# frank-xwang/InstanceDiffusion

Hardware: AMD Instinct MI355X
Metric: images/sec at 512x512, 50 PLMS steps, N=8 instances (Multi-instance Sampler) (higher is better)
Workload: dtype bf16; 1 GPU; C3: SD-1.5 InstanceDiffusion UNet (1.228B params, seeded random weights), 64x64 latent (512x512), 50 PLMS steps, CFG 7.5, N=8 boxes, MIS 0.36, alpha [0.8,0,0.2]; images_per_gpu=32, unet_forwards_per_image=406

## Files before the change

include/idf.h:

```cpp
#ifndef IDF_H_
#define IDF_H_

#include <stdint.h>

#ifdef __cplusplus
extern "C" {
#endif

#define IDF_ABI_VERSION 5

enum { IDF_BF16 = 0, IDF_F16 = 1 };
enum { IDF_E_ARG = -1, IDF_E_ALIGN = -2, IDF_E_UNSUPPORTED = -3 };

enum {
  IDF_EPI_BIAS     = 1,
  IDF_EPI_ROWBIAS  = 2,
  IDF_EPI_RES      = 4,
  IDF_EPI_GATE     = 8,
  IDF_EPI_SILU     = 16,
  IDF_EPI_GELU     = 32,
  IDF_EPI_GEGLU    = 64,
  IDF_EPI_OUT_F32  = 128,
  IDF_EPI_OUT_NCHW = 256,
  IDF_EPI_LN_ROW   = 512,
  IDF_EPI_LN_COL   = 1024,
  IDF_EPI_GEGLU_P32 = 2048
};

int idf_abi_version(void);
const char* idf_build_info(void);

enum { IDF_TUNE_GEMM_BIG = 0, IDF_TUNE_ATTN2 = 1, IDF_TUNE_GEMM_RING = 2, IDF_TUNE_BIG_MIN_EFF = 3, IDF_TUNE_ATTN8 = 4, IDF_TUNE_MLP = 5,
       IDF_TUNE_QKV_ROW = 6, IDF_TUNE_GEGLU_ROW = 7 };
int idf_set_tuning(int knob, int value);
enum { IDF_STAT_GEMM_BIG_LAUNCHES = 0, IDF_STAT_ATTN2_LAUNCHES = 1, IDF_STAT_GEMM_RING_LAUNCHES = 2, IDF_STAT_ATTN8_LAUNCHES = 3,
       IDF_STAT_GN_EPI_LAUNCHES = 4 ,
       IDF_STAT_QKV_ROW_LAUNCHES = 6 ,
       IDF_STAT_GEGLU_ROW_LAUNCHES = 7  };
long long idf_get_stat(int stat);

typedef struct {
  const void* A; const void* W; void* out;
  const float* bias; const void* rowbias; const void* res; const float* gate;
  int M, N, K;
  int lda, ldw, ldo, ldr, ld_rowbias;
  int rows_per_batch;
  int batch; long long strideA, strideW, strideO, strideR;
  int epi; int dtype;
  void* ws; long long ws_bytes;
  const float* ln_stats; long long stride_ln_stats;
  const float* ln_c;
  const float* ln_d;
  float* out_stats; float out_stats_eps;
  float ln_eps; float* ln_stats_out;
  void* vt_out; int ld_vt; int vt_col0;
} idf_gemm_args;
int idf_gemm(const idf_gemm_args* a, void* stream);

typedef struct {
  const void* x; int ldx;
  const float* ln_stats;
  const void* w1; int ldw1;
  const float* cd;
  const void* w2p; int ldw2;
  const float* b2;
  const float* gate;
  void* out; int ldo;
  int M, C;
  int dtype;
} idf_mlp_args;
int idf_mlp_geglu(const idf_mlp_args* a, void* stream);

int idf_row_stats(const void* x, int ldx, float* stats, int M, int C, float eps, int dtype, void* stream);

typedef struct {
  const void* x; const void* W; void* out;
  const float* bias; const void* rowbias; const void* res;
  int B, Hin, Win, Cin, Cout;
  int stride;
  int upsample;
  int ldx, ldo, ldr, ld_rowbias;
  int n_valid;
  int epi; int dtype;
  void* ws; long long ws_bytes;
  float* gn_partial;
} idf_conv3x3_args;
int idf_conv3x3(const idf_conv3x3_args* a, void* stream);

int idf_conv_in(const float* x_nchw, const float* w , const float* bias, void* out,
                int B, int Cin, int H, int W, int Cout, int dtype, void* stream);

typedef struct {
  const void* q; int ldq; long long strideQ; int nq;
  const void* k0; int ldk0; long long strideK0; const void* vt0; int ldv0; long long strideV0; int n0;
  const void* k1; int ldk1; long long strideK1; const void* vt1; int ldv1; long long strideV1; int n1;
  void* out; int ldo; long long strideO;
  int B, H, d;
  float scale;
  int dtype;
  const void* qbits; long long strideQb;
  const void* kbits0; long long strideKb0;
  const void* kbits1; long long strideKb1;
} idf_attn_args;
int idf_attention(const idf_attn_args* a, void* stream);

long long idf_groupnorm_ws_floats(int B, int HW);
int idf_groupnorm(const void* x, void* out, const float* gamma, const float* beta, float* ws,
                  int B, int HW, int C, float eps, int silu, int dtype, void* stream);
int idf_groupnorm_stats(const void* x, float* partial, int B, int HW, int C, int nchunks, int dtype, void* stream);
int idf_groupnorm_apply(const void* x, void* out, const float* gamma, const float* beta, const float* partial,
                        int B, int HW, int C, int nchunks, float eps, int silu, int dtype, void* stream);

int idf_layernorm(const void* x, int ldx, void* out, int ldo, const float* gamma, const float* beta,
                  int M, int C, float eps, int dtype, void* stream);

int idf_layernorm_patch2(const void* x, void* out, int ldo, const float* gamma, const float* beta,
                         int B, int H, int W, int C, float eps, int dtype, void* stream);

int idf_seg_in_conv(const float* segs, const float* w , const float* bias, void* out,
                    int B, int Cin, int S, int ldo, int dtype, void* stream);
int idf_dwconv7x7(const void* x, const float* w_tap_major, const float* bias, void* out, int B, int H, int W, int C,
                  int dtype, void* stream);

int idf_scaleu_concat(const void* h, const void* skip, void* out, const float* hscale, const float* sm1,
                      float* ws, int B, int H, int W, int Ch, int Cs, int dtype, void* stream);

int idf_timestep_embedding(const float* t, void* out, int B, int dim, int dtype, void* stream);

int idf_unifusion_embed(const float* text, const float* loc, const float* tmask, const float* lmask,
                        const float* null_text, const float* null_loc, const float* freqs , void* out,
                        int rows, int text_dim, int D, int dtype, void* stream);

int idf_cfg_combine(const float* eps_cond, const float* eps_uncond, float guidance, float* e_t,
                    long long n, void* stream);
int idf_plms_update(const float* x, const float* e_t, const float* e1, const float* e2, const float* e3,
                    const float* e_next, int mode, float a_t, float a_prev, float sqrt_1m_at,
                    float* x_out, long long n, void* stream);

int idf_mis_merge(const float* lat, const int* boxes, float* out, int n_inst, int B, int C, int H, int W,
                  int mode, void* stream);

int idf_softmax_rows(const float* s, void* p, long long rows, int n, long long lds, long long ldp, float scale,
                     int dtype, void* stream);
int idf_pointwise_nchw(const float* x, const float* w , const float* bias, float* out, int B, int Cin,
                       int Cout, long long HW, float in_scale, void* stream);

int idf_cast_f32_to_16(const float* x, void* out, long long n, int dtype, void* stream);

#ifdef __cplusplus
}
#endif
#endif
```

instancediffusion_amd/_lib.py:

```python
from __future__ import annotations

import ctypes as C
import os

_HERE = os.path.dirname(os.path.abspath(__file__))
LIB_PATH = os.environ.get("IDF_LIB_PATH", os.path.join(_HERE, "libidf_gfx950.so"))

IDF_BF16, IDF_F16 = 0, 1
IDF_STAT_GEMM_BIG_LAUNCHES, IDF_STAT_ATTN2_LAUNCHES, IDF_STAT_GEMM_RING_LAUNCHES, IDF_STAT_ATTN8_LAUNCHES, IDF_STAT_GN_EPI_LAUNCHES = 0, 1, 2, 3, 4
IDF_STAT_QKV_ROW_LAUNCHES, IDF_STAT_GEGLU_ROW_LAUNCHES = 6, 7
IDF_TUNE_GEMM_BIG, IDF_TUNE_ATTN2, IDF_TUNE_GEMM_RING, IDF_TUNE_BIG_MIN_EFF, IDF_TUNE_ATTN8, IDF_TUNE_MLP, IDF_TUNE_QKV_ROW, IDF_TUNE_GEGLU_ROW = 0, 1, 2, 3, 4, 5, 6, 7
EPI_LN_ROW, EPI_LN_COL, EPI_GEGLU_P32 = 512, 1024, 2048
EPI_BIAS, EPI_ROWBIAS, EPI_RES, EPI_GATE, EPI_SILU, EPI_GELU, EPI_GEGLU, EPI_OUT_F32, EPI_OUT_NCHW = \
    1, 2, 4, 8, 16, 32, 64, 128, 256

vp, ll, ci, cf = C.c_void_p, C.c_longlong, C.c_int, C.c_float


class GemmArgs(C.Structure):
    _fields_ = [("A", vp), ("W", vp), ("out", vp), ("bias", vp), ("rowbias", vp), ("res", vp), ("gate", vp),
                ("M", ci), ("N", ci), ("K", ci),
                ("lda", ci), ("ldw", ci), ("ldo", ci), ("ldr", ci), ("ld_rowbias", ci),
                ("rows_per_batch", ci),
                ("batch", ci), ("strideA", ll), ("strideW", ll), ("strideO", ll), ("strideR", ll),
                ("epi", ci), ("dtype", ci), ("ws", vp), ("ws_bytes", ll),
                ("ln_stats", vp), ("stride_ln_stats", ll), ("ln_c", vp), ("ln_d", vp),
                ("out_stats", vp), ("out_stats_eps", cf),
                ("ln_eps", cf), ("ln_stats_out", vp),
                ("vt_out", vp), ("ld_vt", ci), ("vt_col0", ci)]


class ConvArgs(C.Structure):
    _fields_ = [("x", vp), ("W", vp), ("out", vp), ("bias", vp), ("rowbias", vp), ("res", vp),
                ("B", ci), ("Hin", ci), ("Win", ci), ("Cin", ci), ("Cout", ci),
                ("stride", ci), ("upsample", ci),
                ("ldx", ci), ("ldo", ci), ("ldr", ci), ("ld_rowbias", ci),
                ("n_valid", ci), ("epi", ci), ("dtype", ci), ("ws", vp), ("ws_bytes", ll), ("gn_partial", vp)]


class AttnArgs(C.Structure):
    _fields_ = [("q", vp), ("ldq", ci), ("strideQ", ll), ("nq", ci),
                ("k0", vp), ("ldk0", ci), ("strideK0", ll), ("vt0", vp), ("ldv0", ci), ("strideV0", ll), ("n0", ci),
                ("k1", vp), ("ldk1", ci), ("strideK1", ll), ("vt1", vp), ("ldv1", ci), ("strideV1", ll), ("n1", ci),
                ("out", vp), ("ldo", ci), ("strideO", ll),
                ("B", ci), ("H", ci), ("d", ci), ("scale", cf), ("dtype", ci),
                ("qbits", vp), ("strideQb", ll), ("kbits0", vp), ("strideKb0", ll), ("kbits1", vp), ("strideKb1", ll)]


class MlpArgs(C.Structure):
    _fields_ = [("x", vp), ("ldx", ci), ("ln_stats", vp), ("w1", vp), ("ldw1", ci), ("cd", vp), ("w2p", vp), ("ldw2", ci),
                ("b2", vp), ("gate", vp), ("out", vp), ("ldo", ci), ("M", ci), ("C", ci), ("dtype", ci)]


SYMBOLS = {
    "idf_abi_version": (ci, []),
    "idf_build_info": (C.c_char_p, []),
    "idf_set_tuning": (ci, [ci, ci]),
    "idf_get_stat": (ll, [ci]),
    "idf_gemm": (ci, [C.POINTER(GemmArgs), vp]),
    "idf_conv3x3": (ci, [C.POINTER(ConvArgs), vp]),
    "idf_mlp_geglu": (ci, [C.POINTER(MlpArgs), vp]),
    "idf_conv_in": (ci, [vp, vp, vp, vp, ci, ci, ci, ci, ci, ci, vp]),
    "idf_attention": (ci, [C.POINTER(AttnArgs), vp]),
    "idf_groupnorm_ws_floats": (ll, [ci, ci]),
    "idf_groupnorm": (ci, [vp, vp, vp, vp, vp, ci, ci, ci, cf, ci, ci, vp]),
    "idf_groupnorm_stats": (ci, [vp, vp, ci, ci, ci, ci, ci, vp]),
    "idf_groupnorm_apply": (ci, [vp, vp, vp, vp, vp, ci, ci, ci, ci, cf, ci, ci, vp]),
    "idf_layernorm": (ci, [vp, ci, vp, ci, vp, vp, ci, ci, cf, ci, vp]),
    "idf_row_stats": (ci, [vp, ci, vp, ci, ci, cf, ci, vp]),
    "idf_layernorm_patch2": (ci, [vp, vp, ci, vp, vp, ci, ci, ci, ci, cf, ci, vp]),
    "idf_seg_in_conv": (ci, [vp, vp, vp, vp, ci, ci, ci, ci, ci, vp]),
    "idf_dwconv7x7": (ci, [vp, vp, vp, vp, ci, ci, ci, ci, ci, vp]),
    "idf_scaleu_concat": (ci, [vp, vp, vp, vp, vp, vp, ci, ci, ci, ci, ci, ci, vp]),
    "idf_timestep_embedding": (ci, [vp, vp, ci, ci, ci, vp]),
    "idf_unifusion_embed": (ci, [vp, vp, vp, vp, vp, vp, vp, vp, ci, ci, ci, ci, vp]),
    "idf_cfg_combine": (ci, [vp, vp, cf, vp, ll, vp]),
    "idf_plms_update": (ci, [vp, vp, vp, vp, vp, vp, ci, cf, cf, cf, vp, ll, vp]),
    "idf_mis_merge": (ci, [vp, vp, vp, ci, ci, ci, ci, ci, ci, vp]),
    "idf_cast_f32_to_16": (ci, [vp, vp, ll, ci, vp]),
    "idf_softmax_rows": (ci, [vp, vp, ll, ci, ll, ll, cf, ci, vp]),
    "idf_pointwise_nchw": (ci, [vp, vp, vp, vp, ci, ci, ci, ll, cf, vp]),
}

_lib = None


def load() -> C.CDLL:
    global _lib
    if _lib is not None:
        return _lib
    if not os.path.exists(LIB_PATH):
        raise RuntimeError(
            f"{LIB_PATH} is missing: the MI355X HIP extension has not been built "
            f"(run instancediffusion_amd/csrc/build.sh or __graft_entry__.build()). "
            f"There is no CPU fallback for the InstanceDiffusion sampling path.")
    import torch
    lib = C.CDLL(LIB_PATH)
    for name, (res, args) in SYMBOLS.items():
        fn = getattr(lib, name)
        fn.restype = res
        fn.argtypes = args
    if lib.idf_abi_version() != 5:
        raise RuntimeError("libidf_gfx950.so ABI version mismatch")
    _lib = lib
    return lib


class IdfError(RuntimeError):
    pass


def check(status: int, what: str):
    if status != 0:
        kind = {-1: "invalid argument", -2: "misaligned pointer/leading dimension", -3: "unsupported"}.get(
            status, f"hipError_t {status}")
        raise IdfError(f"{what} failed: {kind}")
```

instancediffusion_amd/csrc/gemm_conv.hip:

```cpp
#include "gemm_core.h"
#include "attn_core.h"
#include <cstdlib>

using namespace idfcore;

namespace {

#ifndef IDF_GEMM_BIG_DEFAULT
#define IDF_GEMM_BIG_DEFAULT 1
#endif
constexpr int LSTR = 72;

template <int DT, int BM, int BN, int WM, int WN, int KLOOP_LDS_BYTES>
__device__ __forceinline__ void tile_epilogue(const CoreParams& p, f32x16 (&acc)[WN / 32][WM / 32], unsigned short* smem,
                                              int m0, int n0, int bz, int wm, int wn, int lane, int wave) {
  constexpr int TM = WM / 32, TN = WN / 32;
  const int l31 = lane & 31, hi = lane >> 5;
  constexpr int CSTR = WN + 4;
  static_assert(4 * WM * CSTR * 4 <= KLOOP_LDS_BYTES, "C staging must fit in the allocated LDS");
  __syncthreads();
  float* Cl = reinterpret_cast<float*>(smem) + wave * (WM * CSTR);
#pragma unroll
  for (int a = 0; a < TN; ++a)
#pragma unroll
    for (int b = 0; b < TM; ++b)
#pragma unroll
      for (int q = 0; q < 4; ++q)
        *reinterpret_cast<f32x4*>(Cl + (b * 32 + l31) * CSTR + a * 32 + 8 * q + 4 * hi) =
            f32x4{acc[a][b][4 * q], acc[a][b][4 * q + 1], acc[a][b][4 * q + 2], acc[a][b][4 * q + 3]};
  __builtin_amdgcn_fence(__ATOMIC_RELEASE, "wavefront");
  __builtin_amdgcn_wave_barrier();
  __builtin_amdgcn_fence(__ATOMIC_ACQUIRE, "wavefront");

  const int epi = p.epi;
  const float gate = (epi & IDF_EPI_GATE) ? p.gate[0] : 0.0f;
  const int mw = m0 + wm * WM, nw = n0 + wn * WN;
  if (epi & IDF_EPI_GEGLU) {
    if constexpr (WN >= 64) {
      constexpr int CHV = WN / 16;
      constexpr int RPP = 64 / CHV;
      const int P = (epi & IDF_EPI_GEGLU_P32) ? 32 : 64, half = P >> 1, cpg = P >> 4;
#pragma unroll
      for (int pass = 0; pass < WM / RPP; ++pass) {
        const int row = pass * RPP + lane / CHV, c = lane % CHV;
        const int grp = c / cpg, cc = c - grp * cpg;
        const int m = mw + row;
        const int npk = nw + grp * P + cc * 8;
        if (m < p.M && npk + half < p.N) {
          const float* src = Cl + row * CSTR + grp * P + cc * 8;
          float v[8], g[8];
          *reinterpret_cast<f32x4*>(v) = *reinterpret_cast<const f32x4*>(src);
          *reinterpret_cast<f32x4*>(v + 4) = *reinterpret_cast<const f32x4*>(src + 4);
          *reinterpret_cast<f32x4*>(g) = *reinterpret_cast<const f32x4*>(src + half);
          *reinterpret_cast<f32x4*>(g + 4) = *reinterpret_cast<const f32x4*>(src + half + 4);
          const f32x4 bv0 = *reinterpret_cast<const f32x4*>(p.bias + npk), bv1 = *reinterpret_cast<const f32x4*>(p.bias + npk + 4);
          const f32x4 bg0 = *reinterpret_cast<const f32x4*>(p.bias + npk + half), bg1 = *reinterpret_cast<const f32x4*>(p.bias + npk + half + 4);
          if (epi & IDF_EPI_LN_ROW) {
            const f32x2 st = *reinterpret_cast<const f32x2*>(p.ln_stats + (size_t)bz * p.stride_ln_stats + 2 * (size_t)m);
#pragma unroll
            for (int e = 0; e < 8; ++e) {
              v[e] = st[1] * fmaf(-st[0], p.ln_c[npk + e], v[e]);
              g[e] = st[1] * fmaf(-st[0], p.ln_c[npk + half + e], g[e]);
            }
          }
#pragma unroll
          for (int e = 0; e < 4; ++e) {
            v[e] = (v[e] + bv0[e]) * gelu_erf_f(g[e] + bg0[e]);
            v[e + 4] = (v[e + 4] + bv1[e]) * gelu_erf_f(g[e + 4] + bg1[e]);
          }
          const int j = (nw + grp * P) / 2 + cc * 8;
          unsigned short* o = reinterpret_cast<unsigned short*>(p.out) + (size_t)bz * p.strideO + (size_t)m * p.ldo + j;
          if ((p.ldo & 7) == 0) {
            *reinterpret_cast<u32x4*>(o) = pack8<DT>(v);
          } else {
            const u32x4 pk = pack8<DT>(v);
            *reinterpret_cast<u32x2*>(o) = u32x2{pk[0], pk[1]};
            *reinterpret_cast<u32x2*>(o + 4) = u32x2{pk[2], pk[3]};
          }
        }
      }
    }
    return;
  }
  constexpr int CH = WN / 8;
  constexpr int RPP = 64 / CH;
#pragma unroll
  for (int pass = 0; pass < WM / RPP; ++pass) {
    const int row = pass * RPP + lane / CH, c = lane % CH;
    const int m = mw + row, n = nw + c * 8;
    if (m >= p.M || n >= p.N) continue;
    const float* src = Cl + row * CSTR + c * 8;
    float v[8];
    *reinterpret_cast<f32x4*>(v) = *reinterpret_cast<const f32x4*>(src);
    *reinterpret_cast<f32x4*>(v + 4) = *reinterpret_cast<const f32x4*>(src + 4);
    if (p.splitk > 1) {
      float* o = p.ws + ((size_t)blockIdx.z * p.M + m) * p.N + n;
      if (n + 7 < p.N && ((p.N & 3) == 0)) {
        *reinterpret_cast<f32x4*>(o) = f32x4{v[0], v[1], v[2], v[3]};
        *reinterpret_cast<f32x4*>(o + 4) = f32x4{v[4], v[5], v[6], v[7]};
      } else {
#pragma unroll
        for (int e = 0; e < 8; ++e) if (n + e < p.N) o[e] = v[e];
      }
    } else {
      epilogue8<DT>(p, bz, m, n, v, gate);
    }
  }
}

template <int DT, int BM, int BN, int WM, int WN, bool CONV>
__global__ __launch_bounds__(256, 2) void gemm_kernel(const CoreParams p) {
  constexpr int TM = WM / 32, TN = WN / 32;
  constexpr int WAVES_N = BN / WN;
  constexpr int AR = BM / 32, WR = BN / 32;
  static_assert((BM / WM) * (BN / WN) == 4, "4 waves per workgroup");
  extern __shared__ __attribute__((aligned(16))) unsigned short smem[];
  constexpr int BUF = (BM + BN) * LSTR;

  const int tid = threadIdx.x;
  const int lane = tid & 63, wave = tid >> 6;
  const int l31 = lane & 31, hi = lane >> 5;
  const int wn = wave % WAVES_N, wm = wave / WAVES_N;
  int tile;
  {
    const int T = gridDim.x, L = blockIdx.x;
    const int q = T >> 3, r = T & 7, xcd = L & 7, i = L >> 3;
    tile = (xcd < r ? xcd * (q + 1) : r * (q + 1) + (xcd - r) * q) + i;
  }
  const int tiles_n = (p.N + BN - 1) / BN;
  const int m_tile = tile / tiles_n;
  const int n0 = (tile - m_tile * tiles_n) * BN, m0 = m_tile * BM;
  const int bz = (p.splitk > 1) ? 0 : blockIdx.z;

  const unsigned short* Wb = p.W + (size_t)bz * p.strideW;
  const unsigned short* Ab = p.A + (size_t)bz * p.strideA;

  const int c = tid & 7, r0 = tid >> 3;
  const unsigned short* wrow[WR];
#pragma unroll
  for (int i = 0; i < WR; ++i) {
    int n = min(n0 + r0 + 32 * i, p.N - 1);
    wrow[i] = Wb + (size_t)n * p.ldw + c * 8;
  }
  const unsigned short* arow[AR];
  int ay[AR], ax[AR];
#pragma unroll
  for (int i = 0; i < AR; ++i) {
    int m = min(m0 + r0 + 32 * i, p.M - 1);
    if (CONV) {
      int hw = p.Ho * p.Wo;
      int b = m / hw, rem = m - b * hw;
      int yo = rem / p.Wo, xo = rem - yo * p.Wo;
      ay[i] = yo * p.stride - 1;
      ax[i] = xo * p.stride - 1;
      arow[i] = Ab + (size_t)b * p.Hin * p.Win * p.lda + c * 8;
    } else {
      ay[i] = ax[i] = 0;
      arow[i] = Ab + (size_t)m * p.lda + c * 8;
    }
  }
  const int nk_all = p.K / BK;
  const int kt_begin = (p.splitk > 1) ? blockIdx.z * p.kt_per_slice : 0;
  const int nk = (p.splitk > 1) ? min(p.kt_per_slice, nk_all - kt_begin) : nk_all;
  int tap = 0, ci0 = 0;
  if (CONV) { tap = (kt_begin * BK) / p.Cin; ci0 = kt_begin * BK - tap * p.Cin; }

  u32x4 raA[AR], rwA[WR], raB[AR], rwB[WR];
  unsigned okA = 0, okB = 0;
  auto load_tile = [&](int kt, u32x4* ra, u32x4* rw, unsigned& okbits) {
#pragma unroll
    for (int i = 0; i < WR; ++i) rw[i] = *reinterpret_cast<const u32x4*>(wrow[i] + (size_t)(kt_begin + kt) * BK);
    if (CONV) {
      const int ky = tap / 3, kx = tap - ky * 3;
      const int Hup = p.Hin << p.up, Wup = p.Win << p.up;
      unsigned bits = 0;
#pragma unroll
      for (int i = 0; i < AR; ++i) {
        const int yi = ay[i] + ky, xi = ax[i] + kx;
        const bool ok = (yi >= 0) & (yi < Hup) & (xi >= 0) & (xi < Wup);
        const int ys = min(max(yi, 0), Hup - 1) >> p.up, xs = min(max(xi, 0), Wup - 1) >> p.up;
        ra[i] = *reinterpret_cast<const u32x4*>(arow[i] + ((size_t)ys * p.Win + xs) * p.lda + ci0);
        bits |= (ok ? 1u : 0u) << i;
      }
      okbits = bits;
      ci0 += BK;
      if (ci0 >= p.Cin) { ci0 = 0; ++tap; }
    } else {
#pragma unroll
      for (int i = 0; i < AR; ++i) ra[i] = *reinterpret_cast<const u32x4*>(arow[i] + (size_t)(kt_begin + kt) * BK);
    }
  };
  auto store_tile = [&](int buf, const u32x4* ra, const u32x4* rw, unsigned okbits) {
    unsigned short* Al = smem + buf * BUF;
    unsigned short* Wl = Al + BM * LSTR;
#pragma unroll
    for (int i = 0; i < AR; ++i) {
      u32x4 v = ra[i];
      if (CONV) {
        const unsigned keep = ((okbits >> i) & 1u) ? 0xffffffffu : 0u;
        v[0] &= keep; v[1] &= keep; v[2] &= keep; v[3] &= keep;
      }
      *reinterpret_cast<u32x4*>(Al + (r0 + 32 * i) * LSTR + c * 8) = v;
    }
#pragma unroll
    for (int i = 0; i < WR; ++i) *reinterpret_cast<u32x4*>(Wl + (r0 + 32 * i) * LSTR + c * 8) = rw[i];
  };

  f32x16 acc[TN][TM];
#pragma unroll
  for (int a = 0; a < TN; ++a)
#pragma unroll
    for (int b = 0; b < TM; ++b)
#pragma unroll
      for (int r = 0; r < 16; ++r) acc[a][b][r] = 0.0f;

  auto compute = [&](int buf) {
    const unsigned short* Al = smem + buf * BUF;
    const unsigned short* Wl = Al + BM * LSTR;
    const unsigned short* af_base = Al + (wm * WM + l31) * LSTR + hi * 8;
    const unsigned short* wf_base = Wl + (wn * WN + l31) * LSTR + hi * 8;
    u32x4 wf[2][TN], af[2][TM];
#pragma unroll
    for (int a = 0; a < TN; ++a) wf[0][a] = *reinterpret_cast<const u32x4*>(wf_base + a * 32 * LSTR);
#pragma unroll
    for (int b = 0; b < TM; ++b) af[0][b] = *reinterpret_cast<const u32x4*>(af_base + b * 32 * LSTR);
#pragma unroll
    for (int ks = 0; ks < BK / 16; ++ks) {
      const int cur = ks & 1, nxt = cur ^ 1;
      if (ks + 1 < BK / 16) {
#pragma unroll
        for (int a = 0; a < TN; ++a) wf[nxt][a] = *reinterpret_cast<const u32x4*>(wf_base + a * 32 * LSTR + (ks + 1) * 16);
#pragma unroll
        for (int b = 0; b < TM; ++b) af[nxt][b] = *reinterpret_cast<const u32x4*>(af_base + b * 32 * LSTR + (ks + 1) * 16);
      }
#pragma unroll
      for (int a = 0; a < TN; ++a)
#pragma unroll
        for (int b = 0; b < TM; ++b) acc[a][b] = Elem<DT>::mfma32(wf[cur][a], af[cur][b], acc[a][b]);
    }
  };

  load_tile(0, raA, rwA, okA);
  store_tile(0, raA, rwA, okA);
  if (nk > 1) load_tile(1, raA, rwA, okA);
  __syncthreads();
  int kt = 0;
  for (; kt + 3 < nk; kt += 2) {
    load_tile(kt + 2, raB, rwB, okB);
    __builtin_amdgcn_sched_barrier(0);
    compute(0);
    store_tile(1, raA, rwA, okA);
    __syncthreads();
    load_tile(kt + 3, raA, rwA, okA);
    __builtin_amdgcn_sched_barrier(0);
    compute(1);
    store_tile(0, raB, rwB, okB);
    __syncthreads();
  }
  const int rem = nk - kt;
  if (rem == 3) {
    load_tile(kt + 2, raB, rwB, okB);
    compute(0);
    store_tile(1, raA, rwA, okA);
    __syncthreads();
    compute(1);
    store_tile(0, raB, rwB, okB);
    __syncthreads();
    compute(0);
  } else if (rem == 2) {
    compute(0);
    store_tile(1, raA, rwA, okA);
    __syncthreads();
    compute(1);
  } else {
    compute(0);
  }

  tile_epilogue<DT, BM, BN, WM, WN, 2 * (BM + BN) * LSTR * 2>(p, acc, smem, m0, n0, bz, wm, wn, lane, wave);
}

template <int DT, int BM, int BN, int WM, int WN, bool CONV>
__global__ __launch_bounds__(256, 2) void gemm_kernel_dma(const CoreParams p) {
  constexpr int TM = WM / 32, TN = WN / 32;
  constexpr int WAVES_N = BN / WN;
  constexpr int RS = 64;
  constexpr int BUF = (BM + BN) * RS;
  constexpr int W_INST = BN / 8 / 4, A_INST = BM / 8 / 4;
  constexpr int AR = BM / 32;
  constexpr int KLOOP_LDS = 2 * BUF * 2;
  constexpr int CSTAGE = 4 * WM * (WN + 4) * 4;
  constexpr int LDS_BYTES = KLOOP_LDS > CSTAGE ? KLOOP_LDS : CSTAGE;
  static_assert((BM / WM) * (BN / WN) == 4, "4 waves per workgroup");
  extern __shared__ __attribute__((aligned(16))) unsigned short smem[];

  const int tid = threadIdx.x;
  const int lane = tid & 63, wave = __builtin_amdgcn_readfirstlane(tid >> 6);
  const int l31 = lane & 31, hi = lane >> 5;
  const int wn = wave % WAVES_N, wm = wave / WAVES_N;
  int tile;
  {
    const int T = gridDim.x, L = blockIdx.x;
    const int q = T >> 3, r = T & 7, xcd = L & 7, i = L >> 3;
    tile = (xcd < r ? xcd * (q + 1) : r * (q + 1) + (xcd - r) * q) + i;
  }
  const int tiles_n = (p.N + BN - 1) / BN;
  const int m_tile = tile / tiles_n;
  const int n0 = (tile - m_tile * tiles_n) * BN, m0 = m_tile * BM;
  const int bz = (p.splitk > 1) ? 0 : blockIdx.z;
  const unsigned short* Wb = p.W + (size_t)bz * p.strideW;
  const unsigned short* Ab = p.A + (size_t)bz * p.strideA;

  const int nk_all = p.K / BK;
  const int kt_begin = (p.splitk > 1) ? blockIdx.z * p.kt_per_slice : 0;
  const int nk = (p.splitk > 1) ? min(p.kt_per_slice, nk_all - kt_begin) : nk_all;

  const int dr = lane >> 3, dc = lane & 7;
  const unsigned short* wsrc[W_INST];
#pragma unroll
  for (int j = 0; j < W_INST; ++j) {
    const int row = 8 * (wave + 4 * j) + dr;
    const int n = min(n0 + row, p.N - 1);
    wsrc[j] = Wb + (size_t)n * p.ldw + (size_t)kt_begin * BK + ((dc ^ ((row >> 1) & 7)) * 8);
  }
  const unsigned short* asrc[A_INST];
  if (!CONV) {
#pragma unroll
    for (int j = 0; j < A_INST; ++j) {
      const int row = 8 * (wave + 4 * j) + dr;
      const int m = min(m0 + row, p.M - 1);
      asrc[j] = Ab + (size_t)m * p.lda + (size_t)kt_begin * BK + ((dc ^ ((row >> 1) & 7)) * 8);
    }
  }
  const int c = tid & 7, r0 = tid >> 3;
  const unsigned short* arow[AR];
  int ay[AR], ax[AR];
  int tap = 0, ci0 = 0;
  if (CONV) {
#pragma unroll
    for (int i = 0; i < AR; ++i) {
      const int m = min(m0 + r0 + 32 * i, p.M - 1);
      const int hw = p.Ho * p.Wo;
      const int b = m / hw, rem = m - b * hw;
      const int yo = rem / p.Wo, xo = rem - yo * p.Wo;
      ay[i] = yo * p.stride - 1;
      ax[i] = xo * p.stride - 1;
      arow[i] = Ab + (size_t)b * p.Hin * p.Win * p.lda + c * 8;
    }
    tap = (kt_begin * BK) / p.Cin;
    ci0 = kt_begin * BK - tap * p.Cin;
  }
  const int a_sw = (c ^ ((r0 >> 1) & 7)) * 8;
  u32x4 ra[AR];
  unsigned okbits = 0;

  auto dma_tile = [&](int kt, int buf) {
    unsigned short* Al = smem + buf * BUF;
    unsigned short* Wl = Al + BM * RS;
#pragma unroll
    for (int j = 0; j < W_INST; ++j)
      __builtin_amdgcn_global_load_lds((const __attribute__((address_space(1))) void*)(wsrc[j] + (size_t)kt * BK),
                                       (__attribute__((address_space(3))) void*)(Wl + 8 * (wave + 4 * j) * RS), 16, 0, 0);
    if (!CONV) {
#pragma unroll
      for (int j = 0; j < A_INST; ++j)
        __builtin_amdgcn_global_load_lds((const __attribute__((address_space(1))) void*)(asrc[j] + (size_t)kt * BK),
                                         (__attribute__((address_space(3))) void*)(Al + 8 * (wave + 4 * j) * RS), 16, 0, 0);
    }
  };
  auto gather_tile = [&]() {
    const int ky = tap / 3, kx = tap - ky * 3;
    const int Hup = p.Hin << p.up, Wup = p.Win << p.up;
    unsigned bits = 0;
#pragma unroll
    for (int i = 0; i < AR; ++i) {
      const int yi = ay[i] + ky, xi = ax[i] + kx;
      const bool ok = (yi >= 0) & (yi < Hup) & (xi >= 0) & (xi < Wup);
      const int ys = min(max(yi, 0), Hup - 1) >> p.up, xs = min(max(xi, 0), Wup - 1) >> p.up;
      ra[i] = *reinterpret_cast<const u32x4*>(arow[i] + ((size_t)ys * p.Win + xs) * p.lda + ci0);
      bits |= (ok ? 1u : 0u) << i;
    }
    okbits = bits;
    ci0 += BK;
    if (ci0 >= p.Cin) { ci0 = 0; ++tap; }
  };
  auto scatter_tile = [&](int buf) {
    unsigned short* Al = smem + buf * BUF;
#pragma unroll
    for (int i = 0; i < AR; ++i) {
      u32x4 v = ra[i];
      const unsigned keep = ((okbits >> i) & 1u) ? 0xffffffffu : 0u;
      v[0] &= keep; v[1] &= keep; v[2] &= keep; v[3] &= keep;
      *reinterpret_cast<u32x4*>(Al + (r0 + 32 * i) * RS + a_sw) = v;
    }
  };

  f32x16 acc[TN][TM];
#pragma unroll
  for (int a = 0; a < TN; ++a)
#pragma unroll
    for (int b = 0; b < TM; ++b)
#pragma unroll
      for (int r = 0; r < 16; ++r) acc[a][b][r] = 0.0f;

  const int f_sw = (l31 >> 1) & 7;
  auto compute = [&](int buf) {
    const unsigned short* Al = smem + buf * BUF;
    const unsigned short* Wl = Al + BM * RS;
    const unsigned short* af_base = Al + (wm * WM + l31) * RS;
    const unsigned short* wf_base = Wl + (wn * WN + l31) * RS;
    u32x4 wf[2][TN], af[2][TM];
    {
      const int slot = (hi ^ f_sw) * 8;
#pragma unroll
      for (int a = 0; a < TN; ++a) wf[0][a] = *reinterpret_cast<const u32x4*>(wf_base + a * 32 * RS + slot);
#pragma unroll
      for (int b = 0; b < TM; ++b) af[0][b] = *reinterpret_cast<const u32x4*>(af_base + b * 32 * RS + slot);
    }
#pragma unroll
    for (int ks = 0; ks < BK / 16; ++ks) {
      const int cur = ks & 1, nxt = cur ^ 1;
      if (ks + 1 < BK / 16) {
        const int slot = (((ks + 1) * 2 + hi) ^ f_sw) * 8;
#pragma unroll
        for (int a = 0; a < TN; ++a) wf[nxt][a] = *reinterpret_cast<const u32x4*>(wf_base + a * 32 * RS + slot);
#pragma unroll
        for (int b = 0; b < TM; ++b) af[nxt][b] = *reinterpret_cast<const u32x4*>(af_base + b * 32 * RS + slot);
      }
#pragma unroll
      for (int a = 0; a < TN; ++a)
#pragma unroll
        for (int b = 0; b < TM; ++b) acc[a][b] = Elem<DT>::mfma32(wf[cur][a], af[cur][b], acc[a][b]);
    }
  };

  dma_tile(0, 0);
  if (CONV) { gather_tile(); scatter_tile(0); }
  __syncthreads();
  for (int kt = 0; kt < nk; ++kt) {
    const bool more = (kt + 1 < nk);
    if (more) {
      dma_tile(kt + 1, (kt + 1) & 1);
      if (CONV) gather_tile();
    }
    compute(kt & 1);
    if (CONV && more) scatter_tile((kt + 1) & 1);
    __syncthreads();
  }
  tile_epilogue<DT, BM, BN, WM, WN, LDS_BYTES>(p, acc, smem, m0, n0, bz, wm, wn, lane, wave);
}

__device__ __attribute__((aligned(128))) unsigned short ring_zero_page[64];

__device__ __forceinline__ void ring_dma16(const void* addr , const void* lds_lane0) {
  const unsigned l = __builtin_amdgcn_readfirstlane((unsigned)(size_t)lds_lane0);
  asm volatile("s_mov_b32 m0, %0\n\ts_nop 0\n\tglobal_load_lds_dwordx4 %1, off" ::"s"(l), "v"(addr) : "memory");
}
template <int PT, int MAXA> __device__ __forceinline__ void ring_wait(int ahead) {
  if constexpr (MAXA <= 0) {
    asm volatile("s_waitcnt vmcnt(0)" ::: "memory");
  } else {
    static_assert(MAXA * PT < 64, "vmcnt is a 6-bit field");
    if (ahead >= MAXA) asm volatile("s_waitcnt vmcnt(%0)" ::"n"(MAXA * PT) : "memory");
    else ring_wait<PT, MAXA - 1>(ahead);
  }
}

template <int DT, int BM, int BN, int WM, int WN, bool CONV, int NS>
__global__ __launch_bounds__(256, 1) void gemm_kernel_ring(const CoreParams p) {
  constexpr int TM = WM / 32, TN = WN / 32;
  constexpr int WAVES_N = BN / WN;
  constexpr int RS = 64;
  constexpr int BUF = (BM + BN) * RS;
  constexpr int W_INST = BN / 8 / 4, A_INST = BM / 8 / 4;
  constexpr int PER_TILE = W_INST + A_INST;
  constexpr int KLOOP_LDS = NS * BUF * 2;
  constexpr int CSTAGE = 4 * WM * (WN + 4) * 4;
  constexpr int LDS_BYTES = KLOOP_LDS > CSTAGE ? KLOOP_LDS : CSTAGE;
  static_assert((BM / WM) * (BN / WN) == 4, "4 waves per workgroup");
  static_assert(NS >= 3 && LDS_BYTES <= 160 * 1024, "ring must fit the CU's LDS");
  extern __shared__ __attribute__((aligned(16))) unsigned short smem[];

  const int tid = threadIdx.x;
  const int lane = tid & 63, wave = __builtin_amdgcn_readfirstlane(tid >> 6);
  const int l31 = lane & 31, hi = lane >> 5;
  const int wn = wave % WAVES_N, wm = wave / WAVES_N;
  int tile;
  {
    const int T = gridDim.x, L = blockIdx.x;
    const int q = T >> 3, r = T & 7, xcd = L & 7, i = L >> 3;
    tile = (xcd < r ? xcd * (q + 1) : r * (q + 1) + (xcd - r) * q) + i;
  }
  const int tiles_n = (p.N + BN - 1) / BN;
  const int m_tile = tile / tiles_n;
  const int n0 = (tile - m_tile * tiles_n) * BN, m0 = m_tile * BM;
  const int bz = (p.splitk > 1) ? 0 : blockIdx.z;
  const unsigned short* Wb = p.W + (size_t)bz * p.strideW;
  const unsigned short* Ab = p.A + (size_t)bz * p.strideA;

  const int nk_all = p.K / BK;
  const int kt_begin = (p.splitk > 1) ? blockIdx.z * p.kt_per_slice : 0;
  const int nk = (p.splitk > 1) ? min(p.kt_per_slice, nk_all - kt_begin) : nk_all;

  const int dr = lane >> 3, dc = lane & 7;
  const unsigned short* wsrc[W_INST];
#pragma unroll
  for (int j = 0; j < W_INST; ++j) {
    const int row = 8 * (wave + 4 * j) + dr;
    const int n = min(n0 + row, p.N - 1);
    wsrc[j] = Wb + (size_t)n * p.ldw + (size_t)kt_begin * BK + ((dc ^ ((row >> 1) & 7)) * 8);
  }
  const unsigned short* asrc[A_INST];
  int ay[A_INST], ax[A_INST];
#pragma unroll
  for (int j = 0; j < A_INST; ++j) {
    const int row = 8 * (wave + 4 * j) + dr;
    const int m = min(m0 + row, p.M - 1);
    const int ch = (dc ^ ((row >> 1) & 7)) * 8;
    if (!CONV) {
      asrc[j] = Ab + (size_t)m * p.lda + (size_t)kt_begin * BK + ch;
      ay[j] = ax[j] = 0;
    } else {
      const int hw = p.Ho * p.Wo;
      const int b = m / hw, rem = m - b * hw;
      const int yo = rem / p.Wo, xo = rem - yo * p.Wo;
      ay[j] = yo * p.stride - 1;
      ax[j] = xo * p.stride - 1;
      asrc[j] = Ab + (size_t)b * p.Hin * p.Win * p.lda + ch;
    }
  }
  int tap = 0, ci0 = 0;
  if (CONV) { tap = (kt_begin * BK) / p.Cin; ci0 = kt_begin * BK - tap * p.Cin; }
  int kt_issue = 0, st_issue = 0;

  auto issue_tile = [&]() {
    unsigned short* Al = smem + st_issue * BUF;
    unsigned short* Wl = Al + BM * RS;
#pragma unroll
    for (int j = 0; j < W_INST; ++j) ring_dma16(wsrc[j] + (size_t)kt_issue * BK, Wl + 8 * (wave + 4 * j) * RS);
    if (!CONV) {
#pragma unroll
      for (int j = 0; j < A_INST; ++j) ring_dma16(asrc[j] + (size_t)kt_issue * BK, Al + 8 * (wave + 4 * j) * RS);
    } else {
      const int ky = tap / 3, kx = tap - ky * 3;
      const int Hup = p.Hin << p.up, Wup = p.Win << p.up;
#pragma unroll
      for (int j = 0; j < A_INST; ++j) {
        const int yi = ay[j] + ky, xi = ax[j] + kx;
        const bool ok = (yi >= 0) & (yi < Hup) & (xi >= 0) & (xi < Wup);
        const int ys = yi >> p.up, xs = xi >> p.up;
        const unsigned short* src = ok ? asrc[j] + ((size_t)ys * p.Win + xs) * p.lda + ci0 : ring_zero_page + dc * 8;
        ring_dma16(src, Al + 8 * (wave + 4 * j) * RS);
      }
      ci0 += BK;
      if (ci0 >= p.Cin) { ci0 = 0; ++tap; }
    }
    ++kt_issue;
    st_issue = (st_issue + 1 == NS) ? 0 : st_issue + 1;
  };

  f32x16 acc[TN][TM];
#pragma unroll
  for (int a = 0; a < TN; ++a)
#pragma unroll
    for (int b = 0; b < TM; ++b)
#pragma unroll
      for (int r = 0; r < 16; ++r) acc[a][b][r] = 0.0f;

  const int f_sw = (l31 >> 1) & 7;
  auto compute = [&](int st) {
    const unsigned short* Al = smem + st * BUF;
    const unsigned short* Wl = Al + BM * RS;
    const unsigned short* af_base = Al + (wm * WM + l31) * RS;
    const unsigned short* wf_base = Wl + (wn * WN + l31) * RS;
    u32x4 wf[2][TN], af[2][TM];
    {
      const int slot = (hi ^ f_sw) * 8;
#pragma unroll
      for (int a = 0; a < TN; ++a) wf[0][a] = *reinterpret_cast<const u32x4*>(wf_base + a * 32 * RS + slot);
#pragma unroll
      for (int b = 0; b < TM; ++b) af[0][b] = *reinterpret_cast<const u32x4*>(af_base + b * 32 * RS + slot);
    }
#pragma unroll
    for (int ks = 0; ks < BK / 16; ++ks) {
      const int cur = ks & 1, nxt = cur ^ 1;
      if (ks + 1 < BK / 16) {
        const int slot = (((ks + 1) * 2 + hi) ^ f_sw) * 8;
#pragma unroll
        for (int a = 0; a < TN; ++a) wf[nxt][a] = *reinterpret_cast<const u32x4*>(wf_base + a * 32 * RS + slot);
#pragma unroll
        for (int b = 0; b < TM; ++b) af[nxt][b] = *reinterpret_cast<const u32x4*>(af_base + b * 32 * RS + slot);
      }
#pragma unroll
      for (int a = 0; a < TN; ++a)
#pragma unroll
        for (int b = 0; b < TM; ++b) acc[a][b] = Elem<DT>::mfma32(wf[cur][a], af[cur][b], acc[a][b]);
    }
  };

  const int pre = min(NS - 1, nk);
  for (int i = 0; i < pre; ++i) issue_tile();
  int st = 0;
  for (int kt = 0; kt < nk; ++kt) {
    ring_wait<PER_TILE, NS - 2>(kt_issue - kt - 1);
    __builtin_amdgcn_s_barrier();
    if (kt_issue < nk) issue_tile();
    compute(st);
    st = (st + 1 == NS) ? 0 : st + 1;
  }
  tile_epilogue<DT, BM, BN, WM, WN, LDS_BYTES>(p, acc, smem, m0, n0, bz, wm, wn, lane, wave);
}

template <int DT>
__global__ __launch_bounds__(256) void splitk_reduce_kernel(const CoreParams p) {
  const int n8 = (p.N + 7) / 8;
  const size_t i = (size_t)blockIdx.x * 256 + threadIdx.x;
  if (i >= (size_t)p.tail_rows * n8) return;
  const int ml = (int)(i / n8), n = (int)(i - (size_t)ml * n8) * 8;
  const int m = p.tail_m0 + ml;
  float v[8] = {0.f, 0.f, 0.f, 0.f, 0.f, 0.f, 0.f, 0.f};
  const bool vec = (n + 7 < p.N) && ((p.N & 3) == 0);
  const size_t slab = (size_t)p.tail_rows * p.N;
  const float* w = p.ws + (size_t)ml * p.N + n;
  if (vec) {
    int s = 0;
    for (; s + 4 <= p.splitk; s += 4) {
      f32x4 a[4][2];
#pragma unroll
      for (int u = 0; u < 4; ++u) {
        a[u][0] = *reinterpret_cast<const f32x4*>(w + (size_t)(s + u) * slab);
        a[u][1] = *reinterpret_cast<const f32x4*>(w + (size_t)(s + u) * slab + 4);
      }
#pragma unroll
      for (int u = 0; u < 4; ++u)
#pragma unroll
        for (int e = 0; e < 4; ++e) { v[e] += a[u][0][e]; v[e + 4] += a[u][1][e]; }
    }
    for (; s < p.splitk; ++s) {
      const f32x4 w0 = *reinterpret_cast<const f32x4*>(w + (size_t)s * slab), w1 = *reinterpret_cast<const f32x4*>(w + (size_t)s * slab + 4);
#pragma unroll
      for (int e = 0; e < 4; ++e) { v[e] += w0[e]; v[e + 4] += w1[e]; }
    }
  } else {
    for (int s = 0; s < p.splitk; ++s) {
#pragma unroll
      for (int e = 0; e < 8; ++e) if (n + e < p.N) v[e] += w[(size_t)s * slab + e];
    }
  }
  const float gate = (p.epi & IDF_EPI_GATE) ? p.gate[0] : 0.0f;
  epilogue8<DT>(p, 0, m, n, v, gate);
}

std::atomic<long long> idf_stat_gn_epi_launches{0};
std::atomic<long long> idf_stat_ring_launches{0};
std::atomic<long long> idf_stat_gegluw_launches{0};
std::atomic<long long> idf_stat_qkvw_launches{0};
int g_big_mode = -2;
inline int gemm_big_mode() {
  if (g_big_mode == -2) {
    const char* e = getenv("IDF_GEMM_BIG");
    const int v = e ? atoi(e) : IDF_GEMM_BIG_DEFAULT;
    g_big_mode = (v < 0 || v > 3) ? IDF_GEMM_BIG_DEFAULT : v;
  }
  return g_big_mode;
}

inline int kloop_variant(bool conv) {
  static int v = -2;
  if (v == -2) { const char* e = getenv("IDF_GEMM_VARIANT"); v = e ? atoi(e) : -1; }
  if (v == 1 || v == 2) return v;
  return conv ? 1 : 2;
}

template <int DT, int BM, int BN, int WM, int WN, bool CONV>
int launch_cfg(const CoreParams& p, int batch, hipStream_t s) {
  const int variant = kloop_variant(CONV);
  void (*kern)(const CoreParams) = gemm_kernel<DT, BM, BN, WM, WN, CONV>;
  constexpr int cstage = 4 * WM * (WN + 4) * 4;
  constexpr int kloop2 = 2 * (BM + BN) * 64 * 2;
  int smem = 2 * (BM + BN) * LSTR * 2;
  if (variant == 2) { kern = gemm_kernel_dma<DT, BM, BN, WM, WN, CONV>; smem = kloop2 > cstage ? kloop2 : cstage; }
  static std::atomic<unsigned long long> attr_done[3];
  if (const int e = idf_lds_optin(reinterpret_cast<const void*>(kern), smem, attr_done[variant])) return e;
  CoreParams q = p;
  const int tiles = ((p.N + BN - 1) / BN) * ((p.M + BM - 1) / BM);
  const int nk = p.K / BK;
  q.splitk = 1; q.kt_per_slice = nk;
  q.tail_m0 = 0; q.tail_rows = p.M;
  if (batch == 1 && p.ws && !(p.epi & IDF_EPI_GEGLU) && tiles < 192 && nk >= 8) {
    int want = (512 + tiles - 1) / tiles;
    if (want > nk / 4) want = nk / 4;
    if (want > 64) want = 64;
    while (want > 1 && (size_t)want * p.M * p.N * sizeof(float) > p.ws_bytes) --want;
    if (want > 1) {
      q.kt_per_slice = (nk + want - 1) / want;
      q.splitk = (nk + q.kt_per_slice - 1) / q.kt_per_slice;
    }
  }
  dim3 grid(tiles, 1, q.splitk > 1 ? q.splitk : batch);
  hipLaunchKernelGGL(kern, grid, dim3(256), smem, s, q);
  if (q.splitk > 1) {
    const size_t n8 = (size_t)q.M * ((q.N + 7) / 8);
    hipLaunchKernelGGL(splitk_reduce_kernel<DT>, dim3((unsigned)((n8 + 255) / 256)), dim3(256), 0, s, q);
  }
  return idf_launch_status();
}

#ifndef IDF_GEMM_RING_DEFAULT
#define IDF_GEMM_RING_DEFAULT 256
#endif
int g_ring_tiles = -1;
inline int gemm_ring_tiles() {
  if (g_ring_tiles < 0) {
    const char* e = getenv("IDF_GEMM_RING");
    const int v = e ? atoi(e) : IDF_GEMM_RING_DEFAULT;
    g_ring_tiles = v < 0 ? IDF_GEMM_RING_DEFAULT : v;
  }
  return g_ring_tiles;
}

template <int DT, int BM, int BN, int WM, int WN, bool CONV, int NS>
int launch_ring_cfg(const CoreParams& p, int batch, hipStream_t s) {
  const int tiles = ((p.N + BN - 1) / BN) * ((p.M + BM - 1) / BM);
  const int nk = p.K / BK;
  static int batched_old = -1;
  if (batched_old < 0) { const char* e = getenv("IDF_RING_BATCHED"); batched_old = (e && e[0] == '1') ? 1 : 0; }
  if ((long long)tiles * (batched_old ? 1 : batch) > gemm_ring_tiles()) return IDF_BIG_UNSUPPORTED;
  const int slots = idf_num_cu();
  if (batch == 1 && p.ws && !(p.epi & IDF_EPI_GEGLU) && tiles * 2 > slots && tiles < 192 && nk >= 8) return IDF_BIG_UNSUPPORTED;
  void (*kern)(const CoreParams) = gemm_kernel_ring<DT, BM, BN, WM, WN, CONV, NS>;
  constexpr int cstage = 4 * WM * (WN + 4) * 4;
  constexpr int kloop = NS * (BM + BN) * 64 * 2;
  constexpr int smem = kloop > cstage ? kloop : cstage;
  static std::atomic<unsigned long long> attr_done{0};
  if (const int e = idf_lds_optin(reinterpret_cast<const void*>(kern), smem, attr_done)) return e;
  CoreParams q = p;
  q.splitk = 1; q.kt_per_slice = nk;
  q.tail_m0 = 0; q.tail_rows = p.M;
  static int slice_kt = 0;
  if (slice_kt == 0) { const char* e = getenv("IDF_RING_SLICE_KT"); slice_kt = e ? atoi(e) : 8; if (slice_kt < 1) slice_kt = 8; }
  if (batch == 1 && p.ws && !(p.epi & IDF_EPI_GEGLU) && tiles * 2 <= slots && nk >= 2 * slice_kt) {
    int want = slots / tiles;
    if (want > nk / slice_kt) want = nk / slice_kt;
    if (want > 64) want = 64;
    while (want > 1 && (size_t)want * p.M * p.N * sizeof(float) > p.ws_bytes) --want;
    if (want > 1) {
      q.kt_per_slice = (nk + want - 1) / want;
      q.splitk = (nk + q.kt_per_slice - 1) / q.kt_per_slice;
    }
  }
  dim3 grid(tiles, 1, q.splitk > 1 ? q.splitk : batch);
  hipLaunchKernelGGL(kern, grid, dim3(256), smem, s, q);
  ++idf_stat_ring_launches;
  if (q.splitk > 1) {
    const size_t n8 = (size_t)q.M * ((q.N + 7) / 8);
    hipLaunchKernelGGL(splitk_reduce_kernel<DT>, dim3((unsigned)((n8 + 255) / 256)), dim3(256), 0, s, q);
  }
  return idf_launch_status();
}

template <int DT, bool CONV>
int launch(const CoreParams& p, int batch, hipStream_t s, int* parts_out = nullptr, int* gst_out = nullptr) {
  const bool geglu = (p.epi & IDF_EPI_GEGLU) != 0;
  static int wide = -2;
  if (wide == -2) { const char* e = getenv("IDF_TILE_WIDE"); wide = e ? (e[0] == '1' ? 1 : 0) : -1; }
  const bool use_wide = (wide >= 0) ? (wide == 1) : CONV;
  const int big = gemm_big_mode();
  const bool t128p = geglu || (p.N % 128 == 0) || p.N > 1024 || (use_wide && p.N > 128);
  const long long tiles_small = (long long)((p.N + (t128p ? 127 : 63)) / (t128p ? 128 : 64)) * ((p.M + 127) / 128);
  const bool ring_first = big != 2 && gemm_ring_tiles() > 0 && tiles_small <= 128 && tiles_small <= gemm_ring_tiles();
  if (big > 0 && batch == 1 && !ring_first) {
    int splitk = 1, tail_m0 = 0;
    const int rc = idf_launch_big(p, DT, CONV, big == 2, s, &splitk, parts_out, big == 3 ? &tail_m0 : nullptr, gst_out);
    if (rc != IDF_BIG_UNSUPPORTED) {
      if (rc == 0 && splitk > 1) {
        CoreParams q = p;
        q.splitk = splitk; q.tail_m0 = tail_m0; q.tail_rows = p.M - tail_m0;
        const size_t n8 = (size_t)q.tail_rows * ((q.N + 7) / 8);
        hipLaunchKernelGGL(splitk_reduce_kernel<DT>, dim3((unsigned)((n8 + 255) / 256)), dim3(256), 0, s, q);
        return idf_launch_status();
      }
      return rc;
    }
  }
  CoreParams q = p;
  if ((p.epi & IDF_EPI_LN_ROW) && !p.ln_stats) {
    float* st = p.ln_stats_out ? p.ln_stats_out : p.ws;
    if (!st || (!p.ln_stats_out && p.ws_bytes < (size_t)p.M * 2 * sizeof(float))) return IDF_E_ARG;
    const int rc = idf_row_stats(p.A, p.lda, st, p.M, p.K, p.ln_eps, DT, s);
    if (rc) return rc;
    q.ln_stats = st; q.stride_ln_stats = 0;
    if (!p.ln_stats_out) { q.ws = nullptr; q.ws_bytes = 0; }
  }
  const bool t128 = geglu || (q.N % 128 == 0) || q.N > 1024 || (use_wide && q.N > 128);
  if (gemm_ring_tiles() > 0) {
    const int rc = t128 ? launch_ring_cfg<DT, 128, 128, 64, 64, CONV, 4>(q, batch, s) : launch_ring_cfg<DT, 128, 64, 64, 32, CONV, 5>(q, batch, s);
    if (rc != IDF_BIG_UNSUPPORTED) return rc;
  }
  if (t128) return launch_cfg<DT, 128, 128, 64, 64, CONV>(q, batch, s);
  return launch_cfg<DT, 128, 64, 64, 32, CONV>(q, batch, s);
}

}

__global__ __launch_bounds__(256) void stats_finalize_kernel(const float* __restrict__ parts, int P, float cols, float* __restrict__ out,
                                                            int M, float eps) {
  const int m = blockIdx.x * 256 + threadIdx.x;
  if (m >= M) return;
  const f32x2* pp = reinterpret_cast<const f32x2*>(parts) + (size_t)m * P;
  f32x2 t = pp[0];
  float mean = t[0], m2 = t[1], n = cols;
  for (int i = 1; i < P; ++i) {
    t = pp[i];
    const float dlt = t[0] - mean, nn = n + cols;
    mean += dlt * (cols / nn);
    m2 += t[1] + dlt * dlt * (n * cols / nn);
    n = nn;
  }
  reinterpret_cast<f32x2*>(out)[m] = f32x2{mean, rsqrtf(m2 / n + eps)};
}

int idf_stats_finalize(const float* stat_parts, int parts, int cols_per_part, float* out_stats, int M, float eps, hipStream_t s) {
  hipLaunchKernelGGL(stats_finalize_kernel, dim3((M + 255) / 256), dim3(256), 0, s, stat_parts, parts, (float)cols_per_part,
                     out_stats, M, eps);
  return idf_launch_status();
}

extern "C" int idf_set_tuning(int knob, int value) {
  if (knob == IDF_TUNE_GEMM_BIG) {
    if (value < 0 || value > 3) return IDF_E_ARG;
    const int prev = gemm_big_mode();
    g_big_mode = value;
    return prev;
  }
  if (knob == IDF_TUNE_GEMM_RING) {
    if (value < 0) return IDF_E_ARG;
    const int prev = gemm_ring_tiles();
    g_ring_tiles = value;
    return prev;
  }
  if (knob == IDF_TUNE_BIG_MIN_EFF) {
    if (value < 1 || value > 100) return IDF_E_ARG;
    return idf_big_min_eff_pct(value);
  }
  if (knob == IDF_TUNE_ATTN2) {
    if (value < 0 || value > 6) return IDF_E_ARG;
    return idf_attn2_set_mode(value);
  }
  if (knob == IDF_TUNE_ATTN8) {
    if (value < 0 || value > 6) return IDF_E_ARG;
    return idf_attn8_set_mode(value);
  }
  if (knob == IDF_TUNE_GEGLU_ROW) {
    if (value < 0 || value > 1) return IDF_E_ARG;
    return idf_gegluw_set_mode(value);
  }
  if (knob == IDF_TUNE_QKV_ROW) {
    if (value < 0 || value > 1) return IDF_E_ARG;
    return idf_qkvw_set_mode(value);
  }
  if (knob == IDF_TUNE_MLP) {
    if (value < 0 || value > 1) return IDF_E_ARG;
    return idf_mlp_set_mode(value);
  }
  return IDF_E_ARG;
}

extern "C" long long idf_get_stat(int stat) {
  if (stat == IDF_STAT_GEMM_BIG_LAUNCHES) return idf_stat_big_launches.load();
  if (stat == IDF_STAT_ATTN2_LAUNCHES) return idf_stat_attn2_launches.load();
  if (stat == IDF_STAT_GEMM_RING_LAUNCHES) return idf_stat_ring_launches.load();
  if (stat == IDF_STAT_ATTN8_LAUNCHES) return idf_stat_attn8_launches.load();
  if (stat == IDF_STAT_GN_EPI_LAUNCHES) return idf_stat_gn_epi_launches.load();
  if (stat == IDF_STAT_QKV_ROW_LAUNCHES) return idf_stat_qkvw_launches.load();
  if (stat == IDF_STAT_GEGLU_ROW_LAUNCHES) return idf_stat_gegluw_launches.load();
  return -1;
}

extern "C" int idf_gemm(const idf_gemm_args* a, void* stream) {
  if (!a || !a->A || !a->W || !a->out) return IDF_E_ARG;
  if (a->M <= 0 || a->N <= 0 || a->K <= 0 || (a->K % BK) != 0) return IDF_E_ARG;
  if ((a->lda % 8) || (a->ldw % 8) || !aligned16(a->A) || !aligned16(a->W)) return IDF_E_ALIGN;
  if ((a->epi & IDF_EPI_GATE) && !(a->epi & IDF_EPI_RES)) return IDF_E_ARG;
  if ((a->epi & IDF_EPI_RES) && !a->res) return IDF_E_ARG;
  if ((a->epi & (IDF_EPI_BIAS | IDF_EPI_GEGLU)) && !a->bias) return IDF_E_ARG;
  if ((a->epi & IDF_EPI_GEGLU) && ((a->N % 64) || (a->ldo % 4))) return IDF_E_ARG;
  if ((a->epi & IDF_EPI_GEGLU_P32) && !(a->epi & IDF_EPI_GEGLU)) return IDF_E_ARG;
  if ((a->epi & IDF_EPI_ROWBIAS) && (!a->rowbias || a->rows_per_batch <= 0)) return IDF_E_ARG;
  if (a->epi & IDF_EPI_OUT_NCHW) return IDF_E_ARG;
  CoreParams p{};
  p.W = (const unsigned short*)a->W; p.ldw = a->ldw; p.strideW = a->strideW; p.N = a->N;
  p.A = (const unsigned short*)a->A; p.lda = a->lda; p.strideA = a->strideA; p.M = a->M; p.K = a->K;
  p.out = a->out; p.ldo = a->ldo; p.strideO = a->strideO;
  p.bias = a->bias; p.rowbias = (const unsigned short*)a->rowbias; p.ld_rowbias = a->ld_rowbias;
  p.rows_per_batch = a->rows_per_batch;
  p.res = (const unsigned short*)a->res; p.ldr = a->ldr; p.strideR = a->strideR;
  p.gate = a->gate; p.epi = a->epi; p.n_valid = a->N;
  p.ws = (float*)a->ws; p.ws_bytes = a->ws ? (size_t)a->ws_bytes : 0;
  const int batch = a->batch > 0 ? a->batch : 1;
  if (a->epi & (IDF_EPI_LN_ROW | IDF_EPI_LN_COL)) {
    if ((a->epi & IDF_EPI_LN_ROW) && (a->epi & IDF_EPI_LN_COL)) return IDF_E_ARG;
    if (!a->ln_c) return IDF_E_ARG;
    if (!a->ln_stats) {
      if (!(a->epi & IDF_EPI_LN_ROW) || batch != 1 || (a->K % 8) || a->K > 1536 || !(a->ln_eps > 0.0f)) return IDF_E_ARG;
      if (a->ln_stats_out && (((uintptr_t)a->ln_stats_out) & 7u)) return IDF_E_ALIGN;
      p.ln_eps = a->ln_eps; p.ln_stats_out = a->ln_stats_out;
    }
    if ((a->epi & IDF_EPI_LN_ROW) && !(a->epi & IDF_EPI_BIAS)) return IDF_E_ARG;
    if ((a->epi & IDF_EPI_LN_COL) && (!a->ln_d || (a->epi & IDF_EPI_GEGLU))) return IDF_E_ARG;
    if ((((uintptr_t)a->ln_stats) & 7u) || (a->stride_ln_stats & 1)) return IDF_E_ALIGN;
    p.ln_stats = a->ln_stats; p.stride_ln_stats = a->stride_ln_stats; p.ln_c = a->ln_c; p.ln_d = a->ln_d;
  }
  if (a->out_stats) {
    if ((a->epi & (IDF_EPI_GEGLU | IDF_EPI_OUT_F32)) || (a->N % 8) || a->N > 1536 || (a->ldo % 8)) return IDF_E_ARG;
    if (batch > 1 && a->strideO != (long long)a->M * a->ldo) return IDF_E_ARG;
  }
  hipStream_t s = (hipStream_t)stream;
  int rc = IDF_E_UNSUPPORTED;
  if (a->vt_out) {
    const int Nv = a->N - a->vt_col0;
    if (a->vt_col0 <= 0 || Nv <= 0 || batch != 1 || a->ld_vt < a->M || (a->ld_vt % 8) || !aligned16(a->vt_out)) return IDF_E_ARG;
    if (a->epi & ~(IDF_EPI_BIAS | IDF_EPI_LN_ROW)) return IDF_E_ARG;
    if (!(a->epi & IDF_EPI_LN_ROW)) return IDF_E_ARG;
    if (a->out_stats) return IDF_E_ARG;
    const bool self_ln = (a->epi & IDF_EPI_LN_ROW) && !a->ln_stats;
    if (self_ln && !a->ln_stats_out) return IDF_E_ARG;
    p.vt_out = (unsigned short*)a->vt_out; p.ld_vt = a->ld_vt; p.vt_col0 = a->vt_col0;
    {
      int r = idf_launch_qkv320w(p, a->dtype, s);
      if (r == IDF_BIG_UNSUPPORTED) r = idf_launch_qkv640w(p, a->dtype, s);
      if (r != IDF_BIG_UNSUPPORTED) { if (r == 0) { ++idf_stat_big_launches; ++idf_stat_qkvw_launches; } return r; }
    }
    if (gemm_big_mode() > 0) {
      const int r = idf_launch_big(p, a->dtype, false, gemm_big_mode() == 2, s, nullptr);
      if (r != IDF_BIG_UNSUPPORTED) return r;
    }
    CoreParams p1 = p;
    p1.vt_out = nullptr; p1.vt_col0 = 0; p1.N = a->vt_col0; p1.n_valid = a->vt_col0;
    if (a->dtype == IDF_BF16) rc = launch<IDF_BF16, false>(p1, 1, s);
    else if (a->dtype == IDF_F16) rc = launch<IDF_F16, false>(p1, 1, s);
    if (rc) return rc;
    CoreParams p2{};
    p2.A = p.W + (size_t)a->vt_col0 * p.ldw; p2.lda = p.ldw; p2.M = Nv; p2.K = a->K;
    p2.W = p.A; p2.ldw = p.lda; p2.N = a->M; p2.n_valid = a->M;
    p2.out = a->vt_out; p2.ldo = a->ld_vt;
    p2.ws = p.ws; p2.ws_bytes = p.ws_bytes;
    p2.epi = 0;
    if (a->epi & IDF_EPI_LN_ROW) {
      p2.epi |= IDF_EPI_LN_COL;
      p2.ln_stats = self_ln ? a->ln_stats_out : a->ln_stats; p2.stride_ln_stats = 0;
      p2.ln_c = a->ln_c + a->vt_col0; p2.ln_d = a->bias + a->vt_col0;
    }
    if (a->dtype == IDF_BF16) return launch<IDF_BF16, false>(p2, 1, s);
    if (a->dtype == IDF_F16) return launch<IDF_F16, false>(p2, 1, s);
    return IDF_E_UNSUPPORTED;
  }
  int parts = 0;
  if ((a->epi & IDF_EPI_GEGLU) && batch == 1 && !a->out_stats) {
    const int r = idf_launch_geglu640w(p, a->dtype, s);
    if (r != IDF_BIG_UNSUPPORTED) { if (r == 0) { ++idf_stat_big_launches; ++idf_stat_gegluw_launches; } return r; }
  }
  if (a->out_stats && batch == 1 && p.ws) p.stat_parts = p.ws;
  if (a->dtype == IDF_BF16) rc = launch<IDF_BF16, false>(p, batch, s, &parts);
  else if (a->dtype == IDF_F16) rc = launch<IDF_F16, false>(p, batch, s, &parts);
  if (rc == 0 && a->out_stats) {
    if (parts > 0) rc = idf_stats_finalize(p.stat_parts, parts, a->N / parts, a->out_stats, a->M, a->out_stats_eps, s);
    else rc = idf_row_stats(a->out, a->ldo, a->out_stats, batch * a->M, a->N, a->out_stats_eps, a->dtype, stream);
  }
  return rc;
}

extern "C" int idf_conv3x3(const idf_conv3x3_args* a, void* stream) {
  if (!a || !a->x || !a->W || !a->out) return IDF_E_ARG;
  if (a->B <= 0 || a->Cin <= 0 || (a->Cin % BK) != 0 || a->Cout <= 0) return IDF_E_ARG;
  if (a->stride != 1 && a->stride != 2) return IDF_E_ARG;
  if (a->upsample != 0 && a->upsample != 1) return IDF_E_ARG;
  if ((a->ldx % 8) || !aligned16(a->x) || !aligned16(a->W)) return IDF_E_ALIGN;
  if (a->epi & (IDF_EPI_GEGLU | IDF_EPI_GATE)) return IDF_E_ARG;
  if ((a->epi & IDF_EPI_RES) && !a->res) return IDF_E_ARG;
  if ((a->epi & IDF_EPI_BIAS) && !a->bias) return IDF_E_ARG;
  CoreParams p{};
  const int Hup = a->Hin << a->upsample, Wup = a->Win << a->upsample;
  p.Ho = (Hup - 1) / a->stride + 1; p.Wo = (Wup - 1) / a->stride + 1;
  p.W = (const unsigned short*)a->W; p.ldw = 9 * a->Cin; p.strideW = 0; p.N = a->Cout;
  p.A = (const unsigned short*)a->x; p.lda = a->ldx; p.strideA = 0; p.M = a->B * p.Ho * p.Wo; p.K = 9 * a->Cin;
  p.Hin = a->Hin; p.Win = a->Win; p.Cin = a->Cin; p.stride = a->stride; p.up = a->upsample;
  p.out = a->out; p.ldo = a->ldo; p.strideO = 0;
  p.bias = a->bias; p.rowbias = (const unsigned short*)a->rowbias; p.ld_rowbias = a->ld_rowbias;
  p.rows_per_batch = p.Ho * p.Wo;
  p.res = (const unsigned short*)a->res; p.ldr = a->ldr; p.strideR = 0;
  p.gate = nullptr; p.epi = a->epi; p.n_valid = a->n_valid > 0 ? a->n_valid : a->Cout;
  p.ws = (float*)a->ws; p.ws_bytes = a->ws ? (size_t)a->ws_bytes : 0;
  if ((a->epi & IDF_EPI_ROWBIAS) && !a->rowbias) return IDF_E_ARG;
  hipStream_t s = (hipStream_t)stream;
  if (a->gn_partial) {
    const int hw = p.Ho * p.Wo;
    if ((hw % 64) || (a->Cout % 32) || a->ldo != a->Cout || (a->epi & (IDF_EPI_OUT_F32 | IDF_EPI_OUT_NCHW))) return IDF_E_ARG;
    if (((uintptr_t)a->gn_partial) & 7u) return IDF_E_ALIGN;
    p.gn_partial = a->gn_partial; p.gn_hw = hw;
  }
  int gst = 0, rc = IDF_E_UNSUPPORTED;
  if (a->dtype == IDF_BF16) rc = launch<IDF_BF16, true>(p, 1, s, nullptr, &gst);
  else if (a->dtype == IDF_F16) rc = launch<IDF_F16, true>(p, 1, s, nullptr, &gst);
  if (rc == 0 && gst) ++idf_stat_gn_epi_launches;
  if (rc == 0 && a->gn_partial && !gst)
    rc = idf_groupnorm_stats(a->out, a->gn_partial, a->B, p.Ho * p.Wo, a->Cout, p.Ho * p.Wo / 64, a->dtype, stream);
  return rc;
}
```

instancediffusion_amd/csrc/gemm_core.h:

```cpp
#pragma once
#include "common.h"
#include <atomic>

namespace idfcore {

struct CoreParams {
  const unsigned short* W; int ldw; long long strideW; int N;
  const unsigned short* A; int lda; long long strideA; int M; int K;
  int Hin, Win, Cin, Ho, Wo, stride, up;
  void* out; int ldo; long long strideO;
  const float* bias; const unsigned short* rowbias; int ld_rowbias; int rows_per_batch;
  const unsigned short* res; int ldr; long long strideR;
  const float* gate; int epi; int n_valid;
  float* ws; size_t ws_bytes; int splitk; int kt_per_slice;
  int full_items; int kt_full; int tail_m0; int tail_rows;
  const float* ln_stats; long long stride_ln_stats; const float* ln_c; const float* ln_d;
  float ln_eps; float* ln_stats_out;
  unsigned short* vt_out; int ld_vt; int vt_col0;
  float* stat_parts; int parts;
  float* gn_partial; int gn_hw;
  int tile_walk; int dephase; int dephase_units; int epi_vmcnt;
};

constexpr int BK = 64;

template <int DT>
__device__ __forceinline__ void epilogue8(const CoreParams& p, int bz, int m, int n, float* v, float gate) {
  const int epi = p.epi;
  const bool full = (n + 7 < p.N);
  if (epi & IDF_EPI_LN_ROW) {
    const f32x2 st = *reinterpret_cast<const f32x2*>(p.ln_stats + (size_t)bz * p.stride_ln_stats + 2 * (size_t)m);
#pragma unroll
    for (int e = 0; e < 8; ++e) if (n + e < p.N) v[e] = st[1] * fmaf(-st[0], p.ln_c[n + e], v[e]);
  }
  if (epi & IDF_EPI_LN_COL) {
    const float cm = p.ln_c[m], dm = p.ln_d[m];
    const float* st = p.ln_stats + (size_t)bz * p.stride_ln_stats + 2 * (size_t)n;
#pragma unroll
    for (int e = 0; e < 8; ++e) if (n + e < p.N) v[e] = fmaf(st[2 * e + 1], fmaf(-cm, st[2 * e], v[e]), dm);
  }
  if (epi & IDF_EPI_BIAS) {
    if (full) {
      const f32x4 b0 = *reinterpret_cast<const f32x4*>(p.bias + n), b1 = *reinterpret_cast<const f32x4*>(p.bias + n + 4);
#pragma unroll
      for (int e = 0; e < 4; ++e) { v[e] += b0[e]; v[e + 4] += b1[e]; }
    } else {
#pragma unroll
      for (int e = 0; e < 8; ++e) if (n + e < p.N) v[e] += p.bias[n + e];
    }
  }
  if (epi & IDF_EPI_ROWBIAS) {
    const unsigned short* rb = p.rowbias + (size_t)(m / p.rows_per_batch) * p.ld_rowbias + n;
    if (full && ((p.ld_rowbias & 7) == 0)) {
      float r[8];
      unpack8<DT>(*reinterpret_cast<const u32x4*>(rb), r);
#pragma unroll
      for (int e = 0; e < 8; ++e) v[e] += r[e];
    } else {
#pragma unroll
      for (int e = 0; e < 8; ++e) if (n + e < p.N) v[e] += Elem<DT>::to_f32(rb[e]);
    }
  }
  if (epi & IDF_EPI_SILU) {
#pragma unroll
    for (int e = 0; e < 8; ++e) v[e] = silu_f(v[e]);
  }
  if (epi & IDF_EPI_GELU) {
#pragma unroll
    for (int e = 0; e < 8; ++e) v[e] = gelu_erf_f(v[e]);
  }
  if (epi & IDF_EPI_RES) {
    const unsigned short* rr = p.res + (size_t)bz * p.strideR + (size_t)m * p.ldr + n;
    const float gm = (epi & IDF_EPI_GATE) ? gate : 1.0f;
    if (full && ((p.ldr & 7) == 0)) {
      float r[8];
      unpack8<DT>(*reinterpret_cast<const u32x4*>(rr), r);
#pragma unroll
      for (int e = 0; e < 8; ++e) v[e] = fmaf(gm, v[e], r[e]);
    } else {
#pragma unroll
      for (int e = 0; e < 8; ++e) if (n + e < p.N) v[e] = fmaf(gm, v[e], Elem<DT>::to_f32(rr[e]));
    }
  }
  if (epi & IDF_EPI_OUT_NCHW) {
    const int hw = p.Ho * p.Wo;
    const int bb = m / hw, rem = m - bb * hw;
    float* o = reinterpret_cast<float*>(p.out);
#pragma unroll
    for (int e = 0; e < 8; ++e)
      if (n + e < p.n_valid) o[((size_t)bb * p.n_valid + (n + e)) * hw + rem] = v[e];
  } else if (epi & IDF_EPI_OUT_F32) {
    float* o = reinterpret_cast<float*>(p.out) + (size_t)bz * p.strideO + (size_t)m * p.ldo + n;
    if (full && ((p.ldo & 3) == 0)) {
      *reinterpret_cast<f32x4*>(o) = f32x4{v[0], v[1], v[2], v[3]};
      *reinterpret_cast<f32x4*>(o + 4) = f32x4{v[4], v[5], v[6], v[7]};
    } else {
#pragma unroll
      for (int e = 0; e < 8; ++e) if (n + e < p.N) o[e] = v[e];
    }
  } else {
    unsigned short* o = reinterpret_cast<unsigned short*>(p.out) + (size_t)bz * p.strideO + (size_t)m * p.ldo + n;
    if (full && ((p.ldo & 7) == 0)) {
      *reinterpret_cast<u32x4*>(o) = pack8<DT>(v);
    } else {
#pragma unroll
      for (int e = 0; e < 8; ++e) if (n + e < p.N) o[e] = Elem<DT>::from_f32(v[e]);
    }
  }
}


}

#define IDF_BIG_UNSUPPORTED (-100)
extern std::atomic<long long> idf_stat_big_launches;
int idf_launch_big(const idfcore::CoreParams& p, int dtype, bool conv, bool force, hipStream_t s, int* splitk_out,
                   int* parts_out = nullptr, int* tail_m0_out = nullptr, int* gst_out = nullptr);
int idf_launch_qkv320w(const idfcore::CoreParams& p, int dtype, hipStream_t s);
int idf_launch_geglu640w(const idfcore::CoreParams& p, int dtype, hipStream_t s);
int idf_gegluw_set_mode(int v);
int idf_launch_qkv640w(const idfcore::CoreParams& p, int dtype, hipStream_t s);
int idf_qkv640w_set_mode(int v);
int idf_qkvw_set_mode(int v);
int idf_mlp_set_mode(int v);
int idf_big_min_eff_pct(int set);
int idf_num_cu();
int idf_stats_finalize(const float* stat_parts, int parts, int cols_per_part, float* out_stats, int M, float eps, hipStream_t s);
```

instancediffusion_amd/csrc/mlp_fused.hip:

```cpp
#include "gemm_core.h"
#include "mw_prims.h"
#include <cstdlib>
#include <atomic>
#include <type_traits>
#include <utility>

using namespace idfcore;
using namespace idfmw;

namespace {

constexpr int MLP_C = 320, MLP_H = 1280, MLP_CH = 32, MLP_NCH = MLP_H / MLP_CH;
constexpr int MLP_BM = 128;
constexpr int W1_BYTES = 5 * 64 * 128;
constexpr int W2_BYTES = 320 * 64;
constexpr int CD_BYTES = 1024;
constexpr int SLOT_BYTES = W1_BYTES + W2_BYTES + CD_BYTES;
constexpr int XCH_OFF = 2 * SLOT_BYTES, STG_OFF = XCH_OFF + 8 * 1024, MLP_SMEM = STG_OFF + 8 * 2048;

struct MlpParams {
  const unsigned short* x; int ldx;
  const float* ln_stats;
  const unsigned short* w1; int ldw1;
  const float* cd;
  const unsigned short* w2p; int ldw2;
  const float* b2; const float* gate;
  unsigned short* out; int ldo;
  int M;
};

__device__ __forceinline__ void mlp_dma16(const void* sbase , unsigned voff_bytes, unsigned lds) {
  lds = __builtin_amdgcn_readfirstlane(lds);
  asm volatile("s_mov_b32 m0, %0\n\ts_nop 0\n\tglobal_load_lds_dwordx4 %1, %2" ::"s"(lds), "v"(voff_bytes), "s"(sbase) : "memory");
}

#ifdef IDF_MLP_TRACE
__device__ unsigned long long idf_mlp_trace_buf[4][10];
#define MTR_DECL unsigned long long tr_last = __builtin_readcyclecounter(), tr_acc[10] = {0, 0, 0, 0, 0, 0, 0, 0, 0, 0};
#define MTR(i) { const unsigned long long tr_now = __builtin_readcyclecounter(); tr_acc[i] += tr_now - tr_last; tr_last = tr_now; }
#define MTR_COUNT(i) { tr_acc[i] += 1; }
#define MTR_DUMP { const int trb = blockIdx.x == 0 ? 0 : ((int)blockIdx.x == (int)gridDim.x / 2 ? 1 : -1);                     \
    if (trb >= 0 && lane == 0 && (wave == 0 || wave == 4)) { for (int i = 0; i < 10; ++i) idf_mlp_trace_buf[trb * 2 + (wave ? 1 : 0)][i] = tr_acc[i]; } }
#else
#define MTR_DECL
#define MTR(i) {}
#define MTR_COUNT(i) {}
#define MTR_DUMP {}
#endif

template <int DT>
__global__ __launch_bounds__(512, 2) void mlp320_kernel(const MlpParams p, const int tiles) {
  constexpr bool PF = true, SK = true;
  extern __shared__ __attribute__((aligned(128))) char smem[];
  const int tid = threadIdx.x;
  const int lane = tid & 63, wave = __builtin_amdgcn_readfirstlane(tid >> 6);
  const int l31 = lane & 31, hi = lane >> 5;
  const int wn = wave & 1, wm = wave >> 1;
  const int G = gridDim.x;

  unsigned w1_voff, w2_voff[3];
  {
    const int row = 8 * wave + (lane >> 3);
    const int src = (lane & 7) ^ ((row >> 1) & 7);
    w1_voff = (unsigned)(row * p.ldw1 + src * 8) * 2u;
  }
#pragma unroll
  for (int t = 0; t < 3; ++t) {
    const int row = 16 * (wave + 8 * t) + (lane >> 2);
    const int src = (lane & 3) ^ ((row >> 2) & 3);
    w2_voff[t] = (unsigned)(row * p.ldw2 + src * 8) * 2u;
  }
  auto issue_piece = [&](int idx, int j, int slot) {
    char* const base = smem + slot * SLOT_BYTES;
    if (idx == 0) {
      if (wave == 7) mlp_dma16(p.cd + (size_t)j * 128, (unsigned)((lane & 31) * 16), lds_u32(base + W1_BYTES + W2_BYTES));
    } else if (idx < 6) {
      mlp_dma16(p.w1 + (size_t)j * 64 * p.ldw1 + (idx - 1) * 64, w1_voff, lds_u32(base + (idx - 1) * 8192 + wave * 1024));
    } else {
      const int t = idx - 6;
      if (wave + 8 * t < 20) mlp_dma16(p.w2p + j * 32, w2_voff[t], lds_u32(base + W1_BYTES + (wave + 8 * t) * 1024));
    }
  };
  auto issue_chunk = [&](int j, int slot) {
#pragma unroll
    for (int idx = 0; idx < 9; ++idx) issue_piece(idx, j, slot);
  };
  auto wait_w1 = [&]() {
    if (wave < 4) asm volatile("s_waitcnt vmcnt(3)" ::: "memory");
    else asm volatile("s_waitcnt vmcnt(2)" ::: "memory");
  };
  auto wait_w2 = [&](bool next_in_flight) {
    if (!next_in_flight) asm volatile("s_waitcnt vmcnt(0)" ::: "memory");
    else if (wave < 4 || wave == 7) asm volatile("s_waitcnt vmcnt(8)" ::: "memory");
    else asm volatile("s_waitcnt vmcnt(7)" ::: "memory");
  };

  const int sw1 = (l31 >> 1) & 7, sw2 = (l31 >> 2) & 3;
  const int w1_row = (32 * wn + l31) * 128;
  const int w2_row = W1_BYTES + (160 * wn + l31) * 64;
  char* const xch_mine = smem + XCH_OFF + wave * 1024 + lane * 16;
  char* const xch_peer = smem + XCH_OFF + (wave ^ 1) * 1024 + lane * 16;
  char* const stg = smem + STG_OFF + wave * 2048;

  int tile = ((G & 7) == 0) ? (int)(blockIdx.x & 7) * (G >> 3) + (int)(blockIdx.x >> 3) : (int)blockIdx.x;
  if (tile >= tiles) return;
  const float gate = p.gate ? p.gate[0] : 1.0f;

  issue_chunk(0, 0);
  int g = 0;
  MTR_DECL
  for (; tile < tiles; tile += G) {
    const int m = tile * MLP_BM + wm * 32 + l31;
    u32x4 xf[20];
    {
      const unsigned short* xr = p.x + (size_t)m * p.ldx + 8 * hi;
#pragma unroll
      for (int ks = 0; ks < 20; ++ks) xf[ks] = *reinterpret_cast<const u32x4*>(xr + 16 * ks);
    }
    const f32x2 st = *reinterpret_cast<const f32x2*>(p.ln_stats + 2 * (size_t)m);
    const float nmu = -st[0], rstd = st[1];
    f32x16 acc2[5];
#pragma unroll
    for (int a = 0; a < 5; ++a)
#pragma unroll
      for (int r = 0; r < 16; ++r) acc2[a][r] = 0.0f;

    MTR(8)
    for (int j = 0; j < MLP_NCH; ++j, ++g) {
      wait_w1();
      MTR(0)
      __builtin_amdgcn_s_barrier();
      asm volatile("" ::: "memory");
      MTR(1) MTR_COUNT(9)
      const bool last = (j == MLP_NCH - 1) && (tile + G >= tiles);
      const int jn = j + 1 == MLP_NCH ? 0 : j + 1;
      const bool late = SK && wave >= 4 && !last;
      if (!last && !late) issue_chunk(jn, (g + 1) & 1);
      MTR(2)
      const char* const sl = smem + (g & 1) * SLOT_BYTES;

      f32x16 acc1;
#pragma unroll
      for (int r = 0; r < 16; ++r) acc1[r] = 0.0f;
      const float* cdp = reinterpret_cast<const float*>(sl + W1_BYTES + W2_BYTES) + 32 * wn + 4 * hi;
      f32x4 cv[2], cg[2], dv[2], dg[2];
      {
        const char* wb = sl + w1_row;
        constexpr int DEPTH = PF ? 4 : 1;
        u32x4 wf[DEPTH + 1];
        auto rd = [&](int ks) {
          const int kt = ks >> 2, c = 2 * (ks & 3) + hi;
          return *reinterpret_cast<const u32x4*>(wb + kt * 8192 + ((c ^ sw1) << 4));
        };
#pragma unroll
        for (int ks = 0; ks < DEPTH; ++ks) wf[ks] = rd(ks);
#pragma unroll
        for (int ks = 0; ks < 20; ++ks) {
          if (ks + DEPTH < 20) wf[(ks + DEPTH) % (DEPTH + 1)] = rd(ks + DEPTH);
          if (PF && ks == 14) {
#pragma unroll
            for (int q = 0; q < 2; ++q) {
              cv[q] = *reinterpret_cast<const f32x4*>(cdp + 8 * q); cg[q] = *reinterpret_cast<const f32x4*>(cdp + 16 + 8 * q);
              dv[q] = *reinterpret_cast<const f32x4*>(cdp + 64 + 8 * q); dg[q] = *reinterpret_cast<const f32x4*>(cdp + 80 + 8 * q);
            }
          }
          acc1 = Elem<DT>::mfma32(wf[ks % (DEPTH + 1)], xf[ks], acc1);
          if (SK && (ks & 1) && (ks >> 1) < 9) {
            if (late) issue_piece(ks >> 1, jn, (g + 1) & 1);
          }
        }
      }
      MTR(3)
      if (!PF) {
#pragma unroll
        for (int q = 0; q < 2; ++q) {
          cv[q] = *reinterpret_cast<const f32x4*>(cdp + 8 * q); cg[q] = *reinterpret_cast<const f32x4*>(cdp + 16 + 8 * q);
          dv[q] = *reinterpret_cast<const f32x4*>(cdp + 64 + 8 * q); dg[q] = *reinterpret_cast<const f32x4*>(cdp + 80 + 8 * q);
        }
      }
      u32x4 hmine;
      {
        float o[8];
#pragma unroll
        for (int q = 0; q < 2; ++q)
#pragma unroll
          for (int e = 0; e < 4; ++e) {
            const float val = fmaf(rstd, fmaf(nmu, cv[q][e], acc1[4 * q + e]), dv[q][e]);
            const float gat = fmaf(rstd, fmaf(nmu, cg[q][e], acc1[4 * (q + 2) + e]), dg[q][e]);
            o[4 * q + e] = val * gelu_erf_f(gat);
          }
        hmine = pack8<DT>(o);
      }
      *reinterpret_cast<u32x4*>(xch_mine) = hmine;
      const char* w2b = sl + w2_row;
      u32x4 w2f[2][5];
#pragma unroll
      for (int kk = 0; kk < 2; ++kk)
#pragma unroll
        for (int a = 0; a < 5; ++a) w2f[kk][a] = *reinterpret_cast<const u32x4*>(w2b + a * 2048 + (((2 * (kk ^ wn) + hi) ^ sw2) << 4));
#pragma unroll
      for (int a = 0; a < 5; ++a) acc2[a] = Elem<DT>::mfma32(w2f[0][a], hmine, acc2[a]);
      asm volatile("s_waitcnt lgkmcnt(0)" ::: "memory");
      wait_w2(!last);
      MTR(4)
      __builtin_amdgcn_s_barrier();
      asm volatile("" ::: "memory");
      MTR(5)
      const u32x4 hpeer = *reinterpret_cast<const u32x4*>(xch_peer);
#pragma unroll
      for (int a = 0; a < 5; ++a) acc2[a] = Elem<DT>::mfma32(w2f[1][a], hpeer, acc2[a]);
      MTR(6)
    }

    const int sl_row = lane >> 2, sl_pc = lane & 3;
    auto stg_f = [](int row) { return ((((row >> 2) ^ (row >> 3)) & 1) << 1) | (((row >> 1) ^ (row >> 3) ^ (row >> 4)) & 1); };
    auto stg_at = [&](int row, int pc) { return reinterpret_cast<u32x4*>(stg + row * 64 + ((pc ^ stg_f(row)) << 4)); };
    const int m_base = tile * MLP_BM + wm * 32;
#pragma unroll
    for (int a = 0; a < 5; ++a) {
      const int n = 160 * wn + 32 * a;
#pragma unroll
      for (int i = 0; i < 2; ++i) {
        const int row = sl_row + 16 * i;
        *stg_at(row, sl_pc) = *reinterpret_cast<const u32x4*>(p.x + (size_t)(m_base + row) * p.ldx + n + sl_pc * 8);
      }
      float v[16];
#pragma unroll
      for (int e = 0; e < 4; ++e) {
        const auto s02 = __builtin_amdgcn_permlane32_swap(__float_as_uint(acc2[a][e]), __float_as_uint(acc2[a][8 + e]), false, false);
        const auto s13 = __builtin_amdgcn_permlane32_swap(__float_as_uint(acc2[a][4 + e]), __float_as_uint(acc2[a][12 + e]), false, false);
        v[e] = __uint_as_float(s02[0]); v[4 + e] = __uint_as_float(s02[1]);
        v[8 + e] = __uint_as_float(s13[0]); v[12 + e] = __uint_as_float(s13[1]);
      }
      const float* bp = p.b2 + n + 16 * hi;
#pragma unroll
      for (int jq = 0; jq < 4; ++jq) {
        const f32x4 bq = *reinterpret_cast<const f32x4*>(bp + 4 * jq);
#pragma unroll
        for (int e = 0; e < 4; ++e) v[4 * jq + e] += bq[e];
      }
      asm volatile("s_waitcnt lgkmcnt(0)" ::: "memory");
      float r[16];
      unpack8<DT>(*stg_at(l31, 2 * hi), r);
      unpack8<DT>(*stg_at(l31, 2 * hi + 1), r + 8);
#pragma unroll
      for (int jq = 0; jq < 16; ++jq) v[jq] = fmaf(gate, v[jq], r[jq]);
      asm volatile("" ::: "memory");
      *stg_at(l31, 2 * hi) = pack8<DT>(v);
      *stg_at(l31, 2 * hi + 1) = pack8<DT>(v + 8);
      asm volatile("s_waitcnt lgkmcnt(0)" ::: "memory");
#pragma unroll
      for (int i = 0; i < 2; ++i) {
        const int row = sl_row + 16 * i;
        *reinterpret_cast<u32x4*>(p.out + (size_t)(m_base + row) * p.ldo + n + sl_pc * 8) = *stg_at(row, sl_pc);
      }
    }
    MTR(7)
  }
  MTR_DUMP
}

template <int DT>
int launch_mlp320(const MlpParams& p, hipStream_t s) {
  void (*kern)(const MlpParams, const int) = mlp320_kernel<DT>;
  static std::atomic<unsigned long long> attr_done{0};
  if (const int e = idf_lds_optin(reinterpret_cast<const void*>(kern), MLP_SMEM, attr_done)) return e;
  int dev = 0, cus = 0;
  if (hipGetDevice(&dev) != hipSuccess || hipDeviceGetAttribute(&cus, hipDeviceAttributeMultiprocessorCount, dev) != hipSuccess || cus <= 0) cus = 256;
  const int tiles = p.M / MLP_BM;
  const int grid = tiles < cus ? tiles : cus;
  hipLaunchKernelGGL(kern, dim3(grid), dim3(512), MLP_SMEM, s, p, tiles);
  return idf_launch_status();
}


constexpr int MW_NAGPR = 240;
constexpr int MW_B2_OFF = 2 * SLOT_BYTES, MW_STG_OFF = MW_B2_OFF + MLP_C * 4, MW_SMEM = MW_STG_OFF + 4 * 2 * 2048;

struct MwCtx {
  unsigned w1a[4], w2a[2], cda;
  f32x2 nmu2, rstd2, k1, k2, k3, one2;
  float lo8, hi8;
  const char* w1src; const char* w2src; const char* cdsrc;
  unsigned w1_ustride, w2_tstride;
  unsigned w1_voff, w2_voff, cd_voff;
  const char* w1b[2]; const char* w2b[5]; const char* cdb;
  unsigned w1_vj, w2_vj, cd_vj;
  unsigned w1dst, w2dst, cddst;
  int wave;
#ifdef IDF_MLPW_TRACE
  mutable unsigned long long tr[12];
#endif
};

#ifdef IDF_MLPW_TRACE
__device__ unsigned long long idf_mlpw_trace_buf[4][12];
#define MW_TR_DECL unsigned long long trm[7];
#define MW_TR_MARK(i) asm volatile("s_memtime %0" : "=s"(trm[i]));
#define MW_TR_END { asm volatile("s_waitcnt lgkmcnt(0)" : "+s"(trm[0]), "+s"(trm[1]), "+s"(trm[2]), "+s"(trm[3]), "+s"(trm[4]), "+s"(trm[5]), "+s"(trm[6])); \
    for (int i = 0; i < 6; ++i) c.tr[i] += trm[i + 1] - trm[i]; c.tr[6] += 1; }
#else
#define MW_TR_DECL
#define MW_TR_MARK(i)
#define MW_TR_END
#endif

#define MW_TOP asm volatile("s_waitcnt vmcnt(0)\n\ts_barrier" ::: "memory");
#ifndef MLPW_STREAM_INC
#define MLPW_STREAM_INC "mlpw_stream.inc"
#endif
#include MLPW_STREAM_INC

template <int DT>
__global__ __launch_bounds__(256, 1) void mlp320w_kernel(const MlpParams p, const int tiles) {
  asm volatile("" ::: "a0", "a239");
  extern __shared__ __attribute__((aligned(128))) char smem[];
  const int tid = threadIdx.x;
  const int lane = tid & 63, wave = __builtin_amdgcn_readfirstlane(tid >> 6);
  const int l31 = lane & 31, hi = lane >> 5;
  const int G = gridDim.x;
  const unsigned smem_lds = lds_u32(smem);

  MwCtx c;
  c.wave = wave;
  c.k1 = f32x2{1.0142652e-3f, 1.0142652e-3f}; c.k2 = f32x2{-1.0677574e-1f, -1.0677574e-1f}; c.k3 = f32x2{-2.3011213f, -2.3011213f};
  c.one2 = f32x2{1.0f, 1.0f};
  c.lo8 = -8.0f; c.hi8 = 8.0f;
  asm volatile("" : "+v"(c.k1), "+v"(c.k2), "+v"(c.k3), "+v"(c.one2), "+v"(c.hi8));
  {
    const int row = 8 * wave + (lane >> 3);
    c.w1_voff = (unsigned)(row * p.ldw1 + (((lane & 7) ^ ((row >> 1) & 7)) << 3)) * 2u;
    const int row2 = 16 * wave + (lane >> 2);
    c.w2_voff = (unsigned)(row2 * p.ldw2 + (((lane & 3) ^ ((row2 >> 2) & 3)) << 3)) * 2u;
    c.cd_voff = (unsigned)((lane & 31) * 16);
    c.w1_ustride = (unsigned)(32 * p.ldw1 * 2);
    c.w2_tstride = (unsigned)(64 * p.ldw2 * 2);
  }
  const int sw1 = (l31 >> 1) & 7, sw2 = (l31 >> 2) & 3;
  unsigned w1o[4], w2o[2];
#pragma unroll
  for (int i = 0; i < 4; ++i) w1o[i] = smem_lds + (unsigned)(l31 * 128 + (((2 * i + hi) ^ sw1) << 4));
#pragma unroll
  for (int kk = 0; kk < 2; ++kk) w2o[kk] = smem_lds + (unsigned)(W1_BYTES + l31 * 64 + (((2 * kk + hi) ^ sw2) << 4));
  const unsigned cdo = smem_lds + (unsigned)(W1_BYTES + W2_BYTES + 16 * hi);
  const char* const w1g = reinterpret_cast<const char*>(p.w1);
  const char* const w2g = reinterpret_cast<const char*>(p.w2p);
  const char* const cdg = reinterpret_cast<const char*>(p.cd);
  const unsigned w1_chunk = (unsigned)(64 * p.ldw1 * 2);
#pragma unroll
  for (int u = 0; u < 2; ++u) c.w1b[u] = w1g + (size_t)u * c.w1_ustride;
#pragma unroll
  for (int t = 0; t < 5; ++t) c.w2b[t] = w2g + (size_t)t * c.w2_tstride;
  c.cdb = cdg;

  auto set_iter = [&](int j) {
    const unsigned sj = (unsigned)((j & 1) * SLOT_BYTES), sn = (unsigned)(((j + 1) & 1) * SLOT_BYTES);
#pragma unroll
    for (int i = 0; i < 4; ++i) c.w1a[i] = w1o[i] + sn;
#pragma unroll
    for (int kk = 0; kk < 2; ++kk) c.w2a[kk] = w2o[kk] + sn;
    c.cda = cdo + sj;
    const int j2 = j + 2 >= MLP_NCH ? j + 2 - MLP_NCH : j + 2, j1 = j + 1 >= MLP_NCH ? j + 1 - MLP_NCH : j + 1;
    c.w1src = w1g + (size_t)j2 * w1_chunk;
    c.w2src = w2g + (size_t)j * 64;
    c.cdsrc = cdg + (size_t)j1 * 512;
    c.w1_vj = c.w1_voff + (unsigned)j2 * w1_chunk; c.w2_vj = c.w2_voff + (unsigned)j * 64u; c.cd_vj = c.cd_voff + (unsigned)j1 * 512u;
    c.w1dst = smem_lds + sj + (unsigned)(wave * 1024);
    c.w2dst = smem_lds + sj + (unsigned)(W1_BYTES + wave * 1024);
    c.cddst = smem_lds + sn + (unsigned)(W1_BYTES + W2_BYTES);
  };

  int tile = ((G & 7) == 0) ? (int)(blockIdx.x & 7) * (G >> 3) + (int)(blockIdx.x >> 3) : (int)blockIdx.x;
  if (tile >= tiles) return;
  const float gate = p.gate ? p.gate[0] : 1.0f;

  {
#pragma unroll
    for (int ch = 0; ch < 2; ++ch)
#pragma unroll
      for (int kt = 0; kt < 5; ++kt)
#pragma unroll
        for (int u = 0; u < 2; ++u)
          mlp_dma16(w1g + (size_t)ch * w1_chunk + u * c.w1_ustride + kt * 128, c.w1_voff,
                    smem_lds + (unsigned)(ch * SLOT_BYTES + wave * 1024 + kt * 8192 + u * 4096));
    if (wave == 3) mlp_dma16(cdg, c.cd_voff, smem_lds + (unsigned)(W1_BYTES + W2_BYTES));
  }

  f32x16 acc1[2][2];
  u32x4 hh[2][2];
  if (tid < MLP_C / 4) reinterpret_cast<f32x4*>(smem + MW_B2_OFF)[tid] = reinterpret_cast<const f32x4*>(p.b2)[tid];
#ifdef IDF_MLPW_TRACE
  for (int i = 0; i < 12; ++i) c.tr[i] = 0;
  unsigned long long trt = __builtin_readcyclecounter();
#define MW_TRT(i) { const unsigned long long now = __builtin_readcyclecounter(); c.tr[i] += now - trt; trt = now; }
#else
#define MW_TRT(i)
#endif
  auto row_ptr = [&](int t) { return p.x + (size_t)(t * MLP_BM + wave * 32 + l31) * p.ldx + 8 * hi; };
  {
    const unsigned short* xr = row_ptr(tile);
    mw_static_for<20>([&](auto kc) { mw_load_x<decltype(kc)::value>(xr); });
  }
  f32x2 st = *reinterpret_cast<const f32x2*>(p.ln_stats + 2 * (size_t)(tile * MLP_BM + wave * 32 + l31));
  asm volatile("" : "+v"(st));
  bool first = true;
  for (;;) {
    c.nmu2 = f32x2{-st[0], -st[0]};
    c.rstd2 = f32x2{st[1], st[1]};
    asm volatile("" : "+v"(c.nmu2), "+v"(c.rstd2));
    mw_static_for<160>([&](auto rc) { mw_agpr_write<MW_OA + decltype(rc)::value>(0u); });
    if (first) {
      asm volatile("s_waitcnt vmcnt(0)" ::: "memory");
      __builtin_amdgcn_s_barrier();
      first = false;
    } else {
#ifdef MW_DIRECT_STORES
      asm volatile("s_waitcnt vmcnt(2)" ::: "memory");
#else
      asm volatile("s_waitcnt vmcnt(4)" ::: "memory");
#endif
    }
    asm volatile("" ::: "memory");

    MW_TRT(7)
    set_iter(-1);
    mw_pro<DT>(acc1[1], acc1[0], hh[1], hh[0], c);
    set_iter(0);
    mw_body_01<DT>(acc1[0], acc1[1], hh[1], hh[0], c);
    MW_TRT(9)
    for (int j = 1; j < MLP_NCH - 1; j += 2) {
      set_iter(j);
      mw_body_11<DT>(acc1[1], acc1[0], hh[0], hh[1], c);
      set_iter(j + 1);
      mw_body_11<DT>(acc1[0], acc1[1], hh[1], hh[0], c);
    }
    MW_TRT(10)
    set_iter(MLP_NCH - 1);
    mw_body_10<DT>(acc1[1], acc1[0], hh[0], hh[1], c);
    set_iter(MLP_NCH);
    mw_drain<DT>(acc1[0], acc1[1], hh[1], hh[0], c);
    asm volatile("s_nop 15\n\ts_nop 15\n\ts_nop 7" ::: "memory");
    MW_TRT(9)

    const int next = tile + G;
    const bool has_next = next < tiles;
    const unsigned short* const xn = row_ptr(has_next ? next : tile);
    if (has_next) st = *reinterpret_cast<const f32x2*>(p.ln_stats + 2 * (size_t)(next * MLP_BM + wave * 32 + l31));
#ifdef MW_DIRECT_STORES
    unsigned short* const orow = p.out + (size_t)(tile * MLP_BM + wave * 32 + l31) * p.ldo + 16 * hi;
#else
    char* const stg = smem + MW_STG_OFF + wave * 4096;
    const int sl_row = lane >> 2, sl_pc = lane & 3;
    auto stg_f = [](int row) { return ((((row >> 2) ^ (row >> 3)) & 1) << 1) | (((row >> 1) ^ (row >> 3) ^ (row >> 4)) & 1); };
    auto stg_at = [&](int slot, int row, int pc) { return reinterpret_cast<u32x4*>(stg + slot * 2048 + row * 64 + ((pc ^ stg_f(row)) << 4)); };
    unsigned short* const orow = p.out + (size_t)(tile * MLP_BM + wave * 32 + sl_row) * p.ldo + sl_pc * 8;
    u32x4 po0, po1;
#endif
    const char* const b2l = smem + MW_B2_OFF + 64 * hi;
    mw_static_for<10>([&](auto ac) {
      constexpr int a = decltype(ac)::value;
      if constexpr (a == 9) asm volatile("" : "+v"(st));
      float acc[16];
      mw_static_for<16>([&](auto rc) { acc[decltype(rc)::value] = __uint_as_float(mw_agpr_read<MW_OA + 16 * a + decltype(rc)::value>()); });
      float v[16];
#pragma unroll
      for (int e = 0; e < 4; ++e) {
        const auto s02 = __builtin_amdgcn_permlane32_swap(__float_as_uint(acc[e]), __float_as_uint(acc[8 + e]), false, false);
        const auto s13 = __builtin_amdgcn_permlane32_swap(__float_as_uint(acc[4 + e]), __float_as_uint(acc[12 + e]), false, false);
        v[e] = __uint_as_float(s02[0]); v[4 + e] = __uint_as_float(s02[1]);
        v[8 + e] = __uint_as_float(s13[0]); v[12 + e] = __uint_as_float(s13[1]);
      }
#pragma unroll
      for (int jq = 0; jq < 4; ++jq) {
        const f32x4 bq = *reinterpret_cast<const f32x4*>(b2l + (32 * a + 4 * jq) * 4);
#pragma unroll
        for (int e = 0; e < 4; ++e) v[4 * jq + e] += bq[e];
      }
      u32x4 r0, r1;
      mw_static_for<4>([&](auto dc) {
        constexpr int d = decltype(dc)::value;
        const unsigned xa = mw_agpr_read<MW_XA + 4 * (2 * a) + d>(), xb = mw_agpr_read<MW_XA + 4 * (2 * a + 1) + d>();
        const auto sw = __builtin_amdgcn_permlane32_swap(xa, xb, false, false);
        r0[d] = sw[0]; r1[d] = sw[1];
      });
#ifndef MW_NO_XLOAD
      if (has_next) { mw_load_x<2 * a>(xn); mw_load_x<2 * a + 1>(xn); }
#endif
      float r[16];
      unpack8<DT>(r0, r);
      unpack8<DT>(r1, r + 8);
#pragma unroll
      for (int jq = 0; jq < 16; ++jq) v[jq] = fmaf(gate, v[jq], r[jq]);
#ifdef MW_DIRECT_STORES
      *reinterpret_cast<u32x4*>(orow + 32 * a) = pack8<DT>(v);
      *reinterpret_cast<u32x4*>(orow + 32 * a + 8) = pack8<DT>(v + 8);
#else
      if constexpr (a > 0) {
        *reinterpret_cast<u32x4*>(orow + 32 * (a - 1)) = po0;
        *reinterpret_cast<u32x4*>(orow + (size_t)16 * p.ldo + 32 * (a - 1)) = po1;
      }
      *stg_at(a & 1, l31, 2 * hi) = pack8<DT>(v);
      *stg_at(a & 1, l31, 2 * hi + 1) = pack8<DT>(v + 8);
      asm volatile("" ::: "memory");
      po0 = *stg_at(a & 1, sl_row, sl_pc); po1 = *stg_at(a & 1, sl_row + 16, sl_pc);
      if constexpr (a == 9) {
        *reinterpret_cast<u32x4*>(orow + 32 * a) = po0;
        *reinterpret_cast<u32x4*>(orow + (size_t)16 * p.ldo + 32 * a) = po1;
      }
#endif
    });
    MW_TRT(8)
    if (!has_next) break;
    tile = next;
  }
#ifdef IDF_MLPW_TRACE
  if ((int)blockIdx.x == (int)gridDim.x / 2 && lane == 0) { for (int i = 0; i < 12; ++i) idf_mlpw_trace_buf[wave][i] = c.tr[i]; }
#endif
}

template <int DT>
int launch_mlp320w(const MlpParams& p, hipStream_t s) {
  void (*kern)(const MlpParams, const int) = mlp320w_kernel<DT>;
  static std::atomic<unsigned long long> attr_done{0};
  if (const int e = idf_lds_optin(reinterpret_cast<const void*>(kern), MW_SMEM, attr_done)) return e;
  int dev = 0, cus = 0;
  if (hipGetDevice(&dev) != hipSuccess || hipDeviceGetAttribute(&cus, hipDeviceAttributeMultiprocessorCount, dev) != hipSuccess || cus <= 0) cus = 256;
  const int tiles = p.M / MLP_BM;
  const int grid = tiles < cus ? tiles : cus;
  hipLaunchKernelGGL(kern, dim3(grid), dim3(256), MW_SMEM, s, p, tiles);
  return idf_launch_status();
}

#ifndef IDF_MLP_MODE_DEFAULT
#define IDF_MLP_MODE_DEFAULT 1
#endif
int g_mlp_mode = -1;
inline int mlp_mode() {
  if (g_mlp_mode < 0) { const char* e = getenv("IDF_MLP_MODE"); g_mlp_mode = e ? (e[0] == '0' ? 0 : 1) : IDF_MLP_MODE_DEFAULT; }
  return g_mlp_mode;
}

}

int idf_mlp_set_mode(int v) {
  const int prev = mlp_mode();
  g_mlp_mode = v;
  return prev;
}

#ifdef IDF_MLPW_TRACE
extern "C" int idf_mlpw_trace_read(unsigned long long* host ) {
  return (int)hipMemcpyFromSymbol(host, HIP_SYMBOL(idf_mlpw_trace_buf), sizeof(idf_mlpw_trace_buf));
}
#endif

#ifdef IDF_MLP_TRACE
extern "C" int idf_mlp_trace_read(unsigned long long* host ) {
  return (int)hipMemcpyFromSymbol(host, HIP_SYMBOL(idf_mlp_trace_buf), sizeof(idf_mlp_trace_buf));
}
#endif

extern "C" int idf_mlp_geglu(const idf_mlp_args* a, void* stream) {
  if (!a) return IDF_E_ARG;
  if (!a->x || !a->ln_stats || !a->w1 || !a->cd || !a->w2p || !a->b2 || !a->out) return IDF_E_ARG;
  if (a->M <= 0 || a->C <= 0) return IDF_E_ARG;
  if (a->dtype != IDF_BF16 && a->dtype != IDF_F16) return IDF_E_ARG;
  if (a->C != MLP_C || (a->M % MLP_BM) != 0) return IDF_E_UNSUPPORTED;
  if (a->ldx < MLP_C || a->ldo < MLP_C || a->ldw1 < MLP_C || a->ldw2 < MLP_H) return IDF_E_ARG;
  if ((a->ldx % 8) || (a->ldo % 8) || (a->ldw1 % 8) || (a->ldw2 % 8)) return IDF_E_ALIGN;
  if (!aligned16(a->x) || !aligned16(a->out) || !aligned16(a->w1) || !aligned16(a->w2p) || !aligned16(a->cd) || !aligned16(a->b2) ||
      (((uintptr_t)a->ln_stats) & 7u))
    return IDF_E_ALIGN;
  if ((long long)64 * a->ldw1 * 2 >= (1ll << 31) || (long long)320 * a->ldw2 * 2 >= (1ll << 31)) return IDF_E_UNSUPPORTED;
  MlpParams p;
  p.x = static_cast<const unsigned short*>(a->x); p.ldx = a->ldx; p.ln_stats = a->ln_stats;
  p.w1 = static_cast<const unsigned short*>(a->w1); p.ldw1 = a->ldw1; p.cd = a->cd;
  p.w2p = static_cast<const unsigned short*>(a->w2p); p.ldw2 = a->ldw2; p.b2 = a->b2; p.gate = a->gate;
  p.out = static_cast<unsigned short*>(a->out); p.ldo = a->ldo; p.M = a->M;
  hipStream_t s = static_cast<hipStream_t>(stream);
  if (mlp_mode() == 1) return a->dtype == IDF_BF16 ? launch_mlp320w<IDF_BF16>(p, s) : launch_mlp320w<IDF_F16>(p, s);
  return a->dtype == IDF_BF16 ? launch_mlp320<IDF_BF16>(p, s) : launch_mlp320<IDF_F16>(p, s);
}
```

instancediffusion_amd/csrc/mw_prims.h:

```cpp
#pragma once
#include "gemm_core.h"
#include <type_traits>
#include <utility>

namespace idfmw {
using namespace idfcore;

constexpr int MW_XA = 0;
constexpr int MW_OA = 80;

__device__ __forceinline__ unsigned lds_u32(const void* p) { return (unsigned)(size_t)p; }

template <int R> __device__ __forceinline__ void mw_agpr_write(unsigned v) { asm volatile("v_accvgpr_write_b32 a%c1, %0" ::"v"(v), "n"(R)); }
template <int R> __device__ __forceinline__ unsigned mw_agpr_read() {
  unsigned v;
  asm volatile("v_accvgpr_read_b32 %0, a%c1" : "=v"(v) : "n"(R));
  return v;
}
template <class F, int... I>
__device__ __forceinline__ void mw_static_for_impl(F&& f, std::integer_sequence<int, I...>) { (f(std::integral_constant<int, I>{}), ...); }
template <int N, class F>
__device__ __forceinline__ void mw_static_for(F&& f) { mw_static_for_impl(f, std::make_integer_sequence<int, N>{}); }

template <int DT, int KS, bool FIRST> __device__ __forceinline__ void mw_mf1(f32x16& acc, const u32x4& w) {
  constexpr int lo = MW_XA + 4 * KS;
  if constexpr (FIRST) {
    if constexpr (DT == IDF_BF16) asm volatile("v_mfma_f32_32x32x16_bf16 %0, %1, a[%c2:%c3], 0" : "=&v"(acc) : "v"(w), "n"(lo), "n"(lo + 3));
    else asm volatile("v_mfma_f32_32x32x16_f16 %0, %1, a[%c2:%c3], 0" : "=&v"(acc) : "v"(w), "n"(lo), "n"(lo + 3));
  } else {
    if constexpr (DT == IDF_BF16) asm volatile("v_mfma_f32_32x32x16_bf16 %0, %1, a[%c2:%c3], %0" : "+v"(acc) : "v"(w), "n"(lo), "n"(lo + 3));
    else asm volatile("v_mfma_f32_32x32x16_f16 %0, %1, a[%c2:%c3], %0" : "+v"(acc) : "v"(w), "n"(lo), "n"(lo + 3));
  }
}
template <int DT, int A> __device__ __forceinline__ void mw_mf2(const u32x4& w, const u32x4& h) {
  constexpr int lo = MW_OA + 16 * A;
  if constexpr (DT == IDF_BF16) asm volatile("v_mfma_f32_32x32x16_bf16 a[%c2:%c3], %0, %1, a[%c2:%c3]" ::"v"(w), "v"(h), "n"(lo), "n"(lo + 15));
  else asm volatile("v_mfma_f32_32x32x16_f16 a[%c2:%c3], %0, %1, a[%c2:%c3]" ::"v"(w), "v"(h), "n"(lo), "n"(lo + 15));
}
template <int OFF> __device__ __forceinline__ u32x4 mw_lds128(unsigned addr) {
  u32x4 r;
  asm volatile("ds_read_b128 %0, %1 offset:%c2" : "=v"(r) : "v"(addr), "n"(OFF));
  return r;
}
template <int OFF> __device__ __forceinline__ f32x4 mw_lds128f(unsigned addr) {
  f32x4 r;
  asm volatile("ds_read_b128 %0, %1 offset:%c2" : "=v"(r) : "v"(addr), "n"(OFF));
  return r;
}
template <int N> __device__ __forceinline__ void mw_wait_lgkm() { asm volatile("s_waitcnt lgkmcnt(%c0)" ::"n"(N)); }
#ifdef MW_PACKED_VALU
__device__ __forceinline__ f32x2 mw_pk_fma(f32x2 a, f32x2 b, f32x2 c) {
  f32x2 d;
  asm volatile("v_pk_fma_f32 %0, %1, %2, %3" : "=v"(d) : "v"(a), "v"(b), "v"(c));
  return d;
}
__device__ __forceinline__ f32x2 mw_pk_mul(f32x2 a, f32x2 b) {
  f32x2 d;
  asm volatile("v_pk_mul_f32 %0, %1, %2" : "=v"(d) : "v"(a), "v"(b));
  return d;
}
__device__ __forceinline__ f32x2 mw_pk_add(f32x2 a, f32x2 b) {
  f32x2 d;
  asm volatile("v_pk_add_f32 %0, %1, %2" : "=v"(d) : "v"(a), "v"(b));
  return d;
}
#else
__device__ __forceinline__ f32x2 mw_pk_fma(f32x2 a, f32x2 b, f32x2 c) {
  float x, y;
  asm volatile("v_fma_f32 %0, %1, %2, %3" : "=v"(x) : "v"(a.x), "v"(b.x), "v"(c.x));
  asm volatile("v_fma_f32 %0, %1, %2, %3" : "=v"(y) : "v"(a.y), "v"(b.y), "v"(c.y));
  return f32x2{x, y};
}
__device__ __forceinline__ f32x2 mw_pk_mul(f32x2 a, f32x2 b) {
  float x, y;
  asm volatile("v_mul_f32_e32 %0, %1, %2" : "=v"(x) : "v"(a.x), "v"(b.x));
  asm volatile("v_mul_f32_e32 %0, %1, %2" : "=v"(y) : "v"(a.y), "v"(b.y));
  return f32x2{x, y};
}
__device__ __forceinline__ f32x2 mw_pk_add(f32x2 a, f32x2 b) {
  float x, y;
  asm volatile("v_add_f32_e32 %0, %1, %2" : "=v"(x) : "v"(a.x), "v"(b.x));
  asm volatile("v_add_f32_e32 %0, %1, %2" : "=v"(y) : "v"(a.y), "v"(b.y));
  return f32x2{x, y};
}
#endif
__device__ __forceinline__ float mw_med3(float x, float lo , float hi) {
  float d;
  asm volatile("v_med3_f32 %0, %1, %2, %3" : "=v"(d) : "v"(x), "s"(lo), "v"(hi));
  return d;
}
__device__ __forceinline__ float mw_exp2(float x) {
  float d;
  asm volatile("v_exp_f32_e32 %0, %1" : "=v"(d) : "v"(x));
  return d;
}
__device__ __forceinline__ float mw_rcp(float x) {
  float d;
  asm volatile("v_rcp_f32_e32 %0, %1" : "=v"(d) : "v"(x));
  return d;
}
template <int DT> __device__ __forceinline__ unsigned mw_cvt_pk(float lo, float hi) {
  unsigned r;
  if constexpr (DT == IDF_BF16) asm volatile("v_cvt_pk_bf16_f32 %0, %1, %2" : "=v"(r) : "v"(lo), "v"(hi));
  else asm volatile("v_cvt_pk_f16_f32 %0, %1, %2" : "=v"(r) : "v"(lo), "v"(hi));
  return r;
}
template <int H> __device__ __forceinline__ f32x2 mw_half(const f32x4& v) { return __builtin_shufflevector(v, v, 2 * H, 2 * H + 1); }
template <int I> __device__ __forceinline__ f32x2 mw_pair(const f32x16& v) { return __builtin_shufflevector(v, v, I, I + 1); }
template <int KS> __device__ __forceinline__ void mw_load_x(const unsigned short* rowp) {
  asm volatile("global_load_dwordx4 a[%c1:%c2], %0, off offset:%c3" ::"v"(rowp), "n"(MW_XA + 4 * KS), "n"(MW_XA + 4 * KS + 3), "n"(32 * KS) : "memory");
}

template <int LDSOFF, int SRCOFF> __device__ __forceinline__ void mw_dma(unsigned ldsbase , unsigned voff, const void* sbase ) {
  constexpr int L = LDSOFF - SRCOFF;
  asm volatile("s_add_i32 m0, %0, %c1\n\ts_nop 0\n\tglobal_load_lds_dwordx4 %2, %3 offset:%c4" ::"s"(ldsbase), "n"(L), "v"(voff), "s"(sbase), "n"(SRCOFF) : "memory", "scc");
}


template <int KA, int KO> __device__ __forceinline__ void mw_load_x2(const unsigned short* rowp) {
  asm volatile("global_load_dwordx4 a[%c1:%c2], %0, off offset:%c3" ::"v"(rowp), "n"(MW_XA + 4 * KA), "n"(MW_XA + 4 * KA + 3), "n"(32 * KO) : "memory");
}

template <int DT, int KS, bool FIRST> __device__ __forceinline__ void mw_mf1t(f32x16& acc, const u32x4& w) {
  constexpr int lo = MW_XA + 4 * KS;
  if constexpr (FIRST) {
    if constexpr (DT == IDF_BF16) asm volatile("v_mfma_f32_32x32x16_bf16 %0, a[%c2:%c3], %1, 0" : "=&v"(acc) : "v"(w), "n"(lo), "n"(lo + 3));
    else asm volatile("v_mfma_f32_32x32x16_f16 %0, a[%c2:%c3], %1, 0" : "=&v"(acc) : "v"(w), "n"(lo), "n"(lo + 3));
  } else {
    if constexpr (DT == IDF_BF16) asm volatile("v_mfma_f32_32x32x16_bf16 %0, a[%c2:%c3], %1, %0" : "+v"(acc) : "v"(w), "n"(lo), "n"(lo + 3));
    else asm volatile("v_mfma_f32_32x32x16_f16 %0, a[%c2:%c3], %1, %0" : "+v"(acc) : "v"(w), "n"(lo), "n"(lo + 3));
  }
}
__device__ __forceinline__ float mw_fma(float a, float b, float c) {
  float d;
  asm volatile("v_fma_f32 %0, %1, %2, %3" : "=v"(d) : "v"(a), "v"(b), "v"(c));
  return d;
}
__device__ __forceinline__ float mw_add(float a, float b) {
  float d;
  asm volatile("v_add_f32_e32 %0, %1, %2" : "=v"(d) : "v"(a), "v"(b));
  return d;
}
__device__ __forceinline__ float mw_mul(float a, float b) {
  float d;
  asm volatile("v_mul_f32_e32 %0, %1, %2" : "=v"(d) : "v"(a), "v"(b));
  return d;
}
template <int OFF> __device__ __forceinline__ float mw_lds32f(unsigned addr) {
  float r;
  asm volatile("ds_read_b32 %0, %1 offset:%c2" : "=v"(r) : "v"(addr), "n"(OFF));
  return r;
}
template <int OFF> __device__ __forceinline__ void mw_lds_write64(unsigned addr, unsigned lo, unsigned hi) {
  typedef unsigned u32x2_t __attribute__((ext_vector_type(2)));
  const u32x2_t v = {lo, hi};
  asm volatile("ds_write_b64 %0, %1 offset:%c2" ::"v"(addr), "v"(v), "n"(OFF) : "memory");
}
template <int OFF> __device__ __forceinline__ void mw_lds_write128(unsigned addr, const u32x4& v) {
  asm volatile("ds_write_b128 %0, %1 offset:%c2" ::"v"(addr), "v"(v), "n"(OFF) : "memory");
}
__device__ __forceinline__ void mw_swap32(unsigned& x, unsigned& y) { asm volatile("v_permlane32_swap_b32 %0, %1" : "+v"(x), "+v"(y)); }
__device__ __forceinline__ void mw_store128(unsigned voff, const u32x4& v, const void* sbase) {
  asm volatile("global_store_dwordx4 %0, %1, %2" ::"v"(voff), "v"(v), "s"(sbase) : "memory");
}
__device__ __forceinline__ void mw_dma_rt(const void* sbase , unsigned voff, unsigned lds) {
  lds = __builtin_amdgcn_readfirstlane(lds);
  asm volatile("s_mov_b32 m0, %0\n\ts_nop 0\n\tglobal_load_lds_dwordx4 %1, %2" ::"s"(lds), "v"(voff), "s"(sbase) : "memory");
}
template <int N> __device__ __forceinline__ void mw_wait_vm_barrier() { asm volatile("s_waitcnt vmcnt(%c0)\n\ts_barrier" ::"n"(N) : "memory"); }

}
```

instancediffusion_amd/engine.py:

```python
from __future__ import annotations

import os
from typing import Dict, List, Optional, Sequence, Tuple

import torch

from .host.attention import SpatialTransformer
from .host.unet import Downsample, ResBlock, UNetModel, Upsample

LN_SELF_MODE = int(os.environ.get("IDF_LN_SELF", "1"))
if LN_SELF_MODE not in (0, 1, 2):
    raise ValueError(f"IDF_LN_SELF={LN_SELF_MODE}: must be 0, 1 or 2")
QKV_ROW = os.environ.get("IDF_QKV_ROW", "1") != "0"
OBJ_TOKENS = 184
MASK_RES = 64


def _round_up(x: int, m: int) -> int:
    return (x + m - 1) // m * m


GEGLU_PERIOD = int(os.environ.get("IDF_GEGLU_PERIOD", "32"))
if GEGLU_PERIOD not in (32, 64):
    raise ValueError(f"IDF_GEGLU_PERIOD={GEGLU_PERIOD}: must be 32 or 64")
MLP_FUSED = os.environ.get("IDF_MLP_FUSED", "1")
if MLP_FUSED not in ("0", "1"):
    raise ValueError(f"IDF_MLP_FUSED={MLP_FUSED}: must be 0 or 1")
MLP_FUSED = MLP_FUSED == "1" and GEGLU_PERIOD == 32
MLP_MIN_M = int(os.environ.get("IDF_MLP_MIN_M", "32768"))
PAIR_HOIST = os.environ.get("IDF_PAIR_HOIST", "1")
if PAIR_HOIST not in ("0", "1"):
    raise ValueError(f"IDF_PAIR_HOIST={PAIR_HOIST}: must be 0 or 1")
PAIR_HOIST = PAIR_HOIST == "1"
GN_EPI = os.environ.get("IDF_GN_EPI", "1")
if GN_EPI not in ("0", "1"):
    raise ValueError(f"IDF_GN_EPI={GN_EPI}: must be 0 or 1")
GN_EPI = GN_EPI == "1"
DEBUG_PAIRED = os.environ.get("IDF_DEBUG_PAIRED", "0") == "1"


def pack_geglu(w: torch.Tensor, b: torch.Tensor, period: int = 64) -> Tuple[torch.Tensor, torch.Tensor]:
    n2, k = w.shape
    n = n2 // 2
    h = period // 2
    assert n % h == 0
    wv, wg = w[:n].reshape(n // h, h, k), w[n:].reshape(n // h, h, k)
    bv, bg = b[:n].reshape(n // h, h), b[n:].reshape(n // h, h)
    return torch.cat([wv, wg], dim=1).reshape(n2, k).contiguous(), torch.cat([bv, bg], dim=1).reshape(n2).contiguous()


def pack_conv3x3(w: torch.Tensor) -> torch.Tensor:
    co, ci = w.shape[0], w.shape[1]
    return w.permute(0, 2, 3, 1).reshape(co, 9 * ci).contiguous()


class _Lin:
    __slots__ = ("w", "b")

    def __init__(self, w, b):
        self.w, self.b = w, b


class Cond:

    _next_uid = 0

    def __init__(self, B: int):
        Cond._next_uid += 1
        self.uid = Cond._next_uid
        self.B = B
        self.objs: Optional[torch.Tensor] = None
        self.k_ctx: List[torch.Tensor] = []
        self.vt_ctx: List[torch.Tensor] = []
        self.k_obj: List[torch.Tensor] = []
        self.vt_obj: List[torch.Tensor] = []
        self.n_ctx = 0
        self.vis: List[torch.Tensor] = []

    @staticmethod
    def cat(conds: Sequence["Cond"]) -> "Cond":
        out = Cond(sum(c.B for c in conds))
        out.n_ctx = conds[0].n_ctx
        out.objs = torch.cat([c.objs for c in conds], 0)
        for name in ("k_ctx", "vt_ctx", "k_obj", "vt_obj", "vis"):
            lists = [getattr(c, name) for c in conds]
            setattr(out, name, [torch.cat(ts, 0) for ts in zip(*lists)])
        return out

    def _tensors(self):
        return [self.objs] + self.k_ctx + self.vt_ctx + self.k_obj + self.vt_obj + self.vis

    def clone(self) -> "Cond":
        out = Cond(self.B)
        out.n_ctx = self.n_ctx
        out.objs = self.objs.clone()
        for name in ("k_ctx", "vt_ctx", "k_obj", "vt_obj", "vis"):
            setattr(out, name, [t.clone() for t in getattr(self, name)])
        return out

    def copy_from(self, other: "Cond"):
        for dst, src in zip(self._tensors(), other._tensors()):
            dst.copy_(src)

    def same_layout(self, other: "Cond") -> bool:
        a, b = self._tensors(), other._tensors()
        return len(a) == len(b) and all(x.shape == y.shape for x, y in zip(a, b)) and self.n_ctx == other.n_ctx

    def select(self, idx: torch.Tensor) -> "Cond":
        out = Cond(int(idx.numel()))
        out.n_ctx = self.n_ctx
        out.objs = self.objs[idx].contiguous()
        for name in ("k_ctx", "vt_ctx", "k_obj", "vt_obj", "vis"):
            setattr(out, name, [t[idx].contiguous() for t in getattr(self, name)])
        return out


class UNetEngine:
    def __init__(self, model: UNetModel, ops=None, dtype: torch.dtype = torch.bfloat16, use_graphs: bool = True):
        if ops is None:
            from .ops import HipOps
            ops = HipOps(dtype)
        self.ops = ops
        self.dtype = ops.dtype
        self.device = ops.device
        self.model = model
        self.heads = model.num_heads
        self.masked_fuser = not getattr(model, "efficient_attention", True)
        self.vt_global = os.environ.get("IDF_VT_GLOBAL", "1") != "0"
        self.vt_min_n = int(os.environ.get("IDF_VT_MIN_N", "256"))
        if self.vt_min_n < 64 or self.vt_min_n % 64:
            raise ValueError(f"IDF_VT_MIN_N={self.vt_min_n}: a positive multiple of 64 (tokens per sample from which the fused "
                             "q | k | v launch is used; default 256)")
        self.use_graphs = use_graphs and self.device.type == "cuda"
        self._bufs: Dict[tuple, torch.Tensor] = {}
        self._graphs: Dict[tuple, tuple] = {}
        self._paired_checked: set = set()
        self._cond_cache: Dict[tuple, Cond] = {}
        self._slots: Dict[int, Cond] = {}
        self._slot_bound: Dict[int, int] = {}
        self.fuser_scale = None
        self._pack(model)
        self.set_fuser_scale(1.0)

    def _w16(self, t: torch.Tensor) -> torch.Tensor:
        return t.detach().to(device=self.device, dtype=torch.float32).to(self.dtype).contiguous()

    def _f32(self, t: torch.Tensor) -> torch.Tensor:
        return t.detach().to(device=self.device, dtype=torch.float32).contiguous()

    def _lin(self, m, with_bias=True) -> _Lin:
        w = m.weight
        if w.dim() == 4:
            w = w.reshape(w.shape[0], w.shape[1])
        return _Lin(self._w16(w), self._f32(m.bias) if (with_bias and m.bias is not None) else None)

    def _conv(self, m) -> _Lin:
        return _Lin(self._w16(pack_conv3x3(m.weight.detach().float())), self._f32(m.bias))

    def _fold_ln(self, w: torch.Tensor, bias, norm):
        w = w.detach().float()
        g, b = norm.weight.detach().float(), norm.bias.detach().float()
        w16 = self._w16(w * g[None, :])
        d = w @ b + (bias.detach().float() if bias is not None else 0.0)
        return w16, w16.float().sum(1).contiguous(), self._f32(d)

    def _pack_ff(self, ff, norm):
        w = ff.net[0].proj.weight.detach().float()
        g, b = norm.weight.detach().float(), norm.bias.detach().float()
        wp, dp = pack_geglu(w * g[None, :], ff.net[0].proj.bias.detach().float() + w @ b, GEGLU_PERIOD)
        w16 = self._w16(wp)
        f = dict(w1=w16, b1=self._f32(dp), c1=w16.float().sum(1).contiguous(), l2=self._lin(ff.net[2]))
        C = w.shape[1]
        if MLP_FUSED and hasattr(self.ops, "mlp_geglu") and self.ops.mlp_supported(128, C):
            f["cd"], f["w2p"] = self.ops.mlp_pack(w16, f["c1"], f["b1"], f["l2"].w)
        return f

    def _attn(self, a, norm, self_attn: bool):
        d = dict(out=self._lin(a.to_out[0]))
        if self_attn:
            w3, c3, d3 = self._fold_ln(torch.cat([a.to_q.weight.detach(), a.to_k.weight.detach(), a.to_v.weight.detach()], 0),
                                       None, norm)
            C2 = 2 * a.to_q.weight.shape[0]
            d["wqkv"], d["cqkv"], d["dqkv"] = w3, c3, d3
            d["wqk"], d["cqk"], d["dqk"] = w3[:C2], c3[:C2], d3[:C2]
            d["wv"], d["cv"], d["dv"] = w3[C2:], c3[C2:], d3[C2:]
        else:
            d["wq"], d["cq"], d["dq"] = self._fold_ln(a.to_q.weight, None, norm)
            d["wk"], d["wv"] = self._w16(a.to_k.weight), self._w16(a.to_v.weight)
        return d

    def _attn_kv_plain(self, a):
        return dict(wk=self._w16(a.to_k.weight), wv=self._w16(a.to_v.weight))

    def _pack_res(self, rb: ResBlock, emb_w: list, emb_b: list, off: list):
        p = dict(kind="res", cin=rb.channels, cout=rb.out_channels,
                 gn1=(self._f32(rb.in_layers[0].weight), self._f32(rb.in_layers[0].bias)),
                 conv1=self._conv(rb.in_layers[2]),
                 gn2=(self._f32(rb.out_layers[0].weight), self._f32(rb.out_layers[0].bias)),
                 conv2=self._conv(rb.out_layers[3]),
                 skip=None if isinstance(rb.skip_connection, torch.nn.Identity) else self._lin(rb.skip_connection),
                 emb_off=off[0])
        emb_w.append(rb.emb_layers[1].weight.detach().float())
        emb_b.append(rb.emb_layers[1].bias.detach().float())
        off[0] += rb.out_channels
        return p

    def _pack_st(self, st: SpatialTransformer, tanh_alphas: list):
        blk = st.transformer_blocks[0]
        fz = blk.fuser
        idx = len(tanh_alphas)
        tanh_alphas.append(torch.stack([torch.tanh(fz.alpha_attn.detach().float()),
                                        torch.tanh(fz.alpha_dense.detach().float())]))
        return dict(kind="st", c=st.in_channels, idx=idx,
                    norm=(self._f32(st.norm.weight), self._f32(st.norm.bias)),
                    proj_in=self._lin(st.proj_in), proj_out=self._lin(st.proj_out),
                    n1=(self._f32(blk.norm1.weight), self._f32(blk.norm1.bias)),
                    n2=(self._f32(blk.norm2.weight), self._f32(blk.norm2.bias)),
                    n3=(self._f32(blk.norm3.weight), self._f32(blk.norm3.bias)),
                    attn1=self._attn(blk.attn1, blk.norm1, True), attn2=self._attn(blk.attn2, blk.norm2, False),
                    ff=self._pack_ff(blk.ff, blk.norm3),
                    f_lin=self._lin(fz.linear), f_attn=self._attn(fz.attn, fz.norm1, True), f_kv=self._attn_kv_plain(fz.attn),
                    f_ff=self._pack_ff(fz.ff, fz.norm2),
                    f_n1=(self._f32(fz.norm1.weight), self._f32(fz.norm1.bias)),
                    f_n2=(self._f32(fz.norm2.weight), self._f32(fz.norm2.bias)))

    def _pack_layers(self, seq, emb_w, emb_b, off, tanh_alphas):
        out = []
        for _, layer in seq.items():
            if isinstance(layer, ResBlock):
                out.append(self._pack_res(layer, emb_w, emb_b, off))
            elif isinstance(layer, SpatialTransformer):
                out.append(self._pack_st(layer, tanh_alphas))
            elif isinstance(layer, Downsample):
                out.append(dict(kind="down", conv=self._conv(layer.op)))
            elif isinstance(layer, Upsample):
                out.append(dict(kind="up", conv=self._conv(layer.conv)))
            else:
                out.append(dict(kind="conv_in", w=self._f32(layer.weight), b=self._f32(layer.bias)))
        return out

    def _pack(self, model: UNetModel):
        emb_w, emb_b, off, tanh_alphas = [], [], [0], []
        self.te0 = self._lin(model.time_embed[0])
        self.te2 = self._lin(model.time_embed[2])
        self.in_blocks = [self._pack_layers(b, emb_w, emb_b, off, tanh_alphas) for b in model.input_blocks]
        self.mid_block = self._pack_layers(model.middle_block, emb_w, emb_b, off, tanh_alphas)
        self.out_blocks = [self._pack_layers(b, emb_w, emb_b, off, tanh_alphas) for b in model.output_blocks]
        self.emb_all = _Lin(self._w16(torch.cat(emb_w, 0)), self._f32(torch.cat(emb_b, 0)))
        self.emb_total = off[0]
        self.tanh_alphas = torch.stack(tanh_alphas).to(self.device)
        self.gates = torch.zeros_like(self.tanh_alphas)
        self.n_st = len(tanh_alphas)
        self.scaleu = []
        for i in range(len(model.output_blocks)):
            b = getattr(model, f"scaleu_b_{i}").detach().float()
            s = getattr(model, f"scaleu_s_{i}").detach().float()
            self.scaleu.append((self._f32(torch.tanh(b) + 1.0), self._f32(torch.tanh(s))))
        self.out_gn = (self._f32(model.out[0].weight), self._f32(model.out[0].bias))
        oc = model.out[2]
        wpad = torch.zeros(64, oc.weight.shape[1], 3, 3)
        wpad[: oc.weight.shape[0]] = oc.weight.detach().float().cpu()
        bpad = torch.zeros(64)
        bpad[: oc.bias.shape[0]] = oc.bias.detach().float().cpu()
        self.out_conv = _Lin(self._w16(pack_conv3x3(wpad)), self._f32(bpad))
        self.n_out = oc.weight.shape[0]
        self._pack_tokenizer(model.position_net)

    def repack_first_conv(self, conv):
        p = self.in_blocks[0][0]
        p["w"].copy_(conv.weight.detach().float())
        p["b"].copy_(conv.bias.detach().float())

    def _pack_tokenizer(self, pn):
        self.pn = pn
        self.tok_mlps = []
        for i in range(5):
            seq = pn.linears_list[i]
            self.tok_mlps.append([self._lin(seq[0]), self._lin(seq[2]), self._lin(seq[4])])
        self.tok_null = dict(
            text=self._f32(pn.null_positive_feature), box=self._f32(pn.null_position_feature),
            point=self._f32(pn.null_point_feature), scribble=self._f32(pn.null_scribble_feature),
            polygon=self._f32(pn.null_polygon_feature), seg=self._f32(pn.null_seg_feature))
        self.tok_pos = self._f32(pn.pos_embedding)
        self.tok_freqs = (100.0 ** (torch.arange(16) / 16)).to(device=self.device, dtype=torch.float32)
        self._pack_convnext(pn)

    def _pack_convnext(self, pn):
        bb = pn.convnext_tiny_backbone
        cn = dict(in_w=self._f32(pn.in_conv.weight), in_b=self._f32(pn.in_conv.bias), stages=[], down=[])
        stem = bb.downsample_layers[0]
        w = stem[0].weight.detach().float().reshape(stem[0].weight.shape[0], -1)
        wp = torch.zeros(w.shape[0], 64)
        wp[:, :w.shape[1]] = w
        cn["stem"] = _Lin(self._w16(wp), self._f32(stem[0].bias))
        cn["stem_ln"] = (self._f32(stem[1].weight), self._f32(stem[1].bias))
        for i in range(1, 4):
            dl = bb.downsample_layers[i]
            wd = dl[1].weight.detach().float()
            cn["down"].append(dict(ln=(self._f32(dl[0].weight), self._f32(dl[0].bias)),
                                   conv=_Lin(self._w16(wd.permute(0, 2, 3, 1).reshape(wd.shape[0], -1)),
                                             self._f32(dl[1].bias))))
        for i in range(4):
            blocks = []
            for _, blk in bb.stages[i].items():
                C = blk.dwconv.weight.shape[0]
                kpad = _round_up(C, 64)
                w1 = torch.zeros(4 * C, kpad)
                w1[:, :C] = blk.pwconv1.weight.detach().float()
                g = blk.gamma.detach().float()
                blocks.append(dict(
                    C=C, kpad=kpad,
                    dw_w=self._f32(blk.dwconv.weight.detach().float().reshape(C, 49).t().contiguous()),
                    dw_b=self._f32(blk.dwconv.bias), ln=(self._f32(blk.norm.weight), self._f32(blk.norm.bias)),
                    l1=_Lin(self._w16(w1), self._f32(blk.pwconv1.bias)),
                    l2=_Lin(self._w16(g[:, None] * blk.pwconv2.weight.detach().float()),
                            self._f32(g * blk.pwconv2.bias.detach().float()))))
            cn["stages"].append(blocks)
        self.cn = cn
        t = torch.arange(64)
        i = torch.arange(3072)
        self.seg_gather = (((i[None, :] % 4) * 4 + t[:, None] // 16) * 16 + (t[:, None] % 16)) * 768 + i[None, :] // 4
        self.seg_gather = self.seg_gather.to(self.device)

    def convnext_features(self, segs: torch.Tensor) -> torch.Tensor:
        ops, cn = self.ops, self.cn
        B, Cin, S, _ = segs.shape
        P = S // 4
        pm = ops.zeros((B * P * P, 64))
        ops.seg_in_conv(segs.contiguous(), cn["in_w"], cn["in_b"], pm)
        x = ops.gemm(pm, cn["stem"].w, ops.empty((B * P * P, cn["stem"].w.shape[0])), bias=cn["stem"].b)
        C = x.shape[1]
        x = ops.layernorm(x, ops.empty(x.shape), cn["stem_ln"][0], cn["stem_ln"][1], 1e-6).view(B, P, P, C)
        H = P
        for i in range(4):
            if i > 0:
                d = cn["down"][i - 1]
                pmat = ops.layernorm_patch2(x, ops.empty((B * (H // 2) * (H // 2), 4 * C)), d["ln"][0], d["ln"][1], 1e-6)
                H //= 2
                Cn = d["conv"].w.shape[0]
                x = ops.gemm(pmat, d["conv"].w, ops.empty((B * H * H, Cn)), bias=d["conv"].b).view(B, H, H, Cn)
                C = Cn
            M = B * H * H
            for blk in cn["stages"][i]:
                y = ops.dwconv7x7(x, blk["dw_w"], blk["dw_b"], ops.empty(x.shape))
                ln = ops.zeros((M, blk["kpad"])) if blk["kpad"] != C else ops.empty((M, C))
                ops.layernorm(y.view(M, C), ln[:, :C], blk["ln"][0], blk["ln"][1], 1e-6)
                hmid = ops.gemm(ln, blk["l1"].w, ops.empty((M, 4 * C)), bias=blk["l1"].b, act="gelu")
                ops.gemm(hmid, blk["l2"].w, x.view(M, C), bias=blk["l2"].b, res=x.view(M, C))
        return x

    def set_fuser_scale(self, scale: float):
        scale = float(scale)
        if scale != self.fuser_scale:
            self.fuser_scale = scale
            self.gates.copy_(self.tanh_alphas * scale)

    def sync_fuser_scale_from_modules(self):
        from .host.attention import GatedSelfAttentionDense
        for m in self.model.modules():
            if type(m) == GatedSelfAttentionDense:
                self.set_fuser_scale(m.scale)
                return

    def buf(self, role: str, shape, dtype=None, zero=False) -> torch.Tensor:
        dtype = dtype or self.dtype
        key = (role, tuple(int(s) for s in shape), dtype)
        t = self._bufs.get(key)
        if t is None:
            t = (self.ops.zeros if zero else self.ops.empty)(key[1], dtype)
            self._bufs[key] = t
        return t

    def tokens(self, g: Dict[str, torch.Tensor]) -> torch.Tensor:
        ops, pn = self.ops, self.pn
        dev = self.device
        boxes = g["boxes"].to(dev, torch.float32)
        B, N, _ = boxes.shape
        m = g["masks"].to(dev, torch.float32).reshape(B * N)
        text = g["positive_embeddings"].to(dev, torch.float32).reshape(B * N, -1).contiguous()
        points = g.get("points")
        points = ((boxes[..., :2] + boxes[..., 2:]) / 2.0) if points is None else points.to(dev, torch.float32)
        scribbles = g["scribbles"].to(dev, torch.float32)
        polygons = g["polygons"].to(dev, torch.float32)
        drop_point, drop_box, drop_scribble, drop_polygons, drop_segs = pn.eval_drops()
        zero = torch.zeros_like(m)
        masks = [
            zero if drop_box else m,
            zero if drop_point else m,
            zero if drop_scribble else ((scribbles.sum(-1).reshape(-1) + m) > 0).float(),
            zero if drop_polygons else ((polygons.sum(-1).reshape(-1) + m) > 0).float(),
        ]
        locs = [boxes.reshape(B * N, 4), points.reshape(B * N, 2), scribbles.reshape(B * N, -1),
                polygons.reshape(B * N, -1)]
        nulls = [self.tok_null["box"], self.tok_null["point"], self.tok_null["scribble"], self.tok_null["polygon"]]
        objs = ops.zeros((B, OBJ_TOKENS, pn.out_dim))
        for i in range(4):
            loc = locs[i].contiguous()
            inp = ops.empty((B * N, text.shape[1] + 32 * loc.shape[1]))
            ops.unifusion_embed(text, loc, m.contiguous(), masks[i].contiguous(), self.tok_null["text"], nulls[i],
                                self.tok_freqs, inp)
            l0, l1, l2 = self.tok_mlps[i]
            h0 = ops.gemm(inp, l0.w, ops.empty((B * N, l0.w.shape[0])), bias=l0.b, act="silu")
            h1 = ops.gemm(h0, l1.w, ops.empty((B * N, l1.w.shape[0])), bias=l1.b, act="silu")
            ops.gemm(h1.view(B, N, -1), l2.w, objs[:, i * N:(i + 1) * N, :], bias=l2.b)
        segs = g["segs"]
        if segs.dim() == 4 and segs.shape[0] > 1 and segs.stride(0) == 0:
            segs = segs[:1]
        Bs = segs.shape[0]
        use_segs = (not drop_segs) and bool((segs.reshape(Bs, -1).sum(1) > 0).any())
        l0, l1, l2 = self.tok_mlps[4]
        null_in = self.tok_null["seg"].view(1, 1, -1) + self.tok_pos
        if use_segs:
            segs_r = segs.to(dev, torch.float32)
            if segs_r.shape[-1] != pn.resize_input:
                segs_r = torch.nn.functional.interpolate(segs_r, pn.resize_input, mode="nearest")
            feat = self.convnext_features(segs_r)
            sf = feat.reshape(Bs, -1).float()[:, self.seg_gather.reshape(-1)].reshape(Bs, 64, -1)
            sm = (segs_r.reshape(Bs, -1).sum(1) > 0).float().view(Bs, 1, 1)
            seg_in = sf * sm + (1 - sm) * self.tok_null["seg"].view(1, 1, -1) + self.tok_pos
            rows = Bs * 64
        else:
            seg_in, rows = null_in, 64
        seg_in = seg_in.reshape(rows, -1).contiguous()
        seg16 = ops.cast16(seg_in, ops.empty(seg_in.shape))
        h0 = ops.gemm(seg16, l0.w, ops.empty((rows, l0.w.shape[0])), bias=l0.b, act="silu")
        h1 = ops.gemm(h0, l1.w, ops.empty((rows, l1.w.shape[0])), bias=l1.b, act="silu")
        seg_tok = ops.gemm(h1, l2.w, ops.empty((rows, l2.w.shape[0])), bias=l2.b)
        objs[:, 4 * N:, :] = seg_tok.view(-1, 64, seg_tok.shape[-1])
        return objs

    def _st_layers(self):
        for blk in self.in_blocks + [self.mid_block] + self.out_blocks:
            for p in blk:
                if p["kind"] == "st":
                    yield p

    def prepare_cond(self, context: torch.Tensor, grounding: Dict[str, torch.Tensor]) -> Cond:
        ops = self.ops
        B, n_ctx, cd = context.shape
        c = Cond(B)
        c.n_ctx = n_ctx
        c.objs = self.tokens(grounding)
        if self.masked_fuser:
            from .host.attention import visibility_words
            am = grounding.get("att_masks")
            any_flag = grounding.get("att_masks_any")
            if am is None or self.pn.drop_box_mask or any_flag is False:
                am = torch.zeros(B, 1, MASK_RES, MASK_RES, device=self.device)
            assert am.shape[-2:] == (MASK_RES, MASK_RES), "the reference masks at the 64x64 resolution only"
            am = am.to(self.device)
            if am.shape[0] != B:
                am = am.expand(B, *am.shape[1:])
            n_objs = (OBJ_TOKENS - 64) // 4
            if am.shape[1] < n_objs:
                am = torch.cat([am, torch.zeros(B, n_objs - am.shape[1], MASK_RES, MASK_RES, device=self.device)], 1)
            c.vis = list(visibility_words(am, force_masked=bool(any_flag) and not self.pn.drop_box_mask))
        ctx16 = ops.cast16(context.to(self.device, torch.float32).contiguous(), ops.empty((B, n_ctx, cd)))
        ld_ctx, ld_obj = _round_up(n_ctx, 64), _round_up(OBJ_TOKENS, 64)
        for p in self._st_layers():
            C = p["c"]
            a2, fa = p["attn2"], p["f_kv"]
            k = ops.gemm(ctx16.view(B * n_ctx, cd), a2["wk"], ops.empty((B * n_ctx, C))).view(B, n_ctx, C)
            vt = ops.zeros((B, C, ld_ctx))
            ops.gemm(a2["wv"], ctx16, vt[:, :, :n_ctx])
            c.k_ctx.append(k)
            c.vt_ctx.append(vt)
            o = ops.gemm(c.objs.view(B * OBJ_TOKENS, -1), p["f_lin"].w, ops.empty((B * OBJ_TOKENS, C)), bias=p["f_lin"].b)
            ln = ops.layernorm(o, ops.empty((B * OBJ_TOKENS, C)), *p["f_n1"])
            ko = ops.gemm(ln, fa["wk"], ops.empty((B * OBJ_TOKENS, C))).view(B, OBJ_TOKENS, C)
            vo = ops.zeros((B, C, ld_obj))
            ops.gemm(fa["wv"], ln.view(B, OBJ_TOKENS, C), vo[:, :, :OBJ_TOKENS])
            c.k_obj.append(ko)
            c.vt_obj.append(vo)
        return c

    def _gnp(self, role, B, HW, C):
        shape = self.ops.gn_partial_shape(B, HW, C) if (GN_EPI and hasattr(self.ops, "gn_partial_shape")) else None
        return None if shape is None else self.buf(role, shape, torch.float32)

    def _res(self, p, x, emb_all, out_role, gnp=None, want_out=True):
        ops = self.ops
        B, H, W, Cin = x.shape
        Cout = p["cout"]
        g = ops.groupnorm(x, self.buf("gn", x.shape), p["gn1"][0], p["gn1"][1], 1e-5, True, partial=gnp)
        rb = emb_all[:, p["emb_off"]:p["emb_off"] + Cout]
        p1 = self._gnp("gnp.h1", B, H * W, Cout)
        h1 = ops.conv3x3(g, p["conv1"].w, self.buf("rb.h1", (B, H, W, Cout)), bias=p["conv1"].b, rowbias=rb, gn_partial=p1)
        g2 = ops.groupnorm(h1, self.buf("gn", h1.shape), p["gn2"][0], p["gn2"][1], 1e-5, True, partial=p1)
        if p["skip"] is not None:
            xs = ops.gemm(x.view(B * H * W, Cin), p["skip"].w, self.buf("rb.skip", (B * H * W, Cout)),
                          bias=p["skip"].b).view(B, H, W, Cout)
        else:
            xs = x
        p2 = self._gnp("gnp.out", B, H * W, Cout) if want_out else None
        return ops.conv3x3(g2, p["conv2"].w, self.buf(out_role, (B, H, W, Cout)), bias=p["conv2"].b, res=xs, gn_partial=p2), p2

    def _self_attn(self, a, y, st, B, N, C, kv_extra=None, vis=None):
        ops = self.ops
        fused = self.vt_global and N % 64 == 0 and N >= self.vt_min_n
        if fused:
            vtg = self.buf("st.vtg", (C, B * N))
            own = self._qkv_self(C, N)
            qk = ops.gemm(y, a["wqkv"], self.buf("st.qk", (B * N, 2 * C)), bias=a["dqkv"],
                          ln_row=(None if own else st, a["cqkv"]), ln_stats_out=st if own else None,
                          vt_out=vtg).view(B, N, 2 * C)
            vt = vtg.view(C, B, N).permute(1, 0, 2)
        else:
            if self._ln_self(C):
                qk = ops.gemm(y, a["wqk"], self.buf("st.qk", (B * N, 2 * C)), bias=a["dqk"], ln_row=(None, a["cqk"]),
                              ln_stats_out=st).view(B, N, 2 * C)
            else:
                qk = ops.gemm(y, a["wqk"], self.buf("st.qk", (B * N, 2 * C)), bias=a["dqk"], ln_row=(st, a["cqk"])).view(B, N, 2 * C)
            ldv = _round_up(N, 64)
            vt = self.buf("st.vt", (B, C, ldv), zero=True)
            ops.gemm(a["wv"], y.view(B, N, C), vt[:, :, :N], ln_col=(st.view(B, N, 2), a["cv"], a["dv"]))
        att = self.buf("st.att", (B, N, C))
        if kv_extra is None:
            ops.attention(qk[:, :, :C], qk[:, :, C:], vt, N, att, self.heads)
        elif vis is None:
            ops.attention(qk[:, :, :C], qk[:, :, C:], vt, N, att, self.heads, k1=kv_extra[0], vt1=kv_extra[1],
                          n1=OBJ_TOKENS)
        else:
            ops.attention(qk[:, :, :C], qk[:, :, C:], vt, N, att, self.heads, k1=kv_extra[0], vt1=kv_extra[1],
                          n1=OBJ_TOKENS, qbits=vis[0], kbits0=vis[1], kbits1=vis[2])
        return att

    def _qkv_self(self, C, N):
        return self._ln_self(C) and not (QKV_ROW and C == 320 and self.vt_global and N % 64 == 0 and N >= self.vt_min_n)

    @staticmethod
    def _ln_self(C):
        return LN_SELF_MODE == 2 or (LN_SELF_MODE == 1 and C <= 320)

    def _ff(self, f, y, st, M, C, gate=None, out_stats=None):
        ops = self.ops
        if "w2p" in f and st is not None and LN_SELF_MODE != 2 and out_stats is None and M >= MLP_MIN_M and ops.mlp_supported(M, C):
            return ops.mlp_geglu(y, st, f["w1"], f["cd"], f["w2p"], f["l2"].b, y, gate=gate)
        mid = ops.gemm(y, f["w1"], self.buf("st.ffmid", (M, 4 * C)), bias=f["b1"], geglu=True, geglu_period=GEGLU_PERIOD,
                       ln_row=(None if LN_SELF_MODE == 2 else st, f["c1"]))
        return ops.gemm(mid, f["l2"].w, y, bias=f["l2"].b, res=y, gate=gate, out_stats=out_stats)

    def _dup(self, t: torch.Tensor, role: str) -> torch.Tensor:
        n = t.shape[0]
        out = self.buf(role, (2 * n,) + tuple(t.shape[1:]), t.dtype)
        out[:n].copy_(t)
        out[n:].copy_(t)
        return out

    def _st(self, p, x, cond: Cond, fuser_on: bool, dup: bool = False, gnp=None):
        ops = self.ops
        B, H, W, C = x.shape
        N, M = H * W, B * H * W
        g = ops.groupnorm(x, self.buf("gn", x.shape), p["norm"][0], p["norm"][1], 1e-6, False, partial=gnp)
        st = self.buf("st.stats", (M, 2), torch.float32)
        own = self._ln_self(C)
        own_qkv = self._qkv_self(C, N)
        pre, ffs = (None if own else st), (st if LN_SELF_MODE <= 1 else None)
        pqkv = None if own_qkv else st
        y = ops.gemm(g.view(M, C), p["proj_in"].w, self.buf("st.x", (M, C)), bias=p["proj_in"].b, out_stats=pqkv)
        att = self._self_attn(p["attn1"], y, st, B, N, C)
        ops.gemm(att.view(M, C), p["attn1"]["out"].w, y, bias=p["attn1"]["out"].b, res=y,
                 out_stats=pqkv if fuser_on else pre)
        if dup:
            x, y = self._dup(x, "st.x_in2"), self._dup(y.view(B, N, C), "st.x2").view(2 * M, C)
            if (pqkv if fuser_on else pre) is not None:
                st = self._dup(st.view(B, N, 2), "st.stats2").view(2 * M, 2)
                pre = st if pre is not None else None
                pqkv = st if pqkv is not None else None
                ffs = st if ffs is not None else None
            else:
                st = self.buf("st.stats", (2 * M, 2), torch.float32)
                ffs = st if ffs is not None else None
            B, M = 2 * B, 2 * M
        i = p["idx"]
        if fuser_on:
            vis = cond.vis if (cond.vis and N == MASK_RES * MASK_RES) else None
            att = self._self_attn(p["f_attn"], y, st, B, N, C, kv_extra=(cond.k_obj[i], cond.vt_obj[i]), vis=vis)
            ops.gemm(att.view(M, C), p["f_attn"]["out"].w, y, bias=p["f_attn"]["out"].b, res=y, gate=self.gates[i, 0:1],
                     out_stats=ffs)
            self._ff(p["f_ff"], y, st, M, C, gate=self.gates[i, 1:2], out_stats=pre)
        a2 = p["attn2"]
        q = ops.gemm(y, a2["wq"], self.buf("st.q", (M, C)), bias=a2["dq"],
                     ln_row=(None if own else st, a2["cq"])).view(B, N, C)
        att = self.buf("st.att", (B, N, C))
        ops.attention(q, cond.k_ctx[i], cond.vt_ctx[i], cond.n_ctx, att, self.heads)
        ops.gemm(att.view(M, C), a2["out"].w, y, bias=a2["out"].b, res=y, out_stats=ffs)
        self._ff(p["ff"], y, st, M, C)
        ops.gemm(y, p["proj_out"].w, x.view(M, C), bias=p["proj_out"].b, res=x.view(M, C))
        return x

    def _run_block(self, layers, h, x_nchw, emb_all, cond, fuser_on, out_role, dup_st: bool = False, gnp=None, next_kind=None):
        for j, p in enumerate(layers):
            k = p["kind"]
            nxt = layers[j + 1]["kind"] if j + 1 < len(layers) else next_kind
            norm_next = nxt in ("res", "st")
            if k == "conv_in":
                B, _, H, W = x_nchw.shape
                h = self.ops.conv_in(x_nchw, p["w"], p["b"], self.buf(out_role, (B, H, W, p["w"].shape[0])))
                gnp = None
            elif k == "res":
                h, gnp = self._res(p, h, emb_all, out_role, gnp, want_out=norm_next)
            elif k == "st":
                h = self._st(p, h, cond, fuser_on, dup=dup_st, gnp=gnp)
                gnp = None
            elif k == "down":
                B, H, W, C = h.shape
                Ho, Wo = (H + 1) // 2, (W + 1) // 2
                gnp = self._gnp("gnp.out", B, Ho * Wo, C) if norm_next else None
                h = self.ops.conv3x3(h, p["conv"].w, self.buf(out_role, (B, Ho, Wo, C)), bias=p["conv"].b, stride=2, gn_partial=gnp)
            elif k == "up":
                B, H, W, C = h.shape
                h = self.ops.conv3x3(h, p["conv"].w, self.buf(out_role + ".up", (B, 2 * H, 2 * W, C)),
                                     bias=p["conv"].b, upsample=1)
                gnp = None
        return h, gnp

    def _forward_ops(self, x: torch.Tensor, t_f32: torch.Tensor, cond: Cond, eps: torch.Tensor, fuser_on: bool,
                     paired: bool = False):
        ops = self.ops
        B = x.shape[0]
        hoist = (paired and PAIR_HOIST and B % 2 == 0 and len(self.in_blocks) > 1
                 and [p["kind"] for p in self.in_blocks[0]] == ["conv_in"] and [p["kind"] for p in self.in_blocks[1]] == ["res", "st"])
        n = B // 2
        mc = self.model.model_channels
        te = ops.timestep_embedding(t_f32, self.buf("temb.sin", (B, mc)))
        e1 = ops.gemm(te, self.te0.w, self.buf("temb.1", (B, 4 * mc)), bias=self.te0.b, act="silu")
        es = ops.gemm(e1, self.te2.w, self.buf("temb.2", (B, 4 * mc)), bias=self.te2.b, act="silu")
        emb_all = ops.gemm(es, self.emb_all.w, self.buf("temb.all", (B, self.emb_total)), bias=self.emb_all.b)
        hs = []
        h, gnp = None, None
        for i, layers in enumerate(self.in_blocks):
            nk = (self.in_blocks[i + 1] if i + 1 < len(self.in_blocks) else self.mid_block)[0]["kind"]
            if hoist and i == 0:
                h, gnp = self._run_block(layers, h, x[:n], emb_all[:n], cond, fuser_on, "in0.half")
                hs.append(self._dup(h, "in0"))
                continue
            if hoist and i == 1:
                h, gnp = self._run_block(layers, h, x[:n], emb_all[:n], cond, fuser_on, "in1.half", dup_st=True, gnp=gnp, next_kind=nk)
                hs.append(h)
                continue
            h, gnp = self._run_block(layers, h, x, emb_all, cond, fuser_on, f"in{i}", gnp=gnp, next_kind=nk)
            hs.append(h)
        h, gnp = self._run_block(self.mid_block, h, x, emb_all, cond, fuser_on, "mid", gnp=gnp)
        for i, layers in enumerate(self.out_blocks):
            skip = hs.pop()
            Bq, H, W, Ch = h.shape
            cat = ops.scaleu_concat(h, skip, self.buf("cat", (Bq, H, W, Ch + skip.shape[-1])), *self.scaleu[i])
            h, gnp = self._run_block(layers, cat, x, emb_all, cond, fuser_on, f"out{i}")
        g = ops.groupnorm(h, self.buf("gn", h.shape), self.out_gn[0], self.out_gn[1], 1e-5, True)
        ops.conv3x3(g, self.out_conv.w, eps, bias=self.out_conv.b, n_valid=self.n_out)
        return eps

    def _bind(self, cond: Cond) -> Cond:
        B = cond.B
        slot = self._slots.get(B)
        if slot is None or not slot.same_layout(cond):
            slot = cond.clone()
            self._slots[B] = slot
            self._slot_bound[B] = cond.uid
            for k in [k for k in self._graphs if k[0] == B]:
                del self._graphs[k]
        elif self._slot_bound[B] != cond.uid:
            slot.copy_from(cond)
            self._slot_bound[B] = cond.uid
        return slot

    def gather_cond(self, bank: Cond, idx: torch.Tensor) -> Cond:
        B = int(idx.numel())
        slot = self._slots.get(B)
        if slot is None or len(slot._tensors()) != len(bank._tensors()) or any(
                a.shape[1:] != b.shape[1:] for a, b in zip(slot._tensors(), bank._tensors())) or slot.n_ctx != bank.n_ctx:
            slot = bank.select(idx)
            self._slots[B] = slot
            for k in [k for k in self._graphs if k[0] == B]:
                del self._graphs[k]
        else:
            for dst, src in zip(slot._tensors(), bank._tensors()):
                torch.index_select(src, 0, idx, out=dst)
        self._slot_bound[B] = slot.uid
        return slot

    def forward_cond(self, x: torch.Tensor, t: torch.Tensor, cond: Cond, out: Optional[torch.Tensor] = None,
                     paired: bool = False) -> torch.Tensor:
        B = cond.B
        half = bool(paired) and x.shape[0] * 2 == B
        if not half:
            assert x.shape[0] == B
        _, Cx, H, W = x.shape
        fuser_on = self.fuser_scale != 0.0
        key = (B, H, W, fuser_on, bool(paired))
        if paired and not half and (DEBUG_PAIRED or key not in self._paired_checked):
            n = B // 2
            if B % 2 or not (torch.equal(x[:n], x[n:]) and torch.equal(t[:n], t[n:])):
                raise ValueError("forward_cond(paired=True): rows [B/2, B) must repeat the latent and timestep of rows [0, B/2)")
            self._paired_checked.add(key)
        x_s = self.buf("io.x", (B,) + tuple(x.shape[1:]), torch.float32)
        t_s = self.buf("io.t", (B,), torch.float32)
        eps_s = self.buf("io.eps", (B, self.n_out, H, W), torch.float32)
        if half:
            n = B // 2
            x_s[:n].copy_(x)
            x_s[n:].copy_(x)
            t_s[:n].copy_(t)
            t_s[n:].copy_(t)
        else:
            x_s.copy_(x)
            t_s.copy_(t)
        if not self.use_graphs:
            self._forward_ops(x_s, t_s, cond, eps_s, fuser_on, paired)
        else:
            slot = self._bind(cond)
            graph = self._graphs.get(key)
            if graph is None:
                self._forward_ops(x_s, t_s, slot, eps_s, fuser_on, paired)
                torch.cuda.synchronize()
                graph = torch.cuda.CUDAGraph()
                with torch.cuda.graph(graph):
                    self._forward_ops(x_s, t_s, slot, eps_s, fuser_on, paired)
                self._graphs[key] = graph
            graph.replay()
        if out is None:
            return eps_s.clone()
        out.copy_(eps_s)
        return out

    def forward(self, x, timesteps, context, grounding) -> torch.Tensor:
        self.sync_fuser_scale_from_modules()
        key = (context.data_ptr(), context._version, tuple(context.shape)) + tuple(
            (k, v.data_ptr(), v._version) for k, v in sorted(grounding.items()) if torch.is_tensor(v))
        cond = self._cond_cache.get(key)
        if cond is None:
            if len(self._cond_cache) > 64:
                self._cond_cache.clear()
            cond = self.prepare_cond(context, grounding)
            cond._keepalive = (context, grounding)
            self._cond_cache[key] = cond
        return self.forward_cond(x.to(self.device, torch.float32), timesteps.to(self.device), cond)
```

instancediffusion_amd/ops.py:

```python
from __future__ import annotations

import ctypes as C
from typing import Optional

import torch

from . import _lib
from ._lib import (EPI_BIAS, EPI_GATE, EPI_GEGLU, EPI_GEGLU_P32, EPI_GELU, EPI_LN_COL, EPI_LN_ROW, EPI_OUT_F32, EPI_OUT_NCHW,
                   EPI_RES, EPI_ROWBIAS, EPI_SILU)

_DT = {torch.bfloat16: _lib.IDF_BF16, torch.float16: _lib.IDF_F16}


def _p(t: Optional[torch.Tensor]):
    return None if t is None else C.c_void_p(t.data_ptr())


def _rows2d(t: torch.Tensor):
    assert t.stride(-1) == 1 or t.shape[-1] == 1, "last dim must be contiguous"
    return t.stride(-2), (t.stride(0) if t.dim() == 3 else 0)


class HipOps:

    def __init__(self, dtype: torch.dtype = torch.bfloat16, device: Optional[torch.device] = None):
        self.lib = _lib.load()
        if not torch.cuda.is_available():
            raise RuntimeError("no MI355X visible: the InstanceDiffusion HIP path needs a GPU (no CPU fallback)")
        self.dtype = dtype
        self.dt = _DT[dtype]
        self.device = device or torch.device("cuda", torch.cuda.current_device())
        self._ws = {}

    def _stream(self):
        return C.c_void_p(torch.cuda.current_stream().cuda_stream)

    def _workspace(self, key, nfloats: int) -> torch.Tensor:
        k = (key, int(nfloats))
        w = self._ws.get(k)
        if w is None:
            w = torch.empty(int(nfloats), dtype=torch.float32, device=self.device)
            self._ws[k] = w
        return w

    SPLITK_WS_BYTES = 256 << 20

    def _splitk_ws(self) -> torch.Tensor:
        return self._workspace("splitk", self.SPLITK_WS_BYTES // 4)

    def empty(self, shape, dtype=None):
        return torch.empty(shape, dtype=dtype or self.dtype, device=self.device)

    def zeros(self, shape, dtype=None):
        return torch.zeros(shape, dtype=dtype or self.dtype, device=self.device)

    def gemm(self, a, w, out, *, bias=None, rowbias=None, rows_per_batch=0, res=None, gate=None,
             act: Optional[str] = None, geglu: bool = False, geglu_period: int = 64, ln_row=None, ln_col=None, out_stats=None, out_stats_eps=1e-5,
             ln_eps=1e-5, ln_stats_out=None, vt_out=None):
        batched = out.dim() == 3
        M, K = a.shape[-2], a.shape[-1]
        N = w.shape[-2]
        assert w.shape[-1] == K
        lda, sA = _rows2d(a)
        ldw, sW = _rows2d(w)
        ldo, sO = _rows2d(out)
        epi = 0
        if bias is not None:
            epi |= EPI_BIAS
        if rowbias is not None:
            epi |= EPI_ROWBIAS
        ldr = sR = 0
        if res is not None:
            epi |= EPI_RES
            ldr, sR = _rows2d(res)
        if gate is not None:
            epi |= EPI_GATE
        if act == "silu":
            epi |= EPI_SILU
        elif act == "gelu":
            epi |= EPI_GELU
        elif act is not None:
            raise ValueError(act)
        if geglu:
            epi |= EPI_GEGLU
            assert geglu_period in (32, 64)
            if geglu_period == 32:
                epi |= EPI_GEGLU_P32
            assert out.shape[-1] == N // 2
        elif vt_out is not None:
            assert not batched and out.shape[-2] == M and vt_out.shape[0] == N - out.shape[-1] and vt_out.shape[1] >= M
            assert vt_out.stride(1) == 1 and vt_out.dtype == self.dtype
        else:
            assert out.shape[-1] == N and out.shape[-2] == M
        if out.dtype == torch.float32:
            epi |= EPI_OUT_F32
        ln_stats = ln_c = ln_d = None
        s_ln = 0
        if ln_row is not None:
            ln_stats, ln_c = ln_row
            assert bias is not None and ln_c.numel() == N
            assert ln_stats is None or (ln_stats.shape[-2] == M and ln_stats.dtype == torch.float32)
            if ln_stats is None:
                assert not batched
                if ln_stats_out is not None:
                    assert ln_stats_out.is_contiguous() and ln_stats_out.dtype == torch.float32 and ln_stats_out.numel() == 2 * M
            epi |= EPI_LN_ROW
        elif ln_col is not None:
            ln_stats, ln_c, ln_d = ln_col
            assert ln_stats.shape[-2] == N and ln_c.numel() == M and ln_d.numel() == M and ln_stats.dtype == torch.float32
            epi |= EPI_LN_COL
        if ln_stats is not None:
            assert ln_stats.is_contiguous() and ln_stats.shape[-1] == 2
            s_ln = ln_stats.stride(0) if (batched and ln_stats.dim() == 3) else 0
        if out_stats is not None:
            assert out_stats.is_contiguous() and out_stats.dtype == torch.float32 and out_stats.numel() == 2 * out.numel() // N
        args = _lib.GemmArgs(
            A=a.data_ptr(), W=w.data_ptr(), out=out.data_ptr(),
            bias=None if bias is None else bias.data_ptr(),
            rowbias=None if rowbias is None else rowbias.data_ptr(),
            res=None if res is None else res.data_ptr(),
            gate=None if gate is None else gate.data_ptr(),
            M=M, N=N, K=K, lda=lda, ldw=ldw, ldo=ldo, ldr=ldr,
            ld_rowbias=0 if rowbias is None else rowbias.stride(-2), rows_per_batch=rows_per_batch,
            batch=out.shape[0] if batched else 1, strideA=sA, strideW=sW, strideO=sO, strideR=sR,
            epi=epi, dtype=self.dt, ws=self._splitk_ws().data_ptr(), ws_bytes=self.SPLITK_WS_BYTES,
            ln_stats=None if ln_stats is None else ln_stats.data_ptr(), stride_ln_stats=s_ln,
            ln_c=None if ln_c is None else ln_c.data_ptr(), ln_d=None if ln_d is None else ln_d.data_ptr(),
            out_stats=None if out_stats is None else out_stats.data_ptr(), out_stats_eps=float(out_stats_eps),
            ln_eps=float(ln_eps), ln_stats_out=None if ln_stats_out is None else ln_stats_out.data_ptr(),
            vt_out=None if vt_out is None else vt_out.data_ptr(), ld_vt=0 if vt_out is None else vt_out.stride(0),
            vt_col0=0 if vt_out is None else out.shape[-1])
        _lib.check(self.lib.idf_gemm(C.byref(args), self._stream()), "idf_gemm")
        return out

    MLP_W2_PERM = (0, 1, 2, 3, 8, 9, 10, 11, 4, 5, 6, 7, 12, 13, 14, 15)

    @staticmethod
    def mlp_supported(M: int, C: int) -> bool:
        return C == 320 and M % 128 == 0

    @classmethod
    def mlp_pack(cls, w1p16, c1, d1, w2_16):
        n2 = c1.numel()
        cd = torch.cat([c1.float().view(n2 // 64, 64), d1.float().view(n2 // 64, 64)], dim=1).contiguous()
        perm = torch.tensor(cls.MLP_W2_PERM, device=w2_16.device)
        n, k = w2_16.shape
        w2p = w2_16.view(n, k // 16, 16).index_select(2, perm).reshape(n, k).contiguous()
        return cd, w2p

    def mlp_geglu(self, x, stats, w1, cd, w2p, b2, out, *, gate=None):
        M, Cc = x.shape
        assert self.mlp_supported(M, Cc) and out.shape == x.shape and x.stride(-1) == 1 and out.stride(-1) == 1
        assert stats.is_contiguous() and stats.dtype == torch.float32 and stats.numel() == 2 * M
        assert w1.shape == (8 * Cc, Cc) and w2p.shape == (Cc, 4 * Cc) and cd.is_contiguous() and cd.numel() == 16 * Cc
        assert w1.stride(-1) == 1 and w2p.stride(-1) == 1 and b2.dtype == torch.float32 and cd.dtype == torch.float32
        args = _lib.MlpArgs(x=x.data_ptr(), ldx=x.stride(0), ln_stats=stats.data_ptr(), w1=w1.data_ptr(), ldw1=w1.stride(0),
                            cd=cd.data_ptr(), w2p=w2p.data_ptr(), ldw2=w2p.stride(0), b2=b2.data_ptr(),
                            gate=None if gate is None else gate.data_ptr(), out=out.data_ptr(), ldo=out.stride(0), M=M, C=Cc,
                            dtype=self.dt)
        _lib.check(self.lib.idf_mlp_geglu(C.byref(args), self._stream()), "idf_mlp_geglu")
        return out

    @staticmethod
    def gn_partial_shape(B, HW, C):
        return (B, HW // 64, 32, 2) if (HW % 64 == 0 and C % 32 == 0) else None

    def conv3x3(self, x, w, out, *, bias=None, rowbias=None, res=None, stride=1, upsample=0, n_valid=0, gn_partial=None):
        B, H, W_, Cin = x.shape
        assert x.stride(-1) == 1 and x.stride(1) == W_ * x.stride(2) and x.stride(0) == H * x.stride(1)
        Cout = w.shape[0]
        epi = 0
        if bias is not None:
            epi |= EPI_BIAS
        if rowbias is not None:
            epi |= EPI_ROWBIAS
        if res is not None:
            epi |= EPI_RES
        if n_valid:
            epi |= EPI_OUT_NCHW
            assert out.dtype == torch.float32 and out.is_contiguous()
            ldo = 0
        else:
            ldo = out.stride(2)
        args = _lib.ConvArgs(
            x=x.data_ptr(), W=w.data_ptr(), out=out.data_ptr(),
            bias=None if bias is None else bias.data_ptr(),
            rowbias=None if rowbias is None else rowbias.data_ptr(),
            res=None if res is None else res.data_ptr(),
            B=B, Hin=H, Win=W_, Cin=Cin, Cout=Cout, stride=stride, upsample=upsample,
            ldx=x.stride(2), ldo=ldo, ldr=0 if res is None else res.stride(2),
            ld_rowbias=0 if rowbias is None else rowbias.stride(-2), n_valid=n_valid, epi=epi, dtype=self.dt,
            ws=self._splitk_ws().data_ptr(), ws_bytes=self.SPLITK_WS_BYTES,
            gn_partial=None if gn_partial is None else gn_partial.data_ptr())
        if gn_partial is not None:
            assert gn_partial.dtype == torch.float32 and gn_partial.is_contiguous() and out.is_contiguous()
            assert tuple(gn_partial.shape) == self.gn_partial_shape(out.shape[0], out.shape[1] * out.shape[2], Cout)
        _lib.check(self.lib.idf_conv3x3(C.byref(args), self._stream()), "idf_conv3x3")
        return out

    def conv_in(self, x_nchw, w, bias, out):
        B, Cin, H, W_ = x_nchw.shape
        assert x_nchw.dtype == torch.float32 and x_nchw.is_contiguous() and out.is_contiguous()
        _lib.check(self.lib.idf_conv_in(_p(x_nchw), _p(w), _p(bias), _p(out), B, Cin, H, W_, out.shape[-1], self.dt,
                                        self._stream()), "idf_conv_in")
        return out

    def attention(self, q, k0, vt0, n0, out, heads, *, k1=None, vt1=None, n1=0, qbits=None, kbits0=None, kbits1=None):
        if qbits is not None:
            for t in (qbits, kbits0) + ((kbits1,) if n1 else ()):
                assert t.dtype == torch.int32 and t.stride(-1) == 1 and t.dim() == 2
        B, Nq, Cc = q.shape
        d = Cc // heads
        a = _lib.AttnArgs(
            q=q.data_ptr(), ldq=q.stride(1), strideQ=q.stride(0), nq=Nq,
            k0=k0.data_ptr(), ldk0=k0.stride(1), strideK0=k0.stride(0),
            vt0=vt0.data_ptr(), ldv0=vt0.stride(1), strideV0=vt0.stride(0), n0=n0,
            k1=None if k1 is None else k1.data_ptr(), ldk1=0 if k1 is None else k1.stride(1),
            strideK1=0 if k1 is None else k1.stride(0),
            vt1=None if vt1 is None else vt1.data_ptr(), ldv1=0 if vt1 is None else vt1.stride(1),
            strideV1=0 if vt1 is None else vt1.stride(0), n1=n1,
            out=out.data_ptr(), ldo=out.stride(1), strideO=out.stride(0),
            B=B, H=heads, d=d, scale=float(d) ** -0.5, dtype=self.dt,
            qbits=None if qbits is None else qbits.data_ptr(), strideQb=0 if qbits is None else qbits.stride(0),
            kbits0=None if qbits is None else kbits0.data_ptr(), strideKb0=0 if qbits is None else kbits0.stride(0),
            kbits1=None if (qbits is None or not n1) else kbits1.data_ptr(),
            strideKb1=0 if (qbits is None or not n1) else kbits1.stride(0))
        _lib.check(self.lib.idf_attention(C.byref(a), self._stream()), "idf_attention")
        return out

    def groupnorm(self, x, out, gamma, beta, eps, silu, partial=None):
        assert x.is_contiguous() and out.is_contiguous()
        B, Cc = x.shape[0], x.shape[-1]
        HW = x.numel() // (B * Cc)
        if partial is not None:
            assert partial.dtype == torch.float32 and partial.is_contiguous() and partial.shape[0] == B and partial.shape[2:] == (32, 2)
            _lib.check(self.lib.idf_groupnorm_apply(_p(x), _p(out), _p(gamma), _p(beta), _p(partial), B, HW, Cc,
                                                    int(partial.shape[1]), float(eps), int(bool(silu)), self.dt,
                                                    self._stream()), "idf_groupnorm_apply")
            return out
        ws = self._workspace("gn", self.lib.idf_groupnorm_ws_floats(B, HW))
        _lib.check(self.lib.idf_groupnorm(_p(x), _p(out), _p(gamma), _p(beta), _p(ws), B, HW, Cc, float(eps),
                                          int(bool(silu)), self.dt, self._stream()), "idf_groupnorm")
        return out

    def layernorm(self, x, out, gamma, beta, eps=1e-5):
        M, Cc = x.shape
        _lib.check(self.lib.idf_layernorm(_p(x), x.stride(0), _p(out), out.stride(0), _p(gamma), _p(beta), M, Cc,
                                          float(eps), self.dt, self._stream()), "idf_layernorm")
        return out

    def row_stats(self, x, stats, eps=1e-5):
        M, Cc = x.shape
        assert stats.is_contiguous() and stats.dtype == torch.float32 and stats.numel() == 2 * M
        _lib.check(self.lib.idf_row_stats(_p(x), x.stride(0), _p(stats), M, Cc, float(eps), self.dt, self._stream()),
                   "idf_row_stats")
        return stats

    def layernorm_patch2(self, x, out, gamma, beta, eps):
        B, H, W_, Cc = x.shape
        assert x.is_contiguous() and out.stride(-1) == 1
        _lib.check(self.lib.idf_layernorm_patch2(_p(x), _p(out), out.stride(0), _p(gamma), _p(beta), B, H, W_, Cc,
                                                 float(eps), self.dt, self._stream()), "idf_layernorm_patch2")
        return out

    def seg_in_conv(self, segs, w, bias, out):
        B, Cin, S, _ = segs.shape
        assert segs.is_contiguous() and segs.dtype == torch.float32
        _lib.check(self.lib.idf_seg_in_conv(_p(segs), _p(w), _p(bias), _p(out), B, Cin, S, out.stride(0), self.dt,
                                            self._stream()), "idf_seg_in_conv")
        return out

    def dwconv7x7(self, x, w_tap_major, bias, out):
        B, H, W_, Cc = x.shape
        assert x.is_contiguous() and out.is_contiguous()
        _lib.check(self.lib.idf_dwconv7x7(_p(x), _p(w_tap_major), _p(bias), _p(out), B, H, W_, Cc, self.dt,
                                          self._stream()), "idf_dwconv7x7")
        return out

    def scaleu_concat(self, h, skip, out, hscale, sm1):
        B, H, W_, Ch = h.shape
        Cs = skip.shape[-1]
        assert h.is_contiguous() and skip.is_contiguous() and out.is_contiguous() and out.shape[-1] == Ch + Cs
        ws = self._workspace("scaleu", B * Cs * 64)
        _lib.check(self.lib.idf_scaleu_concat(_p(h), _p(skip), _p(out), _p(hscale), _p(sm1), _p(ws), B, H, W_, Ch, Cs,
                                              self.dt, self._stream()), "idf_scaleu_concat")
        return out

    def timestep_embedding(self, t_f32, out):
        B, dim = out.shape
        _lib.check(self.lib.idf_timestep_embedding(_p(t_f32), _p(out), B, dim, self.dt, self._stream()),
                   "idf_timestep_embedding")
        return out

    def unifusion_embed(self, text, loc, tmask, lmask, null_text, null_loc, freqs, out):
        rows, text_dim = text.shape
        D = loc.shape[-1]
        assert out.is_contiguous() and out.shape == (rows, text_dim + 32 * D)
        for t in (text, loc, tmask, lmask, null_text, null_loc, freqs):
            assert t.dtype == torch.float32 and t.is_contiguous()
        _lib.check(self.lib.idf_unifusion_embed(_p(text), _p(loc), _p(tmask), _p(lmask), _p(null_text), _p(null_loc),
                                                _p(freqs), _p(out), rows, text_dim, D, self.dt, self._stream()),
                   "idf_unifusion_embed")
        return out

    def cfg_combine(self, e_cond, e_uncond, guidance, out):
        _lib.check(self.lib.idf_cfg_combine(_p(e_cond), _p(e_uncond), float(guidance), _p(out), out.numel(),
                                            self._stream()), "idf_cfg_combine")
        return out

    def plms_update(self, x, e_t, old, e_next, mode, a_t, a_prev, sqrt_1m_at, out):
        e1 = old[-1] if len(old) >= 1 else None
        e2 = old[-2] if len(old) >= 2 else None
        e3 = old[-3] if len(old) >= 3 else None
        _lib.check(self.lib.idf_plms_update(_p(x), _p(e_t), _p(e1), _p(e2), _p(e3), _p(e_next), int(mode), float(a_t),
                                            float(a_prev), float(sqrt_1m_at), _p(out), out.numel(), self._stream()),
                   "idf_plms_update")
        return out

    def mis_merge(self, lat, boxes_i32, out, mode):
        n1, B, Cc, H, W_ = lat.shape
        assert lat.is_contiguous() and out.is_contiguous()
        _lib.check(self.lib.idf_mis_merge(_p(lat), _p(boxes_i32), _p(out), n1 - 1, B, Cc, H, W_, int(mode),
                                          self._stream()), "idf_mis_merge")
        return out

    def cast16(self, x_f32, out):
        assert x_f32.is_contiguous() and out.is_contiguous()
        _lib.check(self.lib.idf_cast_f32_to_16(_p(x_f32), _p(out), out.numel(), self.dt, self._stream()),
                   "idf_cast_f32_to_16")
        return out

    def softmax_rows(self, s_f32, out, scale):
        assert s_f32.dtype == torch.float32 and s_f32.is_contiguous() and out.is_contiguous() and out.shape == s_f32.shape
        n = s_f32.shape[-1]
        rows = s_f32.numel() // n
        _lib.check(self.lib.idf_softmax_rows(_p(s_f32), _p(out), rows, n, n, n, float(scale), self.dt, self._stream()),
                   "idf_softmax_rows")
        return out

    def pointwise_nchw(self, x, w, bias, out, in_scale=1.0):
        B, Cin = x.shape[0], x.shape[1]
        Cout = w.shape[0]
        HW = x.numel() // (B * Cin)
        for t in (x, w, out) + ((bias,) if bias is not None else ()):
            assert t.dtype == torch.float32 and t.is_contiguous()
        _lib.check(self.lib.idf_pointwise_nchw(_p(x), _p(w), _p(bias), _p(out), B, Cin, Cout, HW, float(in_scale),
                                               self._stream()), "idf_pointwise_nchw")
        return out
```

Baseline: 2.020 img/s.

## Fuse attention out-proj, LayerNorm, GEGLU MLP and following projection into one block kernel

Adds a new idf_mlp_geglu_block kernel that computes the attention output projection with residual and gate, derives the LayerNorm row stats on the fly, and runs the fused GEGLU MLP. It then applies either the next LN+Q projection or the proj_out residual projection, all inside one persistent launch. The engine uses it by default for C=320 transformer blocks, in both the fuser and the cross-attention paths. The goal is to remove several separate GEMM launches and the HBM round trips of intermediate activations and stats. The cost is extra LDS pressure (nearly the whole CU's LDS) and more serialized work per tile.

```diff
diff --git a/include/idf.h b/include/idf.h
--- a/include/idf.h
+++ b/include/idf.h
@@ -36,7 +36,8 @@
 enum { IDF_STAT_GEMM_BIG_LAUNCHES = 0, IDF_STAT_ATTN2_LAUNCHES = 1, IDF_STAT_GEMM_RING_LAUNCHES = 2, IDF_STAT_ATTN8_LAUNCHES = 3,
        IDF_STAT_GN_EPI_LAUNCHES = 4 ,
        IDF_STAT_QKV_ROW_LAUNCHES = 6 ,
-       IDF_STAT_GEGLU_ROW_LAUNCHES = 7  };
+       IDF_STAT_GEGLU_ROW_LAUNCHES = 7 ,
+       IDF_STAT_MLP_BLOCK_LAUNCHES = 8  };
 long long idf_get_stat(int stat);
 
 typedef struct {
@@ -70,6 +71,23 @@
   int dtype;
 } idf_mlp_args;
 int idf_mlp_geglu(const idf_mlp_args* a, void* stream);
+
+enum { IDF_MLPB_NONE = 0, IDF_MLPB_RES = 1, IDF_MLPB_LNQ = 2 };
+typedef struct {
+  idf_mlp_args mlp;
+  const void* att; int ldatt;
+  const void* wo; int ldwo;
+  const float* bo;
+  const float* gate0;
+  int mode;
+  const void* pw; int ldpw;
+  const float* pb;
+  const float* pc;
+  const void* pres; int ldpres;
+  void* pout; int ldpout;
+  float eps;
+} idf_mlp_block_args;
+int idf_mlp_geglu_block(const idf_mlp_block_args* a, void* stream);
 
 int idf_row_stats(const void* x, int ldx, float* stats, int M, int C, float eps, int dtype, void* stream);
 
diff --git a/instancediffusion_amd/_lib.py b/instancediffusion_amd/_lib.py
--- a/instancediffusion_amd/_lib.py
+++ b/instancediffusion_amd/_lib.py
@@ -8,7 +8,8 @@
 
 IDF_BF16, IDF_F16 = 0, 1
 IDF_STAT_GEMM_BIG_LAUNCHES, IDF_STAT_ATTN2_LAUNCHES, IDF_STAT_GEMM_RING_LAUNCHES, IDF_STAT_ATTN8_LAUNCHES, IDF_STAT_GN_EPI_LAUNCHES = 0, 1, 2, 3, 4
-IDF_STAT_QKV_ROW_LAUNCHES, IDF_STAT_GEGLU_ROW_LAUNCHES = 6, 7
+IDF_STAT_QKV_ROW_LAUNCHES, IDF_STAT_GEGLU_ROW_LAUNCHES, IDF_STAT_MLP_BLOCK_LAUNCHES = 6, 7, 8
+IDF_MLPB_NONE, IDF_MLPB_RES, IDF_MLPB_LNQ = 0, 1, 2
 IDF_TUNE_GEMM_BIG, IDF_TUNE_ATTN2, IDF_TUNE_GEMM_RING, IDF_TUNE_BIG_MIN_EFF, IDF_TUNE_ATTN8, IDF_TUNE_MLP, IDF_TUNE_QKV_ROW, IDF_TUNE_GEGLU_ROW = 0, 1, 2, 3, 4, 5, 6, 7
 EPI_LN_ROW, EPI_LN_COL, EPI_GEGLU_P32 = 512, 1024, 2048
 EPI_BIAS, EPI_ROWBIAS, EPI_RES, EPI_GATE, EPI_SILU, EPI_GELU, EPI_GEGLU, EPI_OUT_F32, EPI_OUT_NCHW = \
@@ -52,6 +53,13 @@
                 ("b2", vp), ("gate", vp), ("out", vp), ("ldo", ci), ("M", ci), ("C", ci), ("dtype", ci)]
 
 
+
+class MlpBlockArgs(C.Structure):
+    _fields_ = [("mlp", MlpArgs), ("att", vp), ("ldatt", ci), ("wo", vp), ("ldwo", ci), ("bo", vp), ("gate0", vp), ("mode", ci),
+                ("pw", vp), ("ldpw", ci), ("pb", vp), ("pc", vp), ("pres", vp), ("ldpres", ci), ("pout", vp), ("ldpout", ci),
+                ("eps", cf)]
+
+
 SYMBOLS = {
     "idf_abi_version": (ci, []),
     "idf_build_info": (C.c_char_p, []),
@@ -60,6 +68,7 @@
     "idf_gemm": (ci, [C.POINTER(GemmArgs), vp]),
     "idf_conv3x3": (ci, [C.POINTER(ConvArgs), vp]),
     "idf_mlp_geglu": (ci, [C.POINTER(MlpArgs), vp]),
+    "idf_mlp_geglu_block": (ci, [C.POINTER(MlpBlockArgs), vp]),
     "idf_conv_in": (ci, [vp, vp, vp, vp, ci, ci, ci, ci, ci, ci, vp]),
     "idf_attention": (ci, [C.POINTER(AttnArgs), vp]),
     "idf_groupnorm_ws_floats": (ll, [ci, ci]),
diff --git a/instancediffusion_amd/csrc/gemm_conv.hip b/instancediffusion_amd/csrc/gemm_conv.hip
--- a/instancediffusion_amd/csrc/gemm_conv.hip
+++ b/instancediffusion_amd/csrc/gemm_conv.hip
@@ -873,6 +873,7 @@
   if (stat == IDF_STAT_GN_EPI_LAUNCHES) return idf_stat_gn_epi_launches.load();
   if (stat == IDF_STAT_QKV_ROW_LAUNCHES) return idf_stat_qkvw_launches.load();
   if (stat == IDF_STAT_GEGLU_ROW_LAUNCHES) return idf_stat_gegluw_launches.load();
+  if (stat == IDF_STAT_MLP_BLOCK_LAUNCHES) return idf_stat_mlpb_launches.load();
   return -1;
 }
 
diff --git a/instancediffusion_amd/csrc/gemm_core.h b/instancediffusion_amd/csrc/gemm_core.h
--- a/instancediffusion_amd/csrc/gemm_core.h
+++ b/instancediffusion_amd/csrc/gemm_core.h
@@ -114,6 +114,7 @@
 
 #define IDF_BIG_UNSUPPORTED (-100)
 extern std::atomic<long long> idf_stat_big_launches;
+extern std::atomic<long long> idf_stat_mlpb_launches;
 int idf_launch_big(const idfcore::CoreParams& p, int dtype, bool conv, bool force, hipStream_t s, int* splitk_out,
                    int* parts_out = nullptr, int* tail_m0_out = nullptr, int* gst_out = nullptr);
 int idf_launch_qkv320w(const idfcore::CoreParams& p, int dtype, hipStream_t s);
diff --git a/instancediffusion_amd/csrc/mlp_fused.hip b/instancediffusion_amd/csrc/mlp_fused.hip
--- a/instancediffusion_amd/csrc/mlp_fused.hip
+++ b/instancediffusion_amd/csrc/mlp_fused.hip
@@ -27,6 +27,14 @@
   const float* b2; const float* gate;
   unsigned short* out; int ldo;
   int M;
+  const unsigned short* att; int ldatt;
+  const unsigned short* wo; int ldwo;
+  const float* bo; const float* gate0;
+  const unsigned short* pw; int ldpw;
+  const float* pb; const float* pc;
+  const unsigned short* pres; int ldpres;
+  unsigned short* pout; int ldpout;
+  float eps;
 };
 
 __device__ __forceinline__ void mlp_dma16(const void* sbase , unsigned voff_bytes, unsigned lds) {
@@ -311,9 +319,202 @@
 #endif
 #include MLPW_STREAM_INC
 
+constexpr int MW_PREG_BYTES = 320 * 64, MW_BSMEM = MW_SMEM + MW_PREG_BYTES;
+static_assert(MW_BSMEM <= 160 * 1024, "the block kernels use all but 768 B of the CU's LDS");
+__device__ __forceinline__ unsigned mw_preg(int r) { return r == 0 ? W1_BYTES : (r == 1 ? SLOT_BYTES + W1_BYTES : MW_SMEM); }
+struct MwProjSrc {
+  const char* wg; unsigned voff; size_t tstride;
+};
+__device__ __forceinline__ MwProjSrc mw_proj_src(const unsigned short* W, int ldw, int wave, int lane) {
+  asm volatile("" : "+v"(lane));
+  const int row2 = 16 * wave + (lane >> 2);
+  return MwProjSrc{reinterpret_cast<const char*>(W), (unsigned)(row2 * ldw + (((lane & 3) ^ ((row2 >> 2) & 3)) << 3)) * 2u,
+                   (size_t)64 * ldw * 2};
+}
+__device__ __forceinline__ void mw_proj_issue(const MwProjSrc& s, int i, unsigned smem_lds, int wave) {
+#pragma unroll
+  for (int t = 0; t < 5; ++t) mw_dma_rt(s.wg + (size_t)i * 64 + t * s.tstride, s.voff, smem_lds + mw_preg(i % 3) + (unsigned)(wave * 1024 + t * 4096));
+}
+__device__ __forceinline__ void mw_proj_prefetch(const unsigned short* W, int ldw, char* smem, int wave, int lane) {
+  const MwProjSrc src = mw_proj_src(W, ldw, wave, lane);
+#pragma unroll
+  for (int i = 0; i < 3; ++i) mw_proj_issue(src, i, lds_u32(smem), wave);
+}
 template <int DT>
-__global__ __launch_bounds__(256, 1) void mlp320w_kernel(const MlpParams p, const int tiles) {
-  asm volatile("" ::: "a0", "a239");
+__device__ __forceinline__ void mw_proj(const unsigned short* W, int ldw, char* smem, int wave, int lane) {
+  asm volatile("" : "+v"(lane));
+  const int l31 = lane & 31, hi = lane >> 5;
+  const MwProjSrc src = mw_proj_src(W, ldw, wave, lane);
+  const int sw2 = (l31 >> 2) & 3;
+  const char* fr[2];
+#pragma unroll
+  for (int kk = 0; kk < 2; ++kk) fr[kk] = smem + l31 * 64 + (((2 * kk + hi) ^ sw2) << 4);
+  mw_static_for<10>([&](auto ic) {
+    constexpr int i = decltype(ic)::value;
+    if constexpr (i == 0 || i == 9) asm volatile("s_waitcnt vmcnt(0)\n\ts_barrier" ::: "memory");
+    else asm volatile("s_waitcnt vmcnt(5)\n\ts_barrier" ::: "memory");
+    if constexpr (i >= 1 && i + 2 < 10) mw_proj_issue(src, i + 2, lds_u32(smem), wave);
+    mw_static_for<2>([&](auto kc) {
+      constexpr int kk = decltype(kc)::value;
+      u32x4 wf[10];
+#pragma unroll
+      for (int a = 0; a < 10; ++a) wf[a] = *reinterpret_cast<const u32x4*>(fr[kk] + mw_preg(i % 3) + a * 2048);
+      mw_static_for<10>([&](auto ac) { mw_mf3<DT, decltype(ac)::value, 2 * i + kk, i == 0 && kk == 0>(wf[decltype(ac)::value]); });
+    });
+  });
+  asm volatile("s_waitcnt lgkmcnt(0)\n\ts_barrier" ::: "memory");
+  asm volatile("s_nop 15\n\ts_nop 15\n\ts_nop 7" ::: "memory");
+}
+
+template <int A> __device__ __forceinline__ void mw_acc_cols(float* v) {
+  float acc[16];
+  mw_static_for<16>([&](auto rc) { acc[decltype(rc)::value] = __uint_as_float(mw_agpr_read<MW_OA + 16 * A + decltype(rc)::value>()); });
+#pragma unroll
+  for (int e = 0; e < 4; ++e) {
+    const auto s02 = __builtin_amdgcn_permlane32_swap(__float_as_uint(acc[e]), __float_as_uint(acc[8 + e]), false, false);
+    const auto s13 = __builtin_amdgcn_permlane32_swap(__float_as_uint(acc[4 + e]), __float_as_uint(acc[12 + e]), false, false);
+    v[e] = __uint_as_float(s02[0]); v[4 + e] = __uint_as_float(s02[1]);
+    v[8 + e] = __uint_as_float(s13[0]); v[12 + e] = __uint_as_float(s13[1]);
+  }
+}
+template <int A> __device__ __forceinline__ void mw_to_bfrag(const u32x4& q0, const u32x4& q1) {
+  mw_static_for<4>([&](auto dc) {
+    constexpr int d = decltype(dc)::value;
+    const auto sw = __builtin_amdgcn_permlane32_swap(q0[d], q1[d], false, false);
+    mw_agpr_write<MW_XA + 4 * (2 * A) + d>(sw[0]);
+    mw_agpr_write<MW_XA + 4 * (2 * A + 1) + d>(sw[1]);
+  });
+}
+template <int DT, int A> __device__ __forceinline__ void mw_stats_acc(const u32x4& q0, const u32x4& q1, float& pv, float& s1, float& s2) {
+  float r[16];
+  unpack8<DT>(q0, r);
+  unpack8<DT>(q1, r + 8);
+  if constexpr (A == 0) pv = r[0];
+#pragma unroll
+  for (int j = 0; j < 16; ++j) { const float d = r[j] - pv; s1 += d; s2 = fmaf(d, d, s2); }
+}
+template <int DT> __device__ __forceinline__ void mw_bfrag_stats(float& pv, float& s1, float& s2) {
+  mw_static_for<20>([&](auto kc) {
+    constexpr int ks = decltype(kc)::value;
+    u32x4 q;
+    mw_static_for<4>([&](auto dc) { q[decltype(dc)::value] = mw_agpr_read<MW_XA + 4 * ks + decltype(dc)::value>(); });
+    float r[8];
+    unpack8<DT>(q, r);
+    if constexpr (ks == 0) pv = r[0];
+#pragma unroll
+    for (int j = 0; j < 8; ++j) { const float d = r[j] - pv; s1 += d; s2 = fmaf(d, d, s2); }
+  });
+}
+__device__ __forceinline__ f32x2 mw_stats_fin(float pv, float s1, float s2, float eps) {
+  constexpr float cnt = 160.0f;
+  const float mean = pv + s1 * (1.0f / cnt);
+  const float m2 = fmaxf(s2 - s1 * s1 * (1.0f / cnt), 0.0f);
+  const float mean_o = __shfl_xor(mean, 32, 64), m2_o = __shfl_xor(m2, 32, 64);
+  const float dlt = mean_o - mean;
+  return f32x2{0.5f * (mean + mean_o), rsqrtf((m2 + m2_o + dlt * dlt * (0.5f * cnt)) / (float)MLP_C + eps)};
+}
+
+template <int DT>
+__device__ __forceinline__ f32x2 mw_block_pro(const MlpParams& p, int tile, char* smem, int wave, int lane, bool load_att) {
+  const int l31 = lane & 31, hi = lane >> 5;
+  const size_t m = (size_t)tile * MLP_BM + wave * 32 + l31;
+  if (load_att) {
+    const unsigned short* const ar = p.att + m * p.ldatt + 8 * hi;
+    mw_static_for<20>([&](auto kc) { mw_load_x<decltype(kc)::value>(ar); });
+  }
+  const unsigned short* const yr = p.x + m * p.ldx + 16 * hi;
+  u32x4 rr[20];
+#pragma unroll
+  for (int a = 0; a < 10; ++a) {
+    rr[2 * a] = *reinterpret_cast<const u32x4*>(yr + 32 * a);
+    rr[2 * a + 1] = *reinterpret_cast<const u32x4*>(yr + 32 * a + 8);
+  }
+  const float g0 = p.gate0 ? p.gate0[0] : 1.0f;
+  mw_proj<DT>(p.wo, p.ldwo, smem, wave, lane);
+  float pv = 0.0f, s1 = 0.0f, s2 = 0.0f;
+  mw_static_for<10>([&](auto ac) {
+    constexpr int a = decltype(ac)::value;
+    float v[16];
+    mw_acc_cols<a>(v);
+    const float* const bp = p.bo + 32 * a + 16 * hi;
+#pragma unroll
+    for (int jq = 0; jq < 4; ++jq) {
+      const f32x4 bq = *reinterpret_cast<const f32x4*>(bp + 4 * jq);
+#pragma unroll
+      for (int e = 0; e < 4; ++e) v[4 * jq + e] += bq[e];
+    }
+    float r[16];
+    unpack8<DT>(rr[2 * a], r);
+    unpack8<DT>(rr[2 * a + 1], r + 8);
+#pragma unroll
+    for (int j = 0; j < 16; ++j) v[j] = fmaf(g0, v[j], r[j]);
+    const u32x4 q0 = pack8<DT>(v), q1 = pack8<DT>(v + 8);
+    mw_stats_acc<DT, a>(q0, q1, pv, s1, s2);
+    mw_to_bfrag<a>(q0, q1);
+  });
+  return mw_stats_fin(pv, s1, s2, p.eps);
+}
+
+template <int DT, int BLK>
+__device__ __forceinline__ void mw_block_epi(const MlpParams& p, int tile, int next, char* smem, int wave, int lane) {
+  const int l31 = lane & 31, hi = lane >> 5;
+  const size_t m = (size_t)tile * MLP_BM + wave * 32 + l31;
+  [[maybe_unused]] f32x2 st;
+  [[maybe_unused]] u32x4 rr[20];
+  if constexpr (BLK == 3) {
+    float pv = 0.0f, s1 = 0.0f, s2 = 0.0f;
+    mw_bfrag_stats<DT>(pv, s1, s2);
+    st = mw_stats_fin(pv, s1, s2, p.eps);
+  }
+  if constexpr (BLK == 2) {
+    const unsigned short* const xr = p.pres + m * p.ldpres + 16 * hi;
+#pragma unroll
+    for (int a = 0; a < 10; ++a) {
+      rr[2 * a] = *reinterpret_cast<const u32x4*>(xr + 32 * a);
+      rr[2 * a + 1] = *reinterpret_cast<const u32x4*>(xr + 32 * a + 8);
+    }
+  }
+  mw_proj<DT>(p.pw, p.ldpw, smem, wave, lane);
+  if (next >= 0) {
+    mw_proj_prefetch(p.wo, p.ldwo, smem, wave, lane);
+    const unsigned short* const ar = p.att + ((size_t)next * MLP_BM + wave * 32 + l31) * p.ldatt + 8 * hi;
+    mw_static_for<20>([&](auto kc) { mw_load_x<decltype(kc)::value>(ar); });
+  }
+  unsigned short* const o = p.pout + m * p.ldpout + 16 * hi;
+  mw_static_for<10>([&](auto ac) {
+    constexpr int a = decltype(ac)::value;
+    float v[16];
+    mw_acc_cols<a>(v);
+    if constexpr (BLK == 3) {
+      const float* const cp = p.pc + 32 * a + 16 * hi;
+#pragma unroll
+      for (int jq = 0; jq < 4; ++jq) {
+        const f32x4 cq = *reinterpret_cast<const f32x4*>(cp + 4 * jq);
+#pragma unroll
+        for (int e = 0; e < 4; ++e) v[4 * jq + e] = st[1] * fmaf(-st[0], cq[e], v[4 * jq + e]);
+      }
+    }
+    const float* const bp = p.pb + 32 * a + 16 * hi;
+#pragma unroll
+    for (int jq = 0; jq < 4; ++jq) {
+      const f32x4 bq = *reinterpret_cast<const f32x4*>(bp + 4 * jq);
+#pragma unroll
+      for (int e = 0; e < 4; ++e) v[4 * jq + e] += bq[e];
+    }
+    if constexpr (BLK == 2) {
+      float r[16];
+      unpack8<DT>(rr[2 * a], r);
+      unpack8<DT>(rr[2 * a + 1], r + 8);
+#pragma unroll
+      for (int j = 0; j < 16; ++j) v[j] = fmaf(1.0f, v[j], r[j]);
+    }
+    *reinterpret_cast<u32x4*>(o + 32 * a) = pack8<DT>(v);
+    *reinterpret_cast<u32x4*>(o + 32 * a + 8) = pack8<DT>(v + 8);
+  });
+}
+
+template <int DT, int BLK>
+__device__ __forceinline__ void mw_run(const MlpParams& p, const int tiles) {
   extern __shared__ __attribute__((aligned(128))) char smem[];
   const int tid = threadIdx.x;
   const int lane = tid & 63, wave = __builtin_amdgcn_readfirstlane(tid >> 6);
@@ -397,14 +598,19 @@
 #define MW_TRT(i)
 #endif
   auto row_ptr = [&](int t) { return p.x + (size_t)(t * MLP_BM + wave * 32 + l31) * p.ldx + 8 * hi; };
-  {
-    const unsigned short* xr = row_ptr(tile);
-    mw_static_for<20>([&](auto kc) { mw_load_x<decltype(kc)::value>(xr); });
-  }
-  f32x2 st = *reinterpret_cast<const f32x2*>(p.ln_stats + 2 * (size_t)(tile * MLP_BM + wave * 32 + l31));
-  asm volatile("" : "+v"(st));
+  f32x2 st;
+  if constexpr (BLK == 0) {
+    {
+      const unsigned short* xr = row_ptr(tile);
+      mw_static_for<20>([&](auto kc) { mw_load_x<decltype(kc)::value>(xr); });
+    }
+    st = *reinterpret_cast<const f32x2*>(p.ln_stats + 2 * (size_t)(tile * MLP_BM + wave * 32 + l31));
+    asm volatile("" : "+v"(st));
+  }
+  if constexpr (BLK > 0) mw_proj_prefetch(p.wo, p.ldwo, smem, wave, lane);
   bool first = true;
   for (;;) {
+    if constexpr (BLK > 0) st = mw_block_pro<DT>(p, tile, smem, wave, lane, first);
     c.nmu2 = f32x2{-st[0], -st[0]};
     c.rstd2 = f32x2{st[1], st[1]};
     asm volatile("" : "+v"(c.nmu2), "+v"(c.rstd2));
@@ -441,11 +647,17 @@
     mw_drain<DT>(acc1[0], acc1[1], hh[1], hh[0], c);
     asm volatile("s_nop 15\n\ts_nop 15\n\ts_nop 7" ::: "memory");
     MW_TRT(9)
+    if constexpr (BLK > 0) {
+      asm volatile("s_waitcnt lgkmcnt(0)\n\ts_barrier" ::: "memory");
+      if constexpr (BLK >= 2) mw_proj_prefetch(p.pw, p.ldpw, smem, wave, lane);
+      else if (tile + G < tiles) mw_proj_prefetch(p.wo, p.ldwo, smem, wave, lane);
+    }
 
     const int next = tile + G;
     const bool has_next = next < tiles;
-    const unsigned short* const xn = row_ptr(has_next ? next : tile);
-    if (has_next) st = *reinterpret_cast<const f32x2*>(p.ln_stats + 2 * (size_t)(next * MLP_BM + wave * 32 + l31));
+    [[maybe_unused]] const unsigned short* const xn = BLK == 0 ? row_ptr(has_next ? next : tile)
+                                              : p.att + (size_t)((has_next ? next : tile) * MLP_BM + wave * 32 + l31) * p.ldatt + 8 * hi;
+    if (BLK == 0 && has_next) st = *reinterpret_cast<const f32x2*>(p.ln_stats + 2 * (size_t)(next * MLP_BM + wave * 32 + l31));
 #ifdef MW_DIRECT_STORES
     unsigned short* const orow = p.out + (size_t)(tile * MLP_BM + wave * 32 + l31) * p.ldo + 16 * hi;
 #else
@@ -459,7 +671,7 @@
     const char* const b2l = smem + MW_B2_OFF + 64 * hi;
     mw_static_for<10>([&](auto ac) {
       constexpr int a = decltype(ac)::value;
-      if constexpr (a == 9) asm volatile("" : "+v"(st));
+      if constexpr (a == 9 && BLK == 0) asm volatile("" : "+v"(st));
       float acc[16];
       mw_static_for<16>([&](auto rc) { acc[decltype(rc)::value] = __uint_as_float(mw_agpr_read<MW_OA + 16 * a + decltype(rc)::value>()); });
       float v[16];
@@ -484,13 +696,18 @@
         r0[d] = sw[0]; r1[d] = sw[1];
       });
 #ifndef MW_NO_XLOAD
-      if (has_next) { mw_load_x<2 * a>(xn); mw_load_x<2 * a + 1>(xn); }
+      if (BLK <= 1 && has_next) { mw_load_x<2 * a>(xn); mw_load_x<2 * a + 1>(xn); }
 #endif
       float r[16];
       unpack8<DT>(r0, r);
       unpack8<DT>(r1, r + 8);
 #pragma unroll
       for (int jq = 0; jq < 16; ++jq) v[jq] = fmaf(gate, v[jq], r[jq]);
+      if constexpr (BLK >= 2) {
+        const u32x4 q0 = pack8<DT>(v), q1 = pack8<DT>(v + 8);
+        mw_to_bfrag<a>(q0, q1);
+      }
+      if constexpr (BLK == 2) return;
 #ifdef MW_DIRECT_STORES
       *reinterpret_cast<u32x4*>(orow + 32 * a) = pack8<DT>(v);
       *reinterpret_cast<u32x4*>(orow + 32 * a + 8) = pack8<DT>(v + 8);
@@ -510,12 +727,25 @@
 #endif
     });
     MW_TRT(8)
+    if constexpr (BLK >= 2) mw_block_epi<DT, BLK>(p, tile, has_next ? next : -1, smem, wave, lane);
     if (!has_next) break;
     tile = next;
   }
 #ifdef IDF_MLPW_TRACE
   if ((int)blockIdx.x == (int)gridDim.x / 2 && lane == 0) { for (int i = 0; i < 12; ++i) idf_mlpw_trace_buf[wave][i] = c.tr[i]; }
 #endif
+}
+
+template <int DT>
+__global__ __launch_bounds__(256, 1) void mlp320w_kernel(const MlpParams p, const int tiles) {
+  asm volatile("" ::: "a0", "a239");
+  mw_run<DT, 0>(p, tiles);
+}
+
+template <int DT, int BLK>
+__global__ __launch_bounds__(256, 1) void mlp320b_kernel(const MlpParams p, const int tiles) {
+  asm volatile("" ::: "a0", "a239");
+  mw_run<DT, BLK>(p, tiles);
 }
 
 template <int DT>
@@ -531,6 +761,19 @@
   return idf_launch_status();
 }
 
+template <int DT, int BLK>
+int launch_mlp320b(const MlpParams& p, hipStream_t s) {
+  void (*kern)(const MlpParams, const int) = mlp320b_kernel<DT, BLK>;
+  static std::atomic<unsigned long long> attr_done{0};
+  if (const int e = idf_lds_optin(reinterpret_cast<const void*>(kern), MW_BSMEM, attr_done)) return e;
+  int dev = 0, cus = 0;
+  if (hipGetDevice(&dev) != hipSuccess || hipDeviceGetAttribute(&cus, hipDeviceAttributeMultiprocessorCount, dev) != hipSuccess || cus <= 0) cus = 256;
+  const int tiles = p.M / MLP_BM;
+  const int grid = tiles < cus ? tiles : cus;
+  hipLaunchKernelGGL(kern, dim3(grid), dim3(256), MW_BSMEM, s, p, tiles);
+  return idf_launch_status();
+}
+
 #ifndef IDF_MLP_MODE_DEFAULT
 #define IDF_MLP_MODE_DEFAULT 1
 #endif
@@ -560,23 +803,71 @@
 }
 #endif
 
-extern "C" int idf_mlp_geglu(const idf_mlp_args* a, void* stream) {
+std::atomic<long long> idf_stat_mlpb_launches{0};
+
+namespace {
+int mlp_validate(const idf_mlp_args* a, bool block) {
   if (!a) return IDF_E_ARG;
-  if (!a->x || !a->ln_stats || !a->w1 || !a->cd || !a->w2p || !a->b2 || !a->out) return IDF_E_ARG;
+  if (!a->x || (!block && !a->ln_stats) || !a->w1 || !a->cd || !a->w2p || !a->b2 || !a->out) return IDF_E_ARG;
   if (a->M <= 0 || a->C <= 0) return IDF_E_ARG;
   if (a->dtype != IDF_BF16 && a->dtype != IDF_F16) return IDF_E_ARG;
   if (a->C != MLP_C || (a->M % MLP_BM) != 0) return IDF_E_UNSUPPORTED;
   if (a->ldx < MLP_C || a->ldo < MLP_C || a->ldw1 < MLP_C || a->ldw2 < MLP_H) return IDF_E_ARG;
   if ((a->ldx % 8) || (a->ldo % 8) || (a->ldw1 % 8) || (a->ldw2 % 8)) return IDF_E_ALIGN;
   if (!aligned16(a->x) || !aligned16(a->out) || !aligned16(a->w1) || !aligned16(a->w2p) || !aligned16(a->cd) || !aligned16(a->b2) ||
-      (((uintptr_t)a->ln_stats) & 7u))
+      (!block && (((uintptr_t)a->ln_stats) & 7u)))
     return IDF_E_ALIGN;
   if ((long long)64 * a->ldw1 * 2 >= (1ll << 31) || (long long)320 * a->ldw2 * 2 >= (1ll << 31)) return IDF_E_UNSUPPORTED;
-  MlpParams p;
+  return 0;
+}
+
+void mlp_params(const idf_mlp_args* a, MlpParams& p) {
+  p = MlpParams{};
   p.x = static_cast<const unsigned short*>(a->x); p.ldx = a->ldx; p.ln_stats = a->ln_stats;
   p.w1 = static_cast<const unsigned short*>(a->w1); p.ldw1 = a->ldw1; p.cd = a->cd;
   p.w2p = static_cast<const unsigned short*>(a->w2p); p.ldw2 = a->ldw2; p.b2 = a->b2; p.gate = a->gate;
   p.out = static_cast<unsigned short*>(a->out); p.ldo = a->ldo; p.M = a->M;
+}
+}
+
+extern "C" int idf_mlp_geglu_block(const idf_mlp_block_args* b, void* stream) {
+  if (!b) return IDF_E_ARG;
+  if (const int e = mlp_validate(&b->mlp, true)) return e;
+  if (b->mode != IDF_MLPB_NONE && b->mode != IDF_MLPB_RES && b->mode != IDF_MLPB_LNQ) return IDF_E_ARG;
+  if (!b->att || !b->wo || !b->bo) return IDF_E_ARG;
+  if (b->mode != IDF_MLPB_NONE && (!b->pw || !b->pb || !b->pout)) return IDF_E_ARG;
+  if ((b->mode == IDF_MLPB_RES && !b->pres) || (b->mode == IDF_MLPB_LNQ && (!b->pc || !(b->eps > 0.0f)))) return IDF_E_ARG;
+  if (b->mode == IDF_MLPB_NONE && !(b->eps > 0.0f)) return IDF_E_ARG;
+  const bool pres = b->mode == IDF_MLPB_RES, proj = b->mode != IDF_MLPB_NONE;
+  if (b->ldatt < MLP_C || b->ldwo < MLP_C || (proj && (b->ldpw < MLP_C || b->ldpout < MLP_C)) || (pres && b->ldpres < MLP_C)) return IDF_E_ARG;
+  if ((b->ldatt % 8) || (b->ldwo % 8) || (proj && ((b->ldpw % 8) || (b->ldpout % 8))) || (pres && (b->ldpres % 8))) return IDF_E_ALIGN;
+  if (!aligned16(b->att) || !aligned16(b->wo) || !aligned16(b->bo) ||
+      (proj && (!aligned16(b->pw) || !aligned16(b->pb) || !aligned16(b->pout))) || (pres && !aligned16(b->pres)) ||
+      (b->mode == IDF_MLPB_LNQ && !aligned16(b->pc)))
+    return IDF_E_ALIGN;
+  if ((long long)320 * b->ldwo * 2 >= (1ll << 31) || (proj && (long long)320 * b->ldpw * 2 >= (1ll << 31))) return IDF_E_UNSUPPORTED;
+  if (mlp_mode() != 1) return IDF_E_UNSUPPORTED;
+  MlpParams p;
+  mlp_params(&b->mlp, p);
+  p.att = static_cast<const unsigned short*>(b->att); p.ldatt = b->ldatt;
+  p.wo = static_cast<const unsigned short*>(b->wo); p.ldwo = b->ldwo; p.bo = b->bo; p.gate0 = b->gate0;
+  p.pw = static_cast<const unsigned short*>(b->pw); p.ldpw = b->ldpw; p.pb = b->pb; p.pc = b->pc;
+  p.pres = static_cast<const unsigned short*>(b->pres); p.ldpres = b->ldpres;
+  p.pout = static_cast<unsigned short*>(b->pout); p.ldpout = b->ldpout; p.eps = b->eps;
+  hipStream_t s = static_cast<hipStream_t>(stream);
+  const bool bf = b->mlp.dtype == IDF_BF16;
+  int rc;
+  if (b->mode == IDF_MLPB_NONE) rc = bf ? launch_mlp320b<IDF_BF16, 1>(p, s) : launch_mlp320b<IDF_F16, 1>(p, s);
+  else if (b->mode == IDF_MLPB_RES) rc = bf ? launch_mlp320b<IDF_BF16, 2>(p, s) : launch_mlp320b<IDF_F16, 2>(p, s);
+  else rc = bf ? launch_mlp320b<IDF_BF16, 3>(p, s) : launch_mlp320b<IDF_F16, 3>(p, s);
+  if (rc == 0) idf_stat_mlpb_launches.fetch_add(1);
+  return rc;
+}
+
+extern "C" int idf_mlp_geglu(const idf_mlp_args* a, void* stream) {
+  if (const int e = mlp_validate(a, false)) return e;
+  MlpParams p;
+  mlp_params(a, p);
   hipStream_t s = static_cast<hipStream_t>(stream);
   if (mlp_mode() == 1) return a->dtype == IDF_BF16 ? launch_mlp320w<IDF_BF16>(p, s) : launch_mlp320w<IDF_F16>(p, s);
   return a->dtype == IDF_BF16 ? launch_mlp320<IDF_BF16>(p, s) : launch_mlp320<IDF_F16>(p, s);
diff --git a/instancediffusion_amd/csrc/mw_prims.h b/instancediffusion_amd/csrc/mw_prims.h
--- a/instancediffusion_amd/csrc/mw_prims.h
+++ b/instancediffusion_amd/csrc/mw_prims.h
@@ -121,6 +121,17 @@
   asm volatile("global_load_dwordx4 a[%c1:%c2], %0, off offset:%c3" ::"v"(rowp), "n"(MW_XA + 4 * KA), "n"(MW_XA + 4 * KA + 3), "n"(32 * KO) : "memory");
 }
 
+template <int DT, int A, int KS, bool FIRST> __device__ __forceinline__ void mw_mf3(const u32x4& w) {
+  constexpr int lo = MW_OA + 16 * A, xb = MW_XA + 4 * KS;
+  if constexpr (FIRST) {
+    if constexpr (DT == IDF_BF16) asm volatile("v_mfma_f32_32x32x16_bf16 a[%c1:%c2], %0, a[%c3:%c4], 0" ::"v"(w), "n"(lo), "n"(lo + 15), "n"(xb), "n"(xb + 3));
+    else asm volatile("v_mfma_f32_32x32x16_f16 a[%c1:%c2], %0, a[%c3:%c4], 0" ::"v"(w), "n"(lo), "n"(lo + 15), "n"(xb), "n"(xb + 3));
+  } else {
+    if constexpr (DT == IDF_BF16) asm volatile("v_mfma_f32_32x32x16_bf16 a[%c1:%c2], %0, a[%c3:%c4], a[%c1:%c2]" ::"v"(w), "n"(lo), "n"(lo + 15), "n"(xb), "n"(xb + 3));
+    else asm volatile("v_mfma_f32_32x32x16_f16 a[%c1:%c2], %0, a[%c3:%c4], a[%c1:%c2]" ::"v"(w), "n"(lo), "n"(lo + 15), "n"(xb), "n"(xb + 3));
+  }
+}
+
 template <int DT, int KS, bool FIRST> __device__ __forceinline__ void mw_mf1t(f32x16& acc, const u32x4& w) {
   constexpr int lo = MW_XA + 4 * KS;
   if constexpr (FIRST) {
diff --git a/instancediffusion_amd/engine.py b/instancediffusion_amd/engine.py
--- a/instancediffusion_amd/engine.py
+++ b/instancediffusion_amd/engine.py
@@ -28,6 +28,10 @@
     raise ValueError(f"IDF_MLP_FUSED={MLP_FUSED}: must be 0 or 1")
 MLP_FUSED = MLP_FUSED == "1" and GEGLU_PERIOD == 32
 MLP_MIN_M = int(os.environ.get("IDF_MLP_MIN_M", "32768"))
+MLP_BLOCK = os.environ.get("IDF_MLP_BLOCK", "1")
+if MLP_BLOCK not in ("0", "1"):
+    raise ValueError(f"IDF_MLP_BLOCK={MLP_BLOCK}: must be 0 or 1")
+MLP_BLOCK = MLP_BLOCK == "1"
 PAIR_HOIST = os.environ.get("IDF_PAIR_HOIST", "1")
 if PAIR_HOIST not in ("0", "1"):
     raise ValueError(f"IDF_PAIR_HOIST={PAIR_HOIST}: must be 0 or 1")
@@ -540,6 +544,10 @@
                        ln_row=(None if LN_SELF_MODE == 2 else st, f["c1"]))
         return ops.gemm(mid, f["l2"].w, y, bias=f["l2"].b, res=y, gate=gate, out_stats=out_stats)
 
+    def _ff_block(self, f, M, C):
+        return (MLP_BLOCK and getattr(self.ops, "mlp_block", False) and LN_SELF_MODE == 1 and self._ln_self(C) and "w2p" in f
+                and M >= MLP_MIN_M and self.ops.mlp_supported(M, C))
+
     def _dup(self, t: torch.Tensor, role: str) -> torch.Tensor:
         n = t.shape[0]
         out = self.buf(role, (2 * n,) + tuple(t.shape[1:]), t.dtype)
@@ -576,14 +584,30 @@
         if fuser_on:
             vis = cond.vis if (cond.vis and N == MASK_RES * MASK_RES) else None
             att = self._self_attn(p["f_attn"], y, st, B, N, C, kv_extra=(cond.k_obj[i], cond.vt_obj[i]), vis=vis)
+        a2 = p["attn2"]
+        q = None
+        if fuser_on and self._ff_block(p["f_ff"], M, C):
+            f = p["f_ff"]
+            qb = self.buf("st.q", (M, C))
+            if ops.mlp_geglu(y, None, f["w1"], f["cd"], f["w2p"], f["l2"].b, y, gate=self.gates[i, 1:2], att=att.view(M, C),
+                             wo=p["f_attn"]["out"].w, bo=p["f_attn"]["out"].b, gate0=self.gates[i, 0:1], proj="lnq",
+                             proj_w=a2["wq"], proj_b=a2["dq"], proj_c=a2["cq"], proj_out=qb) is not None:
+                q = qb
+        if fuser_on and q is None:
             ops.gemm(att.view(M, C), p["f_attn"]["out"].w, y, bias=p["f_attn"]["out"].b, res=y, gate=self.gates[i, 0:1],
                      out_stats=ffs)
             self._ff(p["f_ff"], y, st, M, C, gate=self.gates[i, 1:2], out_stats=pre)
-        a2 = p["attn2"]
-        q = ops.gemm(y, a2["wq"], self.buf("st.q", (M, C)), bias=a2["dq"],
-                     ln_row=(None if own else st, a2["cq"])).view(B, N, C)
+        if q is None:
+            q = ops.gemm(y, a2["wq"], self.buf("st.q", (M, C)), bias=a2["dq"], ln_row=(None if own else st, a2["cq"]))
+        q = q.view(B, N, C)
         att = self.buf("st.att", (B, N, C))
         ops.attention(q, cond.k_ctx[i], cond.vt_ctx[i], cond.n_ctx, att, self.heads)
+        if self._ff_block(p["ff"], M, C):
+            f = p["ff"]
+            if ops.mlp_geglu(y, None, f["w1"], f["cd"], f["w2p"], f["l2"].b, y, att=att.view(M, C), wo=a2["out"].w,
+                             bo=a2["out"].b, proj="res", proj_w=p["proj_out"].w, proj_b=p["proj_out"].b, proj_res=x.view(M, C),
+                             proj_out=x.view(M, C)) is not None:
+                return x
         ops.gemm(att.view(M, C), a2["out"].w, y, bias=a2["out"].b, res=y, out_stats=ffs)
         self._ff(p["ff"], y, st, M, C)
         ops.gemm(y, p["proj_out"].w, x.view(M, C), bias=p["proj_out"].b, res=x.view(M, C))
diff --git a/instancediffusion_amd/ops.py b/instancediffusion_amd/ops.py
--- a/instancediffusion_amd/ops.py
+++ b/instancediffusion_amd/ops.py
@@ -135,6 +135,8 @@
 
     MLP_W2_PERM = (0, 1, 2, 3, 8, 9, 10, 11, 4, 5, 6, 7, 12, 13, 14, 15)
 
+    mlp_block = True
+
     @staticmethod
     def mlp_supported(M: int, C: int) -> bool:
         return C == 320 and M % 128 == 0
@@ -148,18 +150,44 @@
         w2p = w2_16.view(n, k // 16, 16).index_select(2, perm).reshape(n, k).contiguous()
         return cd, w2p
 
-    def mlp_geglu(self, x, stats, w1, cd, w2p, b2, out, *, gate=None):
+    def mlp_geglu(self, x, stats, w1, cd, w2p, b2, out, *, gate=None, att=None, wo=None, bo=None, gate0=None, proj=None,
+                  proj_w=None, proj_b=None, proj_c=None, proj_res=None, proj_out=None, eps=1e-5):
         M, Cc = x.shape
         assert self.mlp_supported(M, Cc) and out.shape == x.shape and x.stride(-1) == 1 and out.stride(-1) == 1
-        assert stats.is_contiguous() and stats.dtype == torch.float32 and stats.numel() == 2 * M
         assert w1.shape == (8 * Cc, Cc) and w2p.shape == (Cc, 4 * Cc) and cd.is_contiguous() and cd.numel() == 16 * Cc
         assert w1.stride(-1) == 1 and w2p.stride(-1) == 1 and b2.dtype == torch.float32 and cd.dtype == torch.float32
-        args = _lib.MlpArgs(x=x.data_ptr(), ldx=x.stride(0), ln_stats=stats.data_ptr(), w1=w1.data_ptr(), ldw1=w1.stride(0),
-                            cd=cd.data_ptr(), w2p=w2p.data_ptr(), ldw2=w2p.stride(0), b2=b2.data_ptr(),
+        if att is None:
+            assert stats.is_contiguous() and stats.dtype == torch.float32 and stats.numel() == 2 * M
+        args = _lib.MlpArgs(x=x.data_ptr(), ldx=x.stride(0), ln_stats=None if stats is None else stats.data_ptr(), w1=w1.data_ptr(),
+                            ldw1=w1.stride(0), cd=cd.data_ptr(), w2p=w2p.data_ptr(), ldw2=w2p.stride(0), b2=b2.data_ptr(),
                             gate=None if gate is None else gate.data_ptr(), out=out.data_ptr(), ldo=out.stride(0), M=M, C=Cc,
                             dtype=self.dt)
-        _lib.check(self.lib.idf_mlp_geglu(C.byref(args), self._stream()), "idf_mlp_geglu")
-        return out
+        if att is None:
+            _lib.check(self.lib.idf_mlp_geglu(C.byref(args), self._stream()), "idf_mlp_geglu")
+            return out
+        mode = {None: _lib.IDF_MLPB_NONE, "res": _lib.IDF_MLPB_RES, "lnq": _lib.IDF_MLPB_LNQ}[proj]
+        assert att.shape == (M, Cc) and att.stride(-1) == 1 and wo.shape == (Cc, Cc) and wo.stride(-1) == 1
+        assert bo.dtype == torch.float32 and bo.numel() == Cc
+        if proj is not None:
+            assert proj_w.shape == (Cc, Cc) and proj_w.stride(-1) == 1 and proj_b.dtype == torch.float32 and proj_b.numel() == Cc
+            assert proj_out.shape == (M, Cc) and proj_out.stride(-1) == 1
+        if proj == "res":
+            assert proj_res.shape == (M, Cc) and proj_res.stride(-1) == 1
+        if proj == "lnq":
+            assert proj_c.dtype == torch.float32 and proj_c.numel() == Cc
+        bargs = _lib.MlpBlockArgs(
+            mlp=args, att=att.data_ptr(), ldatt=att.stride(0), wo=wo.data_ptr(), ldwo=wo.stride(0), bo=bo.data_ptr(),
+            gate0=None if gate0 is None else gate0.data_ptr(), mode=mode,
+            pw=None if proj_w is None else proj_w.data_ptr(), ldpw=0 if proj_w is None else proj_w.stride(0),
+            pb=None if proj_b is None else proj_b.data_ptr(), pc=None if proj_c is None else proj_c.data_ptr(),
+            pres=None if proj_res is None else proj_res.data_ptr(), ldpres=0 if proj_res is None else proj_res.stride(0),
+            pout=None if proj_out is None else proj_out.data_ptr(), ldpout=0 if proj_out is None else proj_out.stride(0),
+            eps=float(eps))
+        rc = self.lib.idf_mlp_geglu_block(C.byref(bargs), self._stream())
+        if rc == -3:
+            return None
+        _lib.check(rc, "idf_mlp_geglu_block")
+        return proj_out if proj == "res" else out
 
     @staticmethod
     def gn_partial_shape(B, HW, C):
```

After: 2.026 img/s, median of 6. Within noise of the previous version (+0.3%).
